# voutcn/megahit

Measured on NVIDIA H100. Metric: sorted (k+1)-mer edges/sec at k=27 on 150bp reads, higher is better.
Workload: dtype u32

## Files before the change

### include/mhb.h

```cpp
#ifndef MHB_H
#define MHB_H
#include <stddef.h>
#include <stdint.h>

#ifdef __cplusplus
extern "C" {
#endif

#define MHB_OK 0
#define MHB_ERR_ARG 1
#define MHB_ERR_CUDA 2
#define MHB_ERR_IO 3
#define MHB_ERR_NOMEM 4

#define MHB_NUM_BUCKETS 65536
#define MHB_MAX_MUL 65535
#define MHB_MAX_K 255
#define MHB_SENTINEL_OFFSET 0xFFFFFFFFu

const char *mhb_last_error(void);
const char *mhb_version(void);
int mhb_device_count(void);
uint64_t mhb_launch_count(void);

uint32_t mhb_count_record_words(uint32_t k);
uint32_t mhb_words_per_edge(uint32_t k);
uint32_t mhb_s2s_record_words(uint32_t k);
uint32_t mhb_count_sort_bytes(uint32_t k, uint8_t *bytes);
uint32_t mhb_s2s_sort_bytes(uint32_t k, uint8_t *bytes);
size_t mhb_sort_workspace_bytes(uint64_t n, uint32_t words);


typedef struct {
  const uint32_t *bin;
  uint64_t bin_words;
  uint64_t n_reads;
  uint32_t fixed_len;
  const uint64_t *rec_off;
  const uint64_t *edge_off;
} mhb_dev_reads;

int mhb_count_extract(void *stream, const mhb_dev_reads *reads, uint32_t k, uint32_t *records,
                      uint64_t n_edges, uint64_t *hist256, int hist_byte);

int mhb_check_fixed_len(void *stream, const uint32_t *bin_dev, uint64_t n_reads, uint32_t fixed_len, uint64_t *flag_dev);

int mhb_count_extract_range(void *stream, const mhb_dev_reads *reads, uint32_t k, uint32_t lo, uint32_t hi, int write,
                            uint64_t *per_read, uint32_t *records, uint64_t *hist256, int hist_byte,
                            uint64_t *total_dev);

int mhb_sort_records(void *stream, uint32_t *a, uint32_t *b, uint64_t n, uint32_t words,
                     const uint8_t *bytes, uint32_t n_bytes, const uint64_t *first_hist, void *ws,
                     size_t ws_bytes, int *result_in_b);

int mhb_sort_records_relaxed(void *stream, uint32_t *a, uint32_t *b, uint64_t n, uint32_t words, const uint8_t *bytes,
                             uint32_t n_bytes, const uint64_t *first_hist, void *ws, size_t ws_bytes, int *result_in_b);

int mhb_partition_scatter(void *stream, const uint32_t *recs, uint64_t n, uint32_t words, int byte,
                          const uint8_t *owner_of_byte_dev, const uint64_t *bin_addr_dev, void *ws, size_t ws_bytes);
int mhb_partition_scatter_hist(void *stream, const uint32_t *recs, uint64_t n, uint32_t words, int byte,
                               const uint8_t *owner_of_byte_dev, const uint64_t *bin_addr_dev, void *ws, size_t ws_bytes,
                               int next_byte, uint64_t *owner_next_hist, int *hist_done);
int mhb_plan_partition(void *stream, const uint64_t *hist_all_dev, uint32_t world, uint32_t rank, uint32_t record_bytes,
                       const uint64_t *peer_base_host, uint8_t *owner_lut_dev, uint64_t *bin_addr_dev, uint64_t *plan_dev);
int mhb_compact_tip_edges(void *stream, const uint32_t *edges, const uint8_t *aux, uint64_t n_solid, uint32_t k,
                          uint32_t *tips_out, uint8_t *tip_aux_out, uint64_t capacity, uint64_t *cursor_dev);
int mhb_dev_malloc(void **ptr, size_t bytes);
int mhb_dev_free(void *ptr);
int mhb_ipc_export(const void *dev_ptr, uint8_t *handle64);
int mhb_ipc_open(const uint8_t *handle64, void **peer_ptr);
int mhb_ipc_close(void *peer_ptr);

int mhb_set_sort_cfg(int cfg);

int mhb_sort_pass_ms(int back, double *pass_ms, uint32_t max_passes, uint32_t *n_passes, uint64_t *n_records,
                     uint32_t *words);

size_t mhb_count_solid_scratch_bytes(uint64_t n);
int mhb_count_solid(void *stream, const uint32_t *sorted_records, uint64_t n, uint32_t k, int32_t m,
                    uint32_t *edges_out, uint8_t *aux_out, uint64_t capacity_edges, uint64_t *mul_hist,
                    uint64_t *n_solid_out, void *scratch, size_t scratch_bytes);

int mhb_count_hashed_supported(uint32_t k, int32_t m);
size_t mhb_count_hashed_workspace_bytes(uint64_t n, uint32_t k, int32_t m);
int mhb_count_solid_hashed(void *stream, uint32_t *recs_a, uint32_t *recs_b, uint64_t n, uint32_t k, int32_t m,
                           const uint64_t *hist_byte5, uint32_t *edges_out, uint8_t *aux_out, uint64_t capacity_edges,
                           uint64_t *mul_hist, uint64_t *n_solid_out, void *ws, size_t ws_bytes);

size_t mhb_tipset_bytes(uint64_t n_tip_edges, uint32_t k);
int mhb_tipset_build(void *stream, const uint32_t *edges, const uint8_t *aux, uint64_t n_solid, uint32_t k,
                     void *tipset, size_t tipset_bytes, uint64_t n_tip_edges);
int mhb_count_mark_mercy(void *stream, const mhb_dev_reads *reads, uint32_t k, const void *tipset,
                         size_t tipset_bytes, uint64_t n_tip_edges, uint32_t *first_0_out, uint32_t *last_0_in);
int mhb_count_tip_edges(void *stream, const uint8_t *aux, uint64_t n_solid, uint64_t *n_tip_host);

size_t mhb_mercy_candidates_scratch_bytes(uint64_t n_reads);
int mhb_mercy_candidates(void *stream, const uint32_t *first_0_out, const uint32_t *last_0_in, uint64_t n_reads,
                         uint64_t *cand_ids, uint64_t *n_cand_host, void *scratch, size_t scratch_bytes);
size_t mhb_mercy_edges_scratch_bytes(uint64_t n_cand, uint32_t max_read_len);
int mhb_mercy_edges(void *stream, const mhb_dev_reads *reads, const uint64_t *cand_ids, uint64_t n_cand,
                    uint32_t max_read_len, uint32_t k, const uint32_t *edges, uint64_t n_edges, uint32_t *mercy_out,
                    uint64_t capacity, uint64_t *n_mercy_host, void *scratch, size_t scratch_bytes);
int mhb_mercy_edges_count(void *stream, const mhb_dev_reads *reads, const uint64_t *cand_ids, uint64_t n_cand,
                          uint32_t max_read_len, uint32_t k, uint32_t n_segs, const uint32_t *const *seg_edges,
                          const uint64_t *seg_counts, const void *const *seg_luts, const uint8_t *owner_of_byte,
                          uint64_t *n_mercy_host, void *scratch, size_t scratch_bytes);
int mhb_mercy_edges_write(void *stream, const mhb_dev_reads *reads, const uint64_t *cand_ids, uint64_t n_cand,
                          uint32_t max_read_len, uint32_t k, uint32_t *mercy_out, uint64_t capacity, uint64_t n_mercy,
                          void *scratch, size_t scratch_bytes);

size_t mhb_mercy_planes_words(uint64_t n_cand, uint32_t max_read_len);
int mhb_mercy_probe_owned(void *stream, const mhb_dev_reads *reads, const uint64_t *cand_ids, uint64_t n_cand,
                          uint32_t max_read_len, uint32_t k, const uint32_t *edges, uint64_t n_edges, const void *lut,
                          const uint8_t *owner_of_byte, uint32_t me, uint32_t *planes_out);
int mhb_mercy_count_planes(void *stream, const mhb_dev_reads *reads, const uint64_t *cand_ids, uint64_t n_cand,
                           uint32_t max_read_len, uint32_t k, const uint32_t *planes, uint32_t n_src,
                           uint64_t src_stride_words, uint64_t *n_mercy_host, void *scratch, size_t scratch_bytes);

int mhb_mercy_edges_segs(void *stream, const mhb_dev_reads *reads, const uint64_t *cand_ids, uint64_t n_cand,
                         uint32_t max_read_len, uint32_t k, uint32_t n_segs, const uint32_t *const *seg_edges,
                         const uint64_t *seg_counts, const void *const *seg_luts, const uint8_t *owner_of_byte,
                         uint32_t *mercy_out, uint64_t capacity, uint64_t *n_mercy_host, void *scratch,
                         size_t scratch_bytes);
size_t mhb_edge_lut_bytes(void);
int mhb_edge_lut_build(void *stream, const uint32_t *edges, uint64_t n_edges, uint32_t k, void *lut);

typedef struct {
  const uint32_t *words;
  uint64_t n_words;
  uint64_t n_seqs;
  uint32_t fixed_len;
  const uint64_t *word_off;
  const uint32_t *len;
  const uint64_t *item_off;
  const uint16_t *mult;
  uint32_t fixed_stride;
} mhb_dev_seqs;

int mhb_s2s_extract(void *stream, const mhb_dev_seqs *seqs, uint32_t k, uint32_t *records, uint64_t n_items,
// ... 139 lines not shown

typedef struct {
  uint32_t *bin;
  uint64_t bin_words;
  uint64_t n_reads, n_bases;
  uint32_t n_libs;
  uint64_t *lib_begin, *lib_end;
  uint32_t *lib_max_len;
  uint64_t n_chunks;
  uint64_t n_walk_passes;
  double t_total_ms;
} mhb_buildlib_result;

int mhb_buildlib_host(const mhb_buildlib_args *args, mhb_buildlib_result *res);
void mhb_buildlib_free(mhb_buildlib_result *res);
int mhb_set_buildlib_chunk(uint64_t bytes);

int mhb_mercy_host(uint32_t k, const uint32_t *edges, uint64_t n_edges, const uint32_t *cand_bin, uint64_t cand_words,
                   uint32_t **mercy_out, uint64_t *n_mercy_out, uint64_t *n_cand_reads_out);

void mhb_free(void *p);
int mhb_release(void);

typedef struct {
  uint32_t k;
  int32_t m;
  double host_mem;
  int32_t num_cpu_threads;
  const char *read_lib_file;
  const char *output_prefix;
  int32_t mem_flag;
} mhb_count_opts;

typedef struct {
  double host_mem;
  uint32_t k;
  uint32_t k_from;
  int32_t num_cpu_threads;
  const char *contig;
  const char *bubble;
  const char *addi_contig;
  const char *local_contig;
  const char *input_prefix;
  const char *output_prefix;
  int32_t need_mercy;
  int32_t mem_flag;
} mhb_seq2sdbg_opts;

typedef struct {
  uint32_t k;
  int32_t m;
  double host_mem;
  int32_t num_cpu_threads;
  const char *read_lib_file;
  const char *output_prefix;
  int32_t mem_flag;
  int32_t need_mercy;
} mhb_read2sdbg_opts;

typedef struct {
  const char *contig_file;
  const char *bubble_file;
  const char *read_file;
  int32_t num_cpu_threads;
  uint32_t k;
  uint32_t step;
  const char *output_prefix;
} mhb_iterate_opts;

int mhb_count_run(const mhb_count_opts *opts);
int mhb_seq2sdbg_run(const mhb_seq2sdbg_opts *opts);
int mhb_iterate_run(const mhb_iterate_opts *opts);
int mhb_read2sdbg_run(const mhb_read2sdbg_opts *opts);
int mhb_buildlib_run(const char *lib_file, const char *out_prefix);

int mhb_count_run_multi(const mhb_count_opts *opts, int n_gpus);

int mhb_selftest_count_record(const uint32_t *read_words, uint32_t nwords, uint32_t L, uint32_t k, uint32_t q,
                              uint32_t *rec_out, uint32_t *strand_out);
int mhb_selftest_count_records_roll(const uint32_t *read_words, uint32_t nwords, uint32_t L, uint32_t k, uint32_t q,
                                    uint64_t *rec4_out, uint32_t *strand4_out);
int mhb_selftest_s2s_record(const uint32_t *seq_words, uint32_t nwords, uint32_t L, uint32_t k, uint32_t strand,
                            uint32_t offset, uint32_t mult, uint32_t *rec_out);

int mhb_selftest_r2s_s1_record(const uint32_t *pkg_words, uint32_t nwords, uint32_t L, uint32_t k, uint32_t e,
                               uint64_t base_off, uint32_t *rec_out);
int mhb_selftest_r2s_item(const uint32_t *pkg_words, uint32_t nwords, uint32_t L, uint32_t k, uint32_t i, uint32_t strand,
                          uint32_t type, uint32_t *rec_out, uint32_t *palindrome_out);
int mhb_selftest_kmsort(uint32_t *recs, uint64_t n, uint32_t nw);
int mhb_selftest_kmsort_smem(uint32_t *recs, uint64_t n, uint32_t nw, uint32_t cap, uint32_t wcap);
int mhb_selftest_r2s_s1_group(const uint32_t *recs, uint64_t n, uint32_t k, int32_t m, uint32_t fixed_len, uint64_t n_reads,
                              int need_mercy, uint32_t *is_solid, uint32_t *no_in, uint32_t *no_out, uint32_t *any,
                              int64_t *counting);
int mhb_selftest_iterate(const mhb_iterate_args *args, mhb_iterate_result *res);
int mhb_selftest_fastx(const uint8_t *text, uint64_t n, uint32_t *len_out, uint32_t *bpos_out, uint64_t cap,
                       uint64_t *n_rec_out, uint32_t *bin_out, uint64_t bin_cap, uint64_t *bin_words_out);
int mhb_selftest_r2s_mercy_read(uint32_t fixed_len, uint64_t n_reads, uint64_t r, uint32_t k, const uint32_t *is_solid,
                                const uint32_t *no_in, const uint32_t *no_out, const uint32_t *any, uint32_t *mercy,
                                uint32_t *added_out);

#ifdef __cplusplus
}
#endif
#endif
```

### megahit_b200/csrc/mhb_hashcount.cu

```cuda
#include <cuda_runtime.h>
#include <stdio.h>
#include <string.h>

#include "mhb.h"
#include "mhb_common.cuh"
#include "mhb_count.cuh"

using namespace mhb;

namespace {

constexpr int kHcHist = 1024;
constexpr u64 kHcEmpty = ~0ull;
constexpr int kHcBatch = 8;
constexpr u32 kRemBits = 42;
constexpr u32 kHcHotCount = 256;
constexpr int kHcHotRound = 32;
constexpr int kHcMaxProbes = 48;
constexpr int kHcStack = 72;
constexpr u32 kHcHistDone = 1u << 31;
constexpr u32 kHcPrefetchChunk = 16384;

__device__ __forceinline__ u64 rec_key64(const uint2 r) { return ((u64)r.x << 32) | r.y; }

__global__ void k_bucket_bounds(const uint2 *__restrict__ recs, u64 n, u64 *__restrict__ bounds) {
  const u32 b = blockIdx.x * blockDim.x + threadIdx.x;
  if (b > 65536u) return;
  u64 lo = 0, hi = n;
  while (lo < hi) {
    const u64 mid = (lo + hi) >> 1;
    if ((recs[mid].x >> 16) < b) lo = mid + 1;
    else hi = mid;
  }
  bounds[b] = lo;
}

__device__ __forceinline__ u64 hc_align(const uint2 *__restrict__ recs, u64 p, u64 lo, u64 hi) {
  if (p <= lo) return lo;
  if (p >= hi) return hi;
  const u32 pre = recs[p - 1].x >> 8;
  u64 a = p, z = hi;
  while (a < z) {
    const u64 mid = (a + z) >> 1;
    if ((recs[mid].x >> 8) > pre) z = mid;
    else a = mid + 1;
  }
  return a;
}

__global__ void k_slice_plan(const uint2 *__restrict__ recs, const u64 *__restrict__ bounds, const u64 *__restrict__ slice_off,
                             int m, ulonglong2 *__restrict__ plan, u64 *__restrict__ slice_base, u32 *__restrict__ slice_bucket) {
  const u32 b = blockIdx.x * blockDim.x + threadIdx.x;
  if (b >= 65536u) return;
  const u64 s0 = slice_off[b], ns = slice_off[b + 1] - s0;
  if (!ns) return;
  const u64 blo = bounds[b], bhi = bounds[b + 1], step = (bhi - blo + ns - 1) / ns;
  u64 lo = blo;
  for (u64 i = 0; i < ns; ++i) {
    const u64 hi = i + 1 == ns ? bhi : hc_align(recs, blo + (i + 1) * step, blo, bhi);
    plan[s0 + i] = make_ulonglong2(lo, hi);
    slice_base[s0 + i] = lo / (u64)m + s0 + i;
    slice_bucket[s0 + i] = b;
    lo = hi;
  }
}

template <int THREADS_, int LOG_SLOTS_, int CTAS_>
struct HcGeom {
  static constexpr int THREADS = THREADS_, LOG_SLOTS = LOG_SLOTS_, SLOTS = 1 << LOG_SLOTS_, CTAS = CTAS_;
  static constexpr int MAX_SOLID = SLOTS / 4;
  static constexpr int CELLS = 2 * THREADS;
  static constexpr int LOG_CELLS = LOG_SLOTS_ - 2 >= 0 ? (THREADS_ == 256 ? 9 : (THREADS_ == 512 ? 10 : 11)) : 9;
  static constexpr u32 SLICE = (u32)(SLOTS * 1.83);
};

template <class G>
struct HcShared {
  u64 keys[G::SLOTS];
  u32 cnt[G::SLOTS];
  u32 pt[G::SLOTS];
  u32 nt[G::SLOTS];
  u64 sorted[G::MAX_SOLID];
  u64 tmp[G::MAX_SOLID];
  u32 cell_base[G::CELLS];
  u32 cell_cur[G::CELLS];
  u32 cta_hist[kHcHist];
  u32 wide[kHcHotRound][8];
  uint16_t hot_rank[G::MAX_SOLID];
  u64 st_prefix[kHcStack];
  u32 st_bits[kHcStack];
  u32 warp_sum[G::THREADS / 32];
  ulonglong2 nx_range[2];
  u32 nx_sl[2];
  u32 n_solid[2], n_hot[2], overflow[2];
};

__device__ __forceinline__ u32 lane_lt_mask() { return (1u << (threadIdx.x & 31)) - 1u; }

__device__ __forceinline__ void smem_add(u32 *p, u32 v) {
  asm volatile("red.shared.add.u32 [%0], %1;" ::"r"((u32)__cvta_generic_to_shared(p)), "r"(v) : "memory");
}

__device__ __forceinline__ void hc_prefetch_l2(const uint2 *recs, u64 lo, u64 hi) {
  const u64 a0 = (u64)(recs + lo) & ~15ull, a1 = (u64)(recs + hi) & ~15ull;
  for (u64 a = a0; a < a1; a += kHcPrefetchChunk) {
    const u32 sz = (u32)(a1 - a < kHcPrefetchChunk ? a1 - a : kHcPrefetchChunk);
    asm volatile("cp.async.bulk.prefetch.L2.global [%0], %1;" ::"l"(a), "r"(sz) : "memory");
  }
}

template <class G>
__device__ __forceinline__ u32 hc_hash(u64 r) { return (u32)((r * 0x9E3779B97F4A7C15ull) >> (64 - G::LOG_SLOTS)); }

template <class G>
__device__ __forceinline__ u32 hc_insert(HcShared<G> &s, u64 r) {
  u32 h = hc_hash<G>(r);
  for (int probes = 0; probes < kHcMaxProbes; ++probes) {
    u64 cur = s.keys[h];
// ... 358 lines not shown
                                                             misc + 1);
  CK_LAUNCH();
  return MHB_OK;
}

struct HcLayout {
  size_t sort_ws, off_bounds, off_bcnt, off_soff, off_bsum, off_misc, off_scount, off_sdst, off_sbase, off_sbucket, off_plan,
      off_list, total;
  uint64_t max_slices;
};
HcLayout hc_layout(uint64_t n, int32_t m) {
  HcLayout L;
  auto pad = [](size_t x) { return (x + 255) & ~(size_t)255; };
  L.max_slices = n / HcGeomB::SLICE + 65536 + 2;
  L.sort_ws = pad(mhb_sort_workspace_bytes(n, 2));
  size_t p = L.sort_ws;
  L.off_bounds = p;
  p += pad(65537 * 8);
  L.off_bcnt = p;
  p += pad(65537 * 4);
  L.off_soff = p;
  p += pad(65537 * 8);
  L.off_bsum = p;
  p += pad((L.max_slices / kScanTile + 4) * 8);
  L.off_misc = p;
  p += 256;
  L.off_scount = p;
  p += pad(L.max_slices * 4);
  L.off_sdst = p;
  p += pad(L.max_slices * 8);
  L.off_sbase = p;
  p += pad(L.max_slices * 8);
  L.off_sbucket = p;
  p += pad(L.max_slices * 4);
  L.off_plan = p;
  p += pad(L.max_slices * 16);
  L.off_list = p;
  p += pad((size_t)(n / (uint64_t)(m < 1 ? 1 : m) + L.max_slices + 8) * 8);
  L.total = p;
  return L;
}

}

extern "C" int mhb_count_hashed_supported(uint32_t k, int32_t m) {
  return count_record_words(k) == 2 && 2 * (k + 1) >= 24 && m >= 1 && m <= kHcHist;
}

extern "C" size_t mhb_count_hashed_workspace_bytes(uint64_t n, uint32_t k, int32_t m) {
  (void)k;
  return hc_layout(n, m).total;
}

extern "C" int mhb_count_solid_hashed(void *stream, uint32_t *recs_a, uint32_t *recs_b, uint64_t n, uint32_t k, int32_t m,
                                      const uint64_t *hist_byte5, uint32_t *edges_out, uint8_t *aux_out,
                                      uint64_t capacity_edges, uint64_t *mul_hist, uint64_t *n_solid_out, void *ws,
                                      size_t ws_bytes) {
  if (!mhb_count_hashed_supported(k, m)) return mhb_set_error(MHB_ERR_ARG, "hashed count needs 8-byte records (13 <= k <= 28) and 1 <= m <= %d", kHcHist);
  if (!mul_hist || !n_solid_out || !ws) return mhb_set_error(MHB_ERR_ARG, "bad args");
  if (n == 0) return MHB_OK;
  if (n >= (1ull << 40)) return mhb_set_error(MHB_ERR_ARG, "too many records for one hashed count call");
  const HcLayout L = hc_layout(n, m);
  if (ws_bytes < L.total) return mhb_set_error(MHB_ERR_ARG, "hashed count workspace too small (%zu < %zu)", ws_bytes, L.total);
  cudaStream_t st = (cudaStream_t)stream;
  const uint8_t bytes[3] = {5, 6, 7};
  int in_b = 0;
  if (int rc = mhb_sort_records_impl(st, recs_a, recs_b, n, 2, bytes, 3, hist_byte5, ws, L.sort_ws, &in_b, nullptr)) return rc;
  const uint2 *recs = (const uint2 *)(in_b ? recs_b : recs_a);
  char *w = (char *)ws;
  u64 *bounds = (u64 *)(w + L.off_bounds);
  u32 *bcnt = (u32 *)(w + L.off_bcnt);
  u64 *slice_off = (u64 *)(w + L.off_soff);
  u64 *bsum = (u64 *)(w + L.off_bsum);
  u32 *misc = (u32 *)(w + L.off_misc);
  u32 *slice_count = (u32 *)(w + L.off_scount);
  u64 *slice_dst = (u64 *)(w + L.off_sdst);
  u64 *slice_base = (u64 *)(w + L.off_sbase);
  u32 *slice_bucket = (u32 *)(w + L.off_sbucket);
  ulonglong2 *plan = (ulonglong2 *)(w + L.off_plan);
  u64 *list = (u64 *)(w + L.off_list);
  u64 *n_slices_dev = (u64 *)(misc + 2);
  CK(cudaMemsetAsync(misc, 0, 256, st));
  CK(cudaMemsetAsync(slice_count, 0, L.max_slices * 4, st));
  k_bucket_bounds<<<(65537 + 255) / 256, 256, 0, st>>>(recs, n, bounds);
  CK_LAUNCH();
  k_slice_counts<<<65536 / 256, 256, 0, st>>>(bounds, HcGeomB::SLICE, bcnt);
  CK_LAUNCH();
  if (int rc = scan_counts(st, bcnt, 65536, slice_off, n_slices_dev, bsum)) return rc;
  CK(cudaMemcpyAsync(slice_off + 65536, n_slices_dev, 8, cudaMemcpyDeviceToDevice, st));
  k_slice_plan<<<65536 / 256, 256, 0, st>>>(recs, bounds, slice_off, m, plan, slice_base, slice_bucket);
  CK_LAUNCH();
  if (int rc = launch_hash_count<HcGeomB>(st, recs, plan, n_slices_dev, m, misc, list, slice_count, mul_hist)) return rc;
  if (int rc = scan_counts(st, slice_count, L.max_slices, slice_dst, n_solid_out, bsum)) return rc;
  k_hash_gather<<<sm_count() * 4, 256, 0, st>>>(list, n_slices_dev, slice_count, slice_dst, slice_base, slice_bucket,
                                               words_per_edge(k), edges_out, aux_out, capacity_edges, misc + 1, n_solid_out);
  CK_LAUNCH();
  return MHB_OK;
}
```

### megahit_b200/csrc/mhb_host.cu

```cuda
#include <cuda_runtime.h>
#include <stdio.h>
#include <stdlib.h>
#include <string.h>

#include <algorithm>
#include <vector>

#include "mhb.h"
#include "mhb_bits.cuh"
#include "mhb_internal.h"

using namespace mhb;

#define CK(call)                                                                                   \
  do {                                                                                             \
    cudaError_t e_ = (call);                                                                       \
    if (e_ != cudaSuccess)                                                                         \
      return mhb_set_error(MHB_ERR_CUDA, "%s failed at %s:%d: %s", #call, __FILE__, __LINE__,      \
                           cudaGetErrorString(e_));                                                \
  } while (0)
#define CKR(call)           \
  do {                      \
    int rc_ = (call);       \
    if (rc_) return rc_;    \
// ... 570 lines not shown
  res->t_h2d_ms = t.stop();

  mhb_dev_reads reads;
  reads.bin = d_bin;
  reads.bin_words = args->bin_words;
  reads.n_reads = n_reads;
  reads.fixed_len = ix.fixed_len;
  reads.rec_off = d_rec_off;
  reads.edge_off = d_edge_off;

  t.start();
  CKR(mhb_count_extract(st, &reads, k, d_a, n, d_hist0, cw.hist_byte));
  res->t_extract_ms = t.stop();

  t.start();
  res->n_rounds = 1;
  CKR(run_count_stage(st, cw, d_a, d_b, n, k, m, d_hist0, d_edges, d_aux, cap_edges, d_mul_hist, d_nsolid, d_work,
                      res->sort_pass_ms, &res->n_sort_passes));
  for (uint32_t p = 0; p < res->n_sort_passes; ++p) res->t_sort_ms += res->sort_pass_ms[p];
  uint64_t n_solid = 0;
  CK(cudaMemcpyAsync(&n_solid, d_nsolid, 8, cudaMemcpyDeviceToHost, st));
  CK(cudaStreamSynchronize(st));
  res->t_count_ms = t.stop();
  if (n_solid > cap_edges) return mhb_set_error(MHB_ERR_NOMEM, "internal: solid edges exceed capacity");
  res->n_solid = n_solid;

  std::vector<uint32_t> h_first, h_last;
  if (args->want_mercy && n_reads) {
    t.start();
    uint64_t n_tip = 0;
    CKR(mhb_count_tip_edges(st, d_aux, n_solid, &n_tip));
    const size_t ts_bytes = mhb_tipset_bytes(n_tip, k);
    char *d_tips = nullptr;
    uint32_t *d_free = d_a;
    bool own = false;
    if (ts_bytes <= (size_t)n * WR * 4) d_tips = (char *)d_free;
    else {
      CK(cudaMalloc((void **)&d_tips, ts_bytes));
      own = true;
    }
    int rc = mhb_tipset_build(st, d_edges, d_aux, n_solid, k, d_tips, ts_bytes, n_tip);
    if (!rc) rc = mhb_count_mark_mercy(st, &reads, k, d_tips, ts_bytes, n_tip, d_first, d_last);
    h_first.resize(n_reads);
    h_last.resize(n_reads);
    if (!rc) {
      cudaMemcpyAsync(h_first.data(), d_first, n_reads * 4, cudaMemcpyDeviceToHost, st);
      cudaMemcpyAsync(h_last.data(), d_last, n_reads * 4, cudaMemcpyDeviceToHost, st);
      if (cudaStreamSynchronize(st) != cudaSuccess) rc = mhb_set_error(MHB_ERR_CUDA, "mercy marking failed: %s", cudaGetErrorString(cudaGetLastError()));
    }
    if (own) cudaFree(d_tips);
    if (rc) return rc;
    res->t_mercy_ms = t.stop();
  }

  t.start();
  res->edges = (uint32_t *)malloc(std::max<size_t>(1, (size_t)n_solid * WE * 4));
  if (!res->edges) return mhb_set_error(MHB_ERR_NOMEM, "host malloc failed");
  if (n_solid) CK(cudaMemcpyAsync(res->edges, d_edges, (size_t)n_solid * WE * 4, cudaMemcpyDeviceToHost, st));
  std::vector<uint64_t> h_hist(65536);
  CK(cudaMemcpyAsync(h_hist.data(), d_mul_hist, 65536 * 8, cudaMemcpyDeviceToHost, st));
  CK(cudaStreamSynchronize(st));
  res->t_d2h_ms = t.stop();
  for (int i = 0; i <= MHB_MAX_MUL; ++i) res->counting[i] = (int64_t)h_hist[i];

  if (args->want_mercy) {
    std::vector<uint64_t> ids;
    for (uint64_t r = 0; r < n_reads; ++r) {
      const uint32_t f = h_first[r], l = h_last[r];
      if (f != MHB_SENTINEL_OFFSET && l != MHB_SENTINEL_OFFSET) {
        ++res->n_has_tips;
        if (l > f) ids.push_back(r);
      }
    }
    res->n_cand = ids.size();
    res->cand_ids = (uint64_t *)malloc(std::max<size_t>(1, ids.size() * 8));
    if (!ids.empty()) memcpy(res->cand_ids, ids.data(), ids.size() * 8);
  }
  res->t_total_ms = t_all.stop();
  return MHB_OK;
}

namespace {
size_t s2s_round_bytes(uint64_t n, uint32_t W, uint32_t k) {
  return 2 * Arena::pad((size_t)n * W * 4 + 16) + Arena::pad(mhb_sort_workspace_bytes(n, W)) +
         Arena::pad(mhb_s2s_emit_scratch_bytes(n, k)) + Arena::pad((size_t)n * (4ull + 4ull * words_per_tip_label(k)) + 16);
}
}

static int s2s_host_rounds(const mhb_s2s_args *args, mhb_s2s_result *res, const std::vector<uint64_t> &item_off,
                           uint64_t n_items, bool fixed, uint32_t L0, uint64_t n_words, uint64_t max_items) {
  const uint32_t k = args->k;
  const uint64_t ns = args->n_seqs;
  const uint32_t W = s2s_record_words(k), WPT = words_per_tip_label(k);
  uint8_t sort_bytes[72];
  const uint32_t n_sort = mhb_s2s_sort_bytes(k, sort_bytes);
  const int top_byte = (int)(4 * W - 1);
  cudaStream_t st = 0;
  Timer t_all(st), t(st);
  t_all.start();

  const size_t fixed_b = Arena::pad(n_words * 4 + 64) + Arena::pad((ns + 1) * 8) * 2 + Arena::pad((ns + 1) * 4) +
                         Arena::pad((ns + 1) * 2) + Arena::pad((size_t)MHB_NUM_BUCKETS * 4 * 8) + 2 * Arena::pad(256 * 8) +
                         Arena::pad(16 * 8) + Arena::pad(64) + 8192;
  if (!max_items) {
    size_t free_b = 0, total_b = 0;
    CK(cudaMemGetInfo(&free_b, &total_b));
    const size_t avail = (size_t)((double)(free_b + g_arena.cap) * 0.92);
    if (avail <= fixed_b) return mhb_set_error(MHB_ERR_NOMEM, "the sequences alone (%zu bytes) do not fit the device", fixed_b);
    uint64_t lo = 1, hi = n_items;
    while (lo < hi) {
      const uint64_t mid = lo + (hi - lo + 1) / 2;
      if (fixed_b + s2s_round_bytes(mid, W, k) <= avail) lo = mid;
      else hi = mid - 1;
    }
    max_items = lo;
  }
  max_items = std::min<uint64_t>(std::max<uint64_t>(max_items, 1), std::max<uint64_t>(n_items, 1));
  CKR(g_arena.reserve(fixed_b + s2s_round_bytes(max_items, W, k)));
  uint32_t *d_words = g_arena.take<uint32_t>(n_words + 16);
  uint64_t *d_word_off = g_arena.take<uint64_t>(ns + 1);
  uint64_t *d_item_off = g_arena.take<uint64_t>(ns + 1);
  uint32_t *d_len = g_arena.take<uint32_t>(ns + 1);
  uint16_t *d_mult = g_arena.take<uint16_t>(ns + 1);
  uint64_t *d_table = g_arena.take<uint64_t>((size_t)MHB_NUM_BUCKETS * 4);
  uint64_t *d_hist0 = g_arena.take<uint64_t>(256);
  uint64_t *d_hist_top = g_arena.take<uint64_t>(256);
  uint64_t *d_totals = g_arena.take<uint64_t>(16);
  uint64_t *d_cursor = g_arena.take<uint64_t>(8);
  uint32_t *d_a = g_arena.take<uint32_t>((size_t)max_items * W + 4);
  uint32_t *d_b = g_arena.take<uint32_t>((size_t)max_items * W + 4);
  const size_t ws_bytes = mhb_sort_workspace_bytes(max_items, W);
  const size_t scratch_bytes = mhb_s2s_emit_scratch_bytes(max_items, k);
  const uint64_t cap_bytes = max_items * (4ull + 4ull * WPT) + 16;
  char *d_ws = g_arena.take<char>(ws_bytes);
  char *d_scratch = g_arena.take<char>(scratch_bytes);
  uint8_t *d_bytes = g_arena.take<uint8_t>(cap_bytes);

  if (ns) {
    CK(cudaMemcpyAsync(d_words, args->words, n_words * 4, cudaMemcpyHostToDevice, st));
    CK(cudaMemcpyAsync(d_word_off, args->word_off, (ns + 1) * 8, cudaMemcpyHostToDevice, st));
    CK(cudaMemcpyAsync(d_item_off, item_off.data(), (ns + 1) * 8, cudaMemcpyHostToDevice, st));
    CK(cudaMemcpyAsync(d_len, args->len, ns * 4, cudaMemcpyHostToDevice, st));
    CK(cudaMemcpyAsync(d_mult, args->mult, ns * 2, cudaMemcpyHostToDevice, st));
  }
  CK(cudaMemsetAsync(d_hist_top, 0, 256 * 8, st));
  mhb_dev_seqs seqs;
  seqs.words = d_words;
  seqs.n_words = n_words;
  seqs.n_seqs = ns;
  seqs.fixed_len = fixed ? L0 : 0;
  seqs.word_off = d_word_off;
  seqs.len = d_len;
  seqs.item_off = d_item_off;
  seqs.mult = d_mult;
  seqs.fixed_stride = 0;

  t.start();
  uint64_t h_top[256];
  CKR(mhb_s2s_extract_range(st, &seqs, k, nullptr, n_items, 0, 65535, nullptr, 0, d_hist_top, top_byte));
  CK(cudaMemcpyAsync(h_top, d_hist_top, sizeof(h_top), cudaMemcpyDeviceToHost, st));
  CK(cudaStreamSynchronize(st));
  std::vector<uint64_t> h_sub;
  for (uint32_t b = 0; b < 256; ++b) {
    if (h_top[b] <= max_items) continue;
    if (h_sub.empty()) h_sub.assign(256 * 256, 0);
    CK(cudaMemsetAsync(d_hist0, 0, 256 * 8, st));
    CKR(mhb_s2s_extract_range(st, &seqs, k, nullptr, n_items, b << 8, (b << 8) | 255u, nullptr, 0, d_hist0, top_byte - 1));
    CK(cudaMemcpyAsync(h_sub.data() + (size_t)b * 256, d_hist0, 256 * 8, cudaMemcpyDeviceToHost, st));
    CK(cudaStreamSynchronize(st));
  }
  std::vector<uint32_t> r_lo(65536), r_hi(65536);
  const int n_ranges = mhb_plan_rounds16(h_top, h_sub.empty() ? nullptr : h_sub.data(), max_items, r_lo.data(), r_hi.data(), 65536);
  if (n_ranges < 0) return MHB_ERR_NOMEM;
  res->t_extract_ms = t.stop();

  SdbgStitch out;
  for (int ri = 0; ri < n_ranges; ++ri) {
    t.start();
    CK(cudaMemsetAsync(d_hist0, 0, 256 * 8, st));
    CK(cudaMemsetAsync(d_cursor, 0, 64, st));
    CKR(mhb_s2s_extract_range(st, &seqs, k, d_a, n_items, r_lo[ri], r_hi[ri], d_cursor, max_items, d_hist0, sort_bytes[0]));
    uint64_t n_round = 0;
    CK(cudaMemcpyAsync(&n_round, d_cursor, 8, cudaMemcpyDeviceToHost, st));
    CK(cudaStreamSynchronize(st));
    res->t_extract_ms += t.stop();
    if (n_round > max_items) return mhb_set_error(MHB_ERR_NOMEM, "internal: round of %llu items exceeds its plan", (unsigned long long)n_round);
    if (n_round == 0) continue;
    t.start();
    int in_b = 0;
    CKR(mhb_sort_records_impl(st, d_a, d_b, n_round, W, sort_bytes, n_sort, d_hist0, d_ws, ws_bytes, &in_b, nullptr));
    res->t_sort_ms += t.stop();
    t.start();
    CKR(mhb_s2s_emit(st, in_b ? d_b : d_a, n_round, k, d_bytes, cap_bytes, d_table, d_totals, d_scratch, scratch_bytes));
    CKR(out.append(st, d_bytes, cap_bytes, d_table, d_totals));
    res->t_emit_ms += t.stop();
  }
  res->n_bytes = out.tot[0];
  res->n_items = out.tot[1];
  res->n_tips = out.tot[2];
  res->n_large_mul = out.tot[3];
  for (int i = 0; i < 9; ++i) res->w_count[i] = out.tot[4 + i];
  res->ones_in_last = out.tot[13];
  memcpy(res->bucket_table, out.table.data(), sizeof(res->bucket_table));
  res->bytes = (uint8_t *)malloc(std::max<size_t>(1, out.bytes.size()));
  if (!res->bytes) return mhb_set_error(MHB_ERR_NOMEM, "host malloc failed");
  if (!out.bytes.empty()) memcpy(res->bytes, out.bytes.data(), out.bytes.size());
  res->t_total_ms = t_all.stop();
  return MHB_OK;
}

extern "C" int mhb_s2s_host(const mhb_s2s_args *args, mhb_s2s_result *res) {
  if (!args || !res) return mhb_set_error(MHB_ERR_ARG, "null args");
  memset(res, 0, sizeof(*res));
  const uint32_t k = args->k;
  if (k < 9 || k > MHB_MAX_K) return mhb_set_error(MHB_ERR_ARG, "kmer size must be >= 9!");
  if (mhb_device_count() == 0) return mhb_set_error(MHB_ERR_CUDA, "no CUDA device: libmhb has no CPU path");
  res->words_per_tip_label = words_per_tip_label(k);
  const uint64_t ns = args->n_seqs;

  std::vector<uint64_t> item_off(ns + 1);
  uint64_t n_items = 0;
  bool fixed = ns > 0;
  const uint32_t L0 = ns ? args->len[0] : 0;
  for (uint64_t s = 0; s < ns; ++s) {
    item_off[s] = n_items;
    const uint32_t L = args->len[s];
    if (L >= k + 1) n_items += 2ull * (L - k + 2);
    if (L != L0 || args->word_off[s] != s * (uint64_t)div_ceil(L0, 16)) fixed = false;
  }
  item_off[ns] = n_items;
  if (L0 < k + 1) fixed = false;
  const uint64_t n_words = ns ? args->word_off[ns] : 0;
  res->n_records = n_items;

  cudaStream_t st = 0;
  Timer t_all(st), t(st);
  t_all.start();
  const uint32_t W = s2s_record_words(k);
  uint8_t sort_bytes[72];
  const uint32_t n_sort = mhb_s2s_sort_bytes(k, sort_bytes);
  const size_t ws_bytes = mhb_sort_workspace_bytes(n_items, W);
  const size_t scratch_bytes = mhb_s2s_emit_scratch_bytes(n_items, k);
  const uint64_t cap_bytes = n_items * (4ull + 4ull * res->words_per_tip_label) + 16;
  size_t need = Arena::pad(n_words * 4 + 64) + Arena::pad((ns + 1) * 8) * 2 + Arena::pad((ns + 1) * 4) +
                Arena::pad((ns + 1) * 2) + 2 * Arena::pad((size_t)n_items * W * 4 + 16) + Arena::pad(ws_bytes) +
                Arena::pad(scratch_bytes) + Arena::pad(cap_bytes) + Arena::pad((size_t)MHB_NUM_BUCKETS * 4 * 8) +
                Arena::pad(256 * 8) + Arena::pad(16 * 8) + 4096;
  {
    bool rounds = g_s2s_round_limit && n_items > g_s2s_round_limit;
    if (!rounds && need > g_arena.cap) {
      size_t free_b = 0, total_b = 0;
      CK(cudaMemGetInfo(&free_b, &total_b));
      rounds = (double)need > 0.92 * (double)(free_b + g_arena.cap);
    }
    if (rounds) return s2s_host_rounds(args, res, item_off, n_items, fixed, L0, n_words, g_s2s_round_limit);
  }
  CKR(g_arena.reserve(need));
  uint32_t *d_words = g_arena.take<uint32_t>(n_words + 16);
  uint64_t *d_word_off = g_arena.take<uint64_t>(ns + 1);
  uint64_t *d_item_off = g_arena.take<uint64_t>(ns + 1);
  uint32_t *d_len = g_arena.take<uint32_t>(ns + 1);
  uint16_t *d_mult = g_arena.take<uint16_t>(ns + 1);
  uint32_t *d_a = g_arena.take<uint32_t>((size_t)n_items * W + 4);
  uint32_t *d_b = g_arena.take<uint32_t>((size_t)n_items * W + 4);
  char *d_ws = g_arena.take<char>(ws_bytes);
  char *d_scratch = g_arena.take<char>(scratch_bytes);
  uint8_t *d_bytes = g_arena.take<uint8_t>(cap_bytes);
  uint64_t *d_table = g_arena.take<uint64_t>((size_t)MHB_NUM_BUCKETS * 4);
  uint64_t *d_hist0 = g_arena.take<uint64_t>(256);
  uint64_t *d_totals = g_arena.take<uint64_t>(16);

  if (ns) {
    CK(cudaMemcpyAsync(d_words, args->words, n_words * 4, cudaMemcpyHostToDevice, st));
    CK(cudaMemcpyAsync(d_word_off, args->word_off, (ns + 1) * 8, cudaMemcpyHostToDevice, st));
    CK(cudaMemcpyAsync(d_item_off, item_off.data(), (ns + 1) * 8, cudaMemcpyHostToDevice, st));
    CK(cudaMemcpyAsync(d_len, args->len, ns * 4, cudaMemcpyHostToDevice, st));
    CK(cudaMemcpyAsync(d_mult, args->mult, ns * 2, cudaMemcpyHostToDevice, st));
  }
  CK(cudaMemsetAsync(d_hist0, 0, 256 * 8, st));

  mhb_dev_seqs seqs;
  seqs.words = d_words;
  seqs.n_words = n_words;
  seqs.n_seqs = ns;
  seqs.fixed_len = fixed ? L0 : 0;
  seqs.word_off = d_word_off;
  seqs.len = d_len;
  seqs.item_off = d_item_off;
  seqs.mult = d_mult;
  seqs.fixed_stride = 0;

  t.start();
  CKR(mhb_s2s_extract(st, &seqs, k, d_a, n_items, d_hist0, sort_bytes[0]));
  res->t_extract_ms = t.stop();
  t.start();
  int in_b = 0;
  CKR(mhb_sort_records_impl(st, d_a, d_b, n_items, W, sort_bytes, n_sort, d_hist0, d_ws, ws_bytes, &in_b, nullptr));
  res->t_sort_ms = t.stop();
  t.start();
  CKR(mhb_s2s_emit(st, in_b ? d_b : d_a, n_items, k, d_bytes, cap_bytes, d_table, d_totals, d_scratch, scratch_bytes));
  uint64_t totals[16];
  CK(cudaMemcpyAsync(totals, d_totals, sizeof(totals), cudaMemcpyDeviceToHost, st));
  CK(cudaMemcpyAsync(res->bucket_table, d_table, sizeof(res->bucket_table), cudaMemcpyDeviceToHost, st));
  CK(cudaStreamSynchronize(st));
  res->t_emit_ms = t.stop();
  res->n_bytes = totals[0];
  res->n_items = totals[1];
  res->n_tips = totals[2];
  res->n_large_mul = totals[3];
  for (int i = 0; i < 9; ++i) res->w_count[i] = totals[4 + i];
  res->ones_in_last = totals[13];
  if (res->n_bytes > cap_bytes) return mhb_set_error(MHB_ERR_NOMEM, "internal: SdBG byte stream exceeds capacity");
  res->bytes = (uint8_t *)malloc(std::max<size_t>(1, res->n_bytes));
  if (!res->bytes) return mhb_set_error(MHB_ERR_NOMEM, "host malloc failed");
  if (res->n_bytes) CK(cudaMemcpy(res->bytes, d_bytes, res->n_bytes, cudaMemcpyDeviceToHost));
  res->t_total_ms = t_all.stop();
  return MHB_OK;
}

static int build_host_impl(const mhb_build_args *args, mhb_build_result *res, bool full_index);

static int build_host_rounds(const mhb_build_args *args, mhb_build_result *res) {
  memset(res, 0, sizeof(*res));
  const uint32_t k = args->k, WE = words_per_edge(k), NWE = div_ceil(k + 1, 16);
  mhb_count_args ca;
  memset(&ca, 0, sizeof(ca));
  ca.k = k;
  ca.m = args->m;
  ca.bin = args->bin;
  ca.bin_words = args->bin_words;
  ca.n_reads = args->n_reads;
  ca.want_mercy = args->need_mercy;
  std::vector<char> cbuf(sizeof(mhb_count_result));
  mhb_count_result *cr = reinterpret_cast<mhb_count_result *>(cbuf.data());
  CKR(mhb_count_host(&ca, cr));
  struct Owned {
    mhb_count_result *r;
    ~Owned() {
      free(r->edges);
      free(r->cand_ids);
    }
  } owned{cr};
  res->n_edge_records = cr->n_edge_records;
  res->n_solid = cr->n_solid;
  res->n_cand = cr->n_cand;
  res->words_per_edge = WE;
  res->words_per_tip_label = words_per_tip_label(k);
  res->t_count_ms = cr->t_total_ms;
  uint32_t *mercy = nullptr;
  uint64_t n_mercy = 0;
  if (args->need_mercy && cr->n_cand) {
    std::vector<uint32_t> cand;
    uint64_t r = 0;
    size_t pos = 0;
    for (uint64_t c = 0; c < cr->n_cand; ++c) {
      while (r < cr->cand_ids[c]) {
        pos += 1 + div_ceil(args->bin[pos], 16);
        ++r;
      }
      const uint32_t L = args->bin[pos], nw = div_ceil(L, 16);
      const size_t at = cand.size();
      cand.resize(at + 1 + nw, 0u);
      cand[at] = L;
      for (uint32_t i = 0; i < L; ++i) cand[at + 1 + (i >> 4)] |= base_at(&args->bin[pos + 1], L - 1 - i) << (30 - 2 * (i & 15));
    }
    uint64_t n_cr = 0;
    CKR(mhb_mercy_host(k, cr->edges, cr->n_solid, cand.data(), cand.size(), &mercy, &n_mercy, &n_cr));
  }
  struct FreeMercy {
    uint32_t *&p;
    ~FreeMercy() { free(p); }
  } fm{mercy};
  res->n_mercy = n_mercy;
  const uint64_t n_seqs = cr->n_solid + n_mercy;
  std::vector<uint32_t> words((size_t)n_seqs * NWE + 1, 0u), len(n_seqs, k + 1);
  std::vector<uint64_t> word_off(n_seqs + 1);
  std::vector<uint16_t> mult(n_seqs);
  const uint32_t tail = (k + 1) % 16;
  for (uint64_t i = 0; i < n_seqs; ++i) {
    const uint32_t *e = i < cr->n_solid ? cr->edges + i * WE : mercy + (i - cr->n_solid) * WE;
// ... 6 lines not shown
  mhb_s2s_args sa;
  memset(&sa, 0, sizeof(sa));
  sa.k = k;
  sa.words = words.data();
  sa.word_off = word_off.data();
  sa.len = len.data();
  sa.mult = mult.data();
  sa.n_seqs = n_seqs;
  std::vector<char> sbuf(sizeof(mhb_s2s_result));
  mhb_s2s_result *sr = reinterpret_cast<mhb_s2s_result *>(sbuf.data());
  CKR(mhb_s2s_host(&sa, sr));
  res->n_sort_items = sr->n_records;
  res->n_items = sr->n_items;
  res->n_tips = sr->n_tips;
  res->n_large_mul = sr->n_large_mul;
  res->n_bytes = sr->n_bytes;
  for (int i = 0; i < 9; ++i) res->w_count[i] = sr->w_count[i];
  res->ones_in_last = sr->ones_in_last;
  res->t_s2s_ms = sr->t_total_ms;
  res->bucket_table = (uint64_t *)malloc((size_t)MHB_NUM_BUCKETS * 32);
  if (!res->bucket_table) {
    free(sr->bytes);
    return mhb_set_error(MHB_ERR_NOMEM, "host malloc failed");
  }
  memcpy(res->bucket_table, sr->bucket_table, (size_t)MHB_NUM_BUCKETS * 32);
  if (args->sdbg_out && args->sdbg_out_capacity >= sr->n_bytes) {
    if (sr->n_bytes) memcpy(args->sdbg_out, sr->bytes, sr->n_bytes);
    free(sr->bytes);
    res->bytes = args->sdbg_out;
  } else {
    res->bytes = sr->bytes;
  }
  if (args->want_edges) {
    res->counting = (int64_t *)malloc(65536 * 8);
    if (!res->counting) return mhb_set_error(MHB_ERR_NOMEM, "host malloc failed");
    memcpy(res->counting, cr->counting, 65536 * 8);
    res->edges = cr->edges;
    res->cand_ids = cr->cand_ids;
    cr->edges = nullptr;
    cr->cand_ids = nullptr;
  }
  res->t_total_ms = res->t_count_ms + res->t_s2s_ms;
  return MHB_OK;
}

extern "C" int mhb_build_host(const mhb_build_args *args, mhb_build_result *res) {
  if (!args || !res) return mhb_set_error(MHB_ERR_ARG, "null args");
  if (g_round_limit || g_s2s_round_limit) return build_host_rounds(args, res);
  const int rc = build_host_impl(args, res, false);
  if (rc == MHB_ERR_NOMEM) {
    mhb_free(res->bytes == args->sdbg_out ? nullptr : res->bytes);
    mhb_free(res->bucket_table);
    mhb_free(res->edges);
    mhb_free(res->cand_ids);
    mhb_free(res->counting);
    mhb_release();
    return build_host_rounds(args, res);
  }
  return rc;
}
static int build_host_impl(const mhb_build_args *args, mhb_build_result *res, bool full_index) {
  memset(res, 0, sizeof(*res));
  const uint32_t k = args->k;
  if (k < 9 || k > MHB_MAX_K) return mhb_set_error(MHB_ERR_ARG, "kmer size must be >= 9 and <= 255");
  if (args->need_mercy && k < 12) return mhb_set_error(MHB_ERR_ARG, "mercy edges need k >= 12");
  if (mhb_device_count() == 0) return mhb_set_error(MHB_ERR_CUDA, "no CUDA device: libmhb has no CPU path");
  const uint32_t WR = count_record_words(k), WE = words_per_edge(k), W2 = s2s_record_words(k), WPT = words_per_tip_label(k);
  res->words_per_edge = WE;
  res->words_per_tip_label = WPT;

  BinIndex ix;
  CKR(index_bin(args->bin, args->bin_words, args->n_reads, k, &ix, !full_index));
  const bool verify_fixed = !full_index && ix.fixed_len != 0;
  const uint64_t n = ix.n_edges, n_reads = args->n_reads;
  res->n_edge_records = n;
  uint32_t max_len = ix.fixed_len;
  if (!ix.fixed_len)
    for (uint64_t r = 0; r < n_reads; ++r) max_len = std::max(max_len, args->bin[ix.rec_off[r]]);

  cudaStream_t st = 0;
  Timer t_all(st), t(st);
  t_all.start();

  uint8_t cbytes[72], sbytes[72];
  const uint32_t n_csort = mhb_count_sort_bytes(k, cbytes), n_ssort = mhb_s2s_sort_bytes(k, sbytes);
  const int32_t m = args->m;
  const uint64_t cap_edges = n / (uint64_t)std::max(1, m) + 1;
  const size_t bin_bytes = (args->bin_words * 4 + 15) & ~(size_t)15;
  const CountWork cw = count_work_plan(n, k, m);
  const size_t count_work = 2 * Arena::pad((size_t)n * WR * 4 + 16) + Arena::pad(cw.bytes);
  size_t fixed = Arena::pad(bin_bytes + 16) + Arena::pad((size_t)cap_edges * WE * 4) + Arena::pad(cap_edges) +
                 Arena::pad(65536 * 8) + 2 * Arena::pad(256 * 8) + Arena::pad(64) + Arena::pad((size_t)MHB_NUM_BUCKETS * 32) +
                 Arena::pad(128) + 8192;
  if (!ix.fixed_len) fixed += 2 * Arena::pad((n_reads + 1) * 8);
  if (args->need_mercy) fixed += 2 * Arena::pad((n_reads + 1) * 4) + Arena::pad((n_reads + 1) * 8);
  CKR(g_arena.reserve(fixed + count_work));

  uint32_t *d_bin = g_arena.take<uint32_t>(bin_bytes / 4 + 4);
  uint32_t *d_edges = g_arena.take<uint32_t>((size_t)cap_edges * WE);
  uint8_t *d_aux = g_arena.take<uint8_t>(cap_edges);
  uint64_t *d_mul_hist = g_arena.take<uint64_t>(65536);
  uint64_t *d_hist0 = g_arena.take<uint64_t>(256);
  uint64_t *d_hist1 = g_arena.take<uint64_t>(256);
  uint64_t *d_nsolid = g_arena.take<uint64_t>(8);
  uint64_t *d_table = g_arena.take<uint64_t>((size_t)MHB_NUM_BUCKETS * 4);
  uint64_t *d_totals = g_arena.take<uint64_t>(16);
  uint64_t *d_rec_off = nullptr, *d_edge_off = nullptr, *d_cand = nullptr;
  uint32_t *d_first = nullptr, *d_last = nullptr;
  if (!ix.fixed_len) {
    d_rec_off = g_arena.take<uint64_t>(n_reads + 1);
    d_edge_off = g_arena.take<uint64_t>(n_reads + 1);
  }
  if (args->need_mercy) {
    d_first = g_arena.take<uint32_t>(n_reads + 1);
    d_last = g_arena.take<uint32_t>(n_reads + 1);
    d_cand = g_arena.take<uint64_t>(n_reads + 1);
  }
  char *work = g_arena.take<char>(count_work);
  size_t work_bytes = count_work;
  char *extra = nullptr;
  char *big_edges = nullptr;
  struct ExtraGuard {
    char *&p;
    ~ExtraGuard() {
      if (p) cudaFree(p);
    }
  } guard{extra}, guard2{big_edges};
  uint32_t *d_all_edges = d_edges;

  static const int h2d_chunks_env = getenv("MHB_H2D_CHUNKS") ? atoi(getenv("MHB_H2D_CHUNKS")) : 4;
  const bool chunked = h2d_chunks_env > 1 && ix.fixed_len >= k + 1 && n_reads >= (uint64_t)h2d_chunks_env * 64;
  t.start();
  CK(cudaMemsetAsync(d_mul_hist, 0, 65536 * 8, st));
  CK(cudaMemsetAsync(d_hist0, 0, 256 * 8, st));
  CK(cudaMemsetAsync(d_hist1, 0, 256 * 8, st));
  CK(cudaMemsetAsync(d_nsolid, 0, 64, st));
  if (!chunked) {
    if (args->bin_words) CK(cudaMemcpyAsync(d_bin, args->bin, args->bin_words * 4, cudaMemcpyHostToDevice, st));
    if (!ix.fixed_len && n_reads) {
      CK(cudaMemcpyAsync(d_rec_off, ix.rec_off.data(), (n_reads + 1) * 8, cudaMemcpyHostToDevice, st));
      CK(cudaMemcpyAsync(d_edge_off, ix.edge_off.data(), (n_reads + 1) * 8, cudaMemcpyHostToDevice, st));
    }
  }
  res->t_h2d_ms = t.stop();

  mhb_dev_reads reads;
  reads.bin = d_bin;
  reads.bin_words = args->bin_words;
  reads.n_reads = n_reads;
  reads.fixed_len = ix.fixed_len;
  reads.rec_off = d_rec_off;
  reads.edge_off = d_edge_off;

  t.start();
  uint32_t *c_a = (uint32_t *)work;
  uint32_t *c_b = (uint32_t *)(work + Arena::pad((size_t)n * WR * 4 + 16));
  char *c_wsp = work + 2 * Arena::pad((size_t)n * WR * 4 + 16);
  if (!chunked) {
    CKR(mhb_count_extract(st, &reads, k, c_a, n, d_hist0, cw.hist_byte));
  } else {
    static cudaStream_t copy_st = nullptr;
    static cudaEvent_t ev[64];
    static bool ev_ready = false;
    if (!ev_ready) {
      CK(cudaStreamCreateWithFlags(&copy_st, cudaStreamNonBlocking));
      for (int i = 0; i < 64; ++i) CK(cudaEventCreateWithFlags(&ev[i], cudaEventDisableTiming));
      ev_ready = true;
    }
// ... 5 lines not shown
    CK(cudaEventRecord(start_ev, st));
    CK(cudaStreamWaitEvent(copy_st, start_ev, 0));
    int c = 0;
    for (uint64_t r0 = 0; r0 < n_reads; r0 += per, ++c) {
      const uint64_t r1 = std::min(n_reads, r0 + per);
      const uint64_t w0 = r0 * stride, w1 = r1 * stride;
      CK(cudaMemcpyAsync(d_bin + w0, args->bin + w0, (w1 - w0) * 4, cudaMemcpyHostToDevice, copy_st));
      CK(cudaEventRecord(ev[c], copy_st));
      CK(cudaStreamWaitEvent(st, ev[c], 0));
      mhb_dev_reads piece = reads;
      piece.bin = d_bin + w0;
      piece.bin_words = w1 - w0;
      piece.n_reads = r1 - r0;
      CKR(mhb_count_extract(st, &piece, k, c_a + (size_t)r0 * e_per_read * WR, (r1 - r0) * e_per_read, d_hist0, cw.hist_byte));
    }
  }
  if (verify_fixed) CKR(mhb_check_fixed_len(st, d_bin, n_reads, ix.fixed_len, d_nsolid + 1));
  CKR(run_count_stage(st, cw, c_a, c_b, n, k, m, d_hist0, d_edges, d_aux, cap_edges, d_mul_hist, d_nsolid, c_wsp, nullptr, nullptr));
  uint64_t h_scal[2] = {0, 0};
  CK(cudaMemcpyAsync(h_scal, d_nsolid, 16, cudaMemcpyDeviceToHost, st));
  CK(cudaStreamSynchronize(st));
  if (verify_fixed && h_scal[1]) return build_host_impl(args, res, true);
  const uint64_t n_solid = h_scal[0];
  if (n_solid > cap_edges) return mhb_set_error(MHB_ERR_NOMEM, "internal: solid edges exceed capacity");
  res->n_solid = n_solid;
  res->t_count_ms = t.stop();

  uint64_t n_cand = 0, n_mercy = 0;
  if (args->need_mercy && n_reads) {
    t.start();
    uint64_t n_tip = 0;
    CKR(mhb_count_tip_edges(st, d_aux, n_solid, &n_tip));
    const size_t ts_bytes = mhb_tipset_bytes(n_tip, k);
    const size_t cs_bytes = mhb_mercy_candidates_scratch_bytes(n_reads);
    auto work_area = [&](size_t bytes) -> char * {
      if (bytes <= work_bytes) return work;
      if (extra) cudaFree(extra);
      extra = nullptr;
      if (cudaMalloc((void **)&extra, bytes) != cudaSuccess) {
        cudaGetLastError();
        return nullptr;
      }
      return extra;
    };
    char *d_tips = work_area(Arena::pad(ts_bytes) + Arena::pad(cs_bytes));
    if (!d_tips) return mhb_set_error(MHB_ERR_NOMEM, "cudaMalloc for the mercy stage failed");
    char *d_cs = d_tips + Arena::pad(ts_bytes);
    CKR(mhb_tipset_build(st, d_edges, d_aux, n_solid, k, d_tips, ts_bytes, n_tip));
    CKR(mhb_count_mark_mercy(st, &reads, k, d_tips, ts_bytes, n_tip, d_first, d_last));
    CKR(mhb_mercy_candidates(st, d_first, d_last, n_reads, d_cand, &n_cand, d_cs, cs_bytes));
    if (n_cand) {
      const size_t ms_bytes = mhb_mercy_edges_scratch_bytes(n_cand, max_len);
      CK(cudaStreamSynchronize(st));
      char *d_ms = work_area(ms_bytes);
      if (!d_ms) return mhb_set_error(MHB_ERR_NOMEM, "cudaMalloc for the mercy stage failed");
      const size_t core = ms_bytes - mhb_edge_lut_bytes();
      void *lut = d_ms + core;
      CKR(mhb_edge_lut_build(st, d_edges, n_solid, k, lut));
      const uint32_t *seg_e[1] = {d_edges};
      const uint64_t seg_n[1] = {n_solid};
      const void *seg_l[1] = {lut};
      CKR(mhb_mercy_edges_count(st, &reads, d_cand, n_cand, max_len, k, 1, seg_e, seg_n, seg_l, nullptr, &n_mercy, d_ms, core));
      if (n_mercy > cap_edges - n_solid) {
        const size_t eb = Arena::pad((size_t)(n_solid + n_mercy) * WE * 4 + 16);
        if (cudaMalloc((void **)&big_edges, eb) != cudaSuccess) {
          cudaGetLastError();
          return mhb_set_error(MHB_ERR_NOMEM, "cudaMalloc of %zu bytes for solid + mercy edges failed", eb);
        }
        CK(cudaMemcpyAsync(big_edges, d_edges, (size_t)n_solid * WE * 4, cudaMemcpyDeviceToDevice, st));
        d_all_edges = (uint32_t *)big_edges;
      }
      CKR(mhb_mercy_edges_write(st, &reads, d_cand, n_cand, max_len, k, d_all_edges + (size_t)n_solid * WE, n_mercy, n_mercy,
                                d_ms, core));
    }
    res->t_mercy_ms = t.stop();
  }
  res->n_cand = n_cand;
  res->n_mercy = n_mercy;

  t.start();
  const uint64_t n_seqs = n_solid + n_mercy;
  const uint64_t n_items = n_seqs * 6;
  res->n_sort_items = n_items;
  const size_t s_ws = mhb_sort_workspace_bytes(n_items, W2), s_scr = mhb_s2s_emit_scratch_bytes(n_items, k);
  const uint64_t cap_bytes = n_items * (4ull + 4ull * WPT) + 16;
  const size_t s2s_work = 2 * Arena::pad((size_t)n_items * W2 * 4 + 16) + Arena::pad(s_ws) + Arena::pad(s_scr) + Arena::pad(cap_bytes);
  char *sw = work;
  if (s2s_work > work_bytes) {
    CK(cudaStreamSynchronize(st));
    if (extra) cudaFree(extra);
    extra = nullptr;
    cudaError_t e = cudaMalloc((void **)&extra, s2s_work);
    if (e != cudaSuccess) {
      cudaGetLastError();
      return mhb_set_error(MHB_ERR_NOMEM, "cudaMalloc of %zu bytes for the SdBG stage failed", s2s_work);
    }
    sw = extra;
  }
  uint32_t *s_a = (uint32_t *)sw;
  uint32_t *s_b = (uint32_t *)(sw + Arena::pad((size_t)n_items * W2 * 4 + 16));
  char *s_wsp = sw + 2 * Arena::pad((size_t)n_items * W2 * 4 + 16);
  char *s_scrp = s_wsp + Arena::pad(s_ws);
  uint8_t *d_bytes = (uint8_t *)(s_scrp + Arena::pad(s_scr));
  mhb_dev_seqs seqs;
  memset(&seqs, 0, sizeof(seqs));
  seqs.words = d_all_edges;
  seqs.n_words = n_seqs * WE;
  seqs.n_seqs = n_seqs;
  seqs.fixed_len = k + 1;
  seqs.fixed_stride = WE;
  static const bool no_prune = getenv("MHB_S2S_NO_PRUNE") != nullptr;
  uint64_t n_sorted = n_items;
  if (!no_prune) {
    CK(cudaMemsetAsync(d_nsolid + 4, 0, 8, st));
    CKR(mhb_s2s_extract_edges_pruned(st, d_all_edges, d_aux, n_seqs, n_solid, k, s_a, n_items, d_nsolid + 4, d_hist1, sbytes[0]));
    CK(cudaMemcpyAsync(&n_sorted, d_nsolid + 4, 8, cudaMemcpyDeviceToHost, st));
    CK(cudaStreamSynchronize(st));
    if (n_sorted > n_items) return mhb_set_error(MHB_ERR_CUDA, "internal: pruned item count exceeds 6 per edge");
    res->n_sort_items = n_sorted;
  } else {
    CKR(mhb_s2s_extract(st, &seqs, k, s_a, n_items, d_hist1, sbytes[0]));
  }
  int s_in_b = 0;
  CKR(mhb_sort_records_impl(st, s_a, s_b, n_sorted, W2, sbytes, n_ssort, d_hist1, s_wsp, s_ws, &s_in_b, nullptr));
  CKR(mhb_s2s_emit(st, s_in_b ? s_b : s_a, n_sorted, k, d_bytes, cap_bytes, d_table, d_totals, s_scrp, s_scr));
  uint64_t totals[16];
  CK(cudaMemcpyAsync(totals, d_totals, sizeof(totals), cudaMemcpyDeviceToHost, st));
  CK(cudaStreamSynchronize(st));
  res->t_s2s_ms = t.stop();
  res->n_bytes = totals[0];
  res->n_items = totals[1];
  res->n_tips = totals[2];
  res->n_large_mul = totals[3];
  for (int i = 0; i < 9; ++i) res->w_count[i] = totals[4 + i];
  res->ones_in_last = totals[13];
  if (res->n_bytes > cap_bytes) return mhb_set_error(MHB_ERR_NOMEM, "internal: SdBG byte stream exceeds capacity");

  t.start();
  res->bucket_table = (uint64_t *)malloc((size_t)MHB_NUM_BUCKETS * 32);
  if (args->sdbg_out && args->sdbg_out_capacity >= res->n_bytes) res->bytes = args->sdbg_out;
  else res->bytes = (uint8_t *)malloc(std::max<size_t>(1, res->n_bytes));
  if (!res->bucket_table || !res->bytes) return mhb_set_error(MHB_ERR_NOMEM, "host malloc failed");
  CK(cudaMemcpyAsync(res->bucket_table, d_table, (size_t)MHB_NUM_BUCKETS * 32, cudaMemcpyDeviceToHost, st));
  if (res->n_bytes) CK(cudaMemcpyAsync(res->bytes, d_bytes, res->n_bytes, cudaMemcpyDeviceToHost, st));
  if (args->want_edges) {
    res->edges = (uint32_t *)malloc(std::max<size_t>(1, (size_t)n_solid * WE * 4));
    res->cand_ids = (uint64_t *)malloc(std::max<size_t>(1, n_cand * 8));
    res->counting = (int64_t *)malloc(65536 * 8);
    if (!res->edges || !res->cand_ids || !res->counting) return mhb_set_error(MHB_ERR_NOMEM, "host malloc failed");
    if (n_solid) CK(cudaMemcpyAsync(res->edges, d_edges, (size_t)n_solid * WE * 4, cudaMemcpyDeviceToHost, st));
    if (n_cand) CK(cudaMemcpyAsync(res->cand_ids, d_cand, n_cand * 8, cudaMemcpyDeviceToHost, st));
    CK(cudaMemcpyAsync(res->counting, d_mul_hist, 65536 * 8, cudaMemcpyDeviceToHost, st));
  }
  CK(cudaStreamSynchronize(st));
  res->t_d2h_ms = t.stop();
  res->t_total_ms = t_all.stop();
  return MHB_OK;
}

extern "C" int mhb_mercy_host(uint32_t k, const uint32_t *edges, uint64_t n_edges, const uint32_t *cand_bin,
                              uint64_t cand_words, uint32_t **mercy_out, uint64_t *n_mercy_out, uint64_t *n_cand_reads_out) {
  if (!mercy_out || !n_mercy_out) return mhb_set_error(MHB_ERR_ARG, "null output");
  *mercy_out = nullptr;
  *n_mercy_out = 0;
  if (n_cand_reads_out) *n_cand_reads_out = 0;
  if (k < 12 || k > MHB_MAX_K) return mhb_set_error(MHB_ERR_ARG, "mercy edges need 12 <= k <= 255");
  if (mhb_device_count() == 0) return mhb_set_error(MHB_ERR_CUDA, "no CUDA device: libmhb has no CPU path");
  const uint32_t WE = words_per_edge(k);
  std::vector<uint32_t> bin;
  std::vector<uint64_t> rec_off, edge_off;
  bin.reserve(cand_words + 8);
  uint32_t max_len = 0;
  uint64_t pos = 0, e = 0;
  while (pos < cand_words) {
    const uint32_t L = cand_bin[pos], nw = div_ceil(L, 16);
    if (pos + 1 + nw > cand_words) return mhb_set_error(MHB_ERR_IO, "candidate read image is truncated");
    rec_off.push_back(bin.size());
    edge_off.push_back(e);
    if (L >= k + 1) e += L - k;
    const size_t at = bin.size();
    bin.resize(at + 1 + nw, 0);
    bin[at] = L;
    for (uint32_t i = 0; i < L; ++i)
      bin[at + 1 + (i >> 4)] |= base_at(cand_bin + pos + 1, L - 1 - i) << (30 - 2 * (i & 15));
    max_len = std::max(max_len, L);
    pos += 1 + nw;
  }
  const uint64_t n_reads = rec_off.size();
  rec_off.push_back(bin.size());
  edge_off.push_back(e);
  if (n_cand_reads_out) *n_cand_reads_out = n_reads;
  if (n_reads == 0 || n_edges == 0) {
    *mercy_out = (uint32_t *)malloc(4);
    return MHB_OK;
  }
  const size_t bin_bytes = (bin.size() * 4 + 15) & ~(size_t)15;
  const size_t ms_bytes = mhb_mercy_edges_scratch_bytes(n_reads, max_len);
  const size_t need = Arena::pad(bin_bytes + 16) + 3 * Arena::pad((n_reads + 1) * 8) + Arena::pad((size_t)n_edges * WE * 4 + 16) +
                      Arena::pad(ms_bytes) + 4096;
  CKR(g_arena.reserve(need));
  cudaStream_t st = 0;
  uint32_t *d_bin = g_arena.take<uint32_t>(bin_bytes / 4 + 4);
  uint64_t *d_rec_off = g_arena.take<uint64_t>(n_reads + 1);
  uint64_t *d_edge_off = g_arena.take<uint64_t>(n_reads + 1);
  uint64_t *d_ids = g_arena.take<uint64_t>(n_reads + 1);
  uint32_t *d_edges = g_arena.take<uint32_t>((size_t)n_edges * WE + 4);
  char *d_ms = g_arena.take<char>(ms_bytes);
// ... 96 lines not shown
```

### megahit_b200/csrc/mhb_internal.h

```cpp
#pragma once
#include <stddef.h>
#include <stdint.h>

#include <vector>

int mhb_set_error(int code, const char *fmt, ...);

int mhb_sort_records_impl(void *stream, uint32_t *a, uint32_t *b, uint64_t n, uint32_t words, const uint8_t *bytes,
                          uint32_t n_bytes, const uint64_t *first_hist, void *ws, size_t ws_bytes, int *result_in_b,
                          double *pass_ms_host);

size_t mhb_arena_bytes(void);

struct SdbgStitch {
  std::vector<uint8_t> bytes;
  std::vector<uint64_t> table = std::vector<uint64_t>((size_t)65536 * 4);
  uint64_t tot[16] = {0};
  int append(void *stream, const uint8_t *d_bytes, uint64_t cap_bytes, const uint64_t *d_table, const uint64_t *d_totals);

 private:
  std::vector<uint64_t> round_table = std::vector<uint64_t>((size_t)65536 * 4);
};
```

### megahit_b200/csrc/mhb_kernels.cuh

```cuda
#pragma once
#include <cuda_runtime.h>
#include <stdint.h>

#include "mhb_bits.cuh"

namespace mhb {

static constexpr u32 kSentinel = 4;


template <int W, int WR>
MHB_HD void make_count_record(const u32 *s, u32 nwords, u32 L, u32 k, u32 q, u32 (&rec)[WR], u32 &strand) {
  const u32 K1 = k + 1;
  u32 prev_pkg, next_pkg;
  bool st;
  if constexpr (W == 2) {
    const u32 w0 = q >> 4, sh = (q & 15) * 2;
    const u32 x0 = s[w0];
    const u32 x1 = (w0 + 1 < nwords) ? s[w0 + 1] : 0u;
    const u32 x2 = (w0 + 2 < nwords) ? s[w0 + 2] : 0u;
    const u32 pi = q + K1;
    const u32 pw = ((pi >> 4) == w0 + 1) ? x1 : x2;
    prev_pkg = (pi < L) ? ((pw >> (30 - 2 * (pi & 15))) & 3u) : kSentinel;
    const u32 nwd = (q & 15) ? x0 : (q ? s[w0 - 1] : 0u);
// ... 8 lines not shown
    rec[1] = (u32)key;
    if constexpr (WR == 3) rec[2] = 0u;
  } else {
    prev_pkg = (q + K1 < L) ? base_at(s, q + K1) : kSentinel;
    next_pkg = (q > 0) ? base_at(s, q - 1) : kSentinel;
    u32 S[W], A[W], B[W];
    load_sub<W>(s, nwords, q, K1, S);
    reverse_sub<W>(S, K1, A);
    complement_sub<W>(S, K1, B);
    st = less_words<W>(B, A);
#pragma unroll
    for (int j = 0; j < WR; ++j) rec[j] = j < W ? (st ? B[j] : A[j]) : 0u;
  }
  u32 p = prev_pkg, n = next_pkg;
  if (st) {
    p = next_pkg == kSentinel ? kSentinel : 3u - next_pkg;
    n = prev_pkg == kSentinel ? kSentinel : 3u - prev_pkg;
  }
  rec[WR - 1] |= (p << 3) | n;
  strand = st ? 1u : 0u;
}

template <int R>
MHB_HD void make_count_records_roll(const u32 *s, u32 nwords, u32 L, u32 k, u32 q, u64 (&rec)[R], u32 (&strand)[R]) {
  const u32 K1 = k + 1;
  const u32 T = 64u - 2u * K1;
  const u32 w0 = q >> 4, sh = (q & 15) * 2;
  const u32 x0 = s[w0];
  const u32 x1 = (w0 + 1 < nwords) ? s[w0 + 1] : 0u;
  const u32 x2 = (w0 + 2 < nwords) ? s[w0 + 2] : 0u;
  const u32 x3 = (w0 + 3 < nwords) ? s[w0 + 3] : 0u;
  u64 S = ((((u64)fshl(x0, x1, sh) << 32) | fshl(x1, x2, sh)) >> T) << T;
  u64 B = ((~S) >> T) << T;
  u64 A = (((u64)rev2((u32)S) << 32) | rev2((u32)(S >> 32))) << T;
  const u32 pi = q + K1;
  const u32 wa = (pi >> 4) - w0;
  u32 LA = fshl(wa == 1 ? x1 : x2, wa == 1 ? x2 : x3, (pi & 15) * 2);
  u32 next_pkg = (q > 0) ? (((q & 15) ? (x0 >> (32 - sh)) : s[w0 - 1]) & 3u) : kSentinel;
  const u64 lowmask = ~((1ull << T) - 1ull);
#pragma unroll
  for (int j = 0; j < R; ++j) {
    const u32 b = LA >> 30;
    const u32 prev_pkg = (pi + j < L) ? b : kSentinel;
    const bool st = B < A;
    const u64 key = st ? B : A;
    u32 p = prev_pkg, n = next_pkg;
    if (st) {
      p = next_pkg == kSentinel ? kSentinel : 3u - next_pkg;
      n = prev_pkg == kSentinel ? kSentinel : 3u - prev_pkg;
    }
    rec[j] = key | (u64)((p << 3) | n);
    strand[j] = st ? 1u : 0u;
    next_pkg = (u32)(S >> 62);
    S = (S << 2) | ((u64)b << T);
    B = (B << 2) | ((u64)(3u - b) << T);
    A = ((A >> 2) & lowmask) | ((u64)b << 62);
    LA <<= 2;
  }
}

template <int W>
MHB_HD void make_s2s_record(const u32 *s, u32 nwords, u32 L, u32 k, u32 strand, u32 offset, u32 mult,
                            u32 (&rec)[W]) {
  const u32 nc = k - ((offset + k > L) ? 1u : 0u);
  const u32 counting = (offset > 0 && offset + k <= L) ? mult : 0u;
  u32 prev;
  if (strand == 0) {
    prev = offset == 0 ? kSentinel : base_at(s, offset - 1);
    load_sub<W>(s, nwords, offset, nc, rec);
  } else {
    prev = offset == 0 ? kSentinel : 3u - base_at(s, L - offset);
    int off2 = (int)L - (int)k - (int)offset;
    if (off2 < 0) off2 = 0;
    u32 S[W], T[W];
    load_sub<W>(s, nwords, (u32)off2, nc, S);
    reverse_sub<W>(S, nc, T);
    complement_sub<W>(T, nc, rec);
  }
  rec[W - 1] |= ((nc == k) ? 1u : 0u) << 19;
  rec[W - 1] |= prev << 16;
  rec[W - 1] |= 65535u - counting;
}

#if defined(__CUDACC__)
template <int WR>
__device__ __forceinline__ void ld_rec(const u32 *base, u64 idx, u32 (&r)[WR]) {
  if constexpr (WR % 4 == 0) {
    const uint4 *p = reinterpret_cast<const uint4 *>(base + idx * WR);
#pragma unroll
    for (int j = 0; j < WR / 4; ++j) {
      const uint4 v = p[j];
      r[4 * j] = v.x;
      r[4 * j + 1] = v.y;
      r[4 * j + 2] = v.z;
      r[4 * j + 3] = v.w;
    }
  } else if constexpr (WR % 2 == 0) {
    const uint2 *p = reinterpret_cast<const uint2 *>(base + idx * WR);
#pragma unroll
    for (int j = 0; j < WR / 2; ++j) {
      const uint2 v = p[j];
      r[2 * j] = v.x;
      r[2 * j + 1] = v.y;
    }
  } else {
    const u32 *p = base + idx * WR;
#pragma unroll
    for (int j = 0; j < WR; ++j) r[j] = p[j];
  }
}
template <int WR>
__device__ __forceinline__ void st_rec(u32 *base, u64 idx, const u32 (&r)[WR]) {
  if constexpr (WR % 4 == 0) {
    uint4 *p = reinterpret_cast<uint4 *>(base + idx * WR);
#pragma unroll
    for (int j = 0; j < WR / 4; ++j) p[j] = make_uint4(r[4 * j], r[4 * j + 1], r[4 * j + 2], r[4 * j + 3]);
  } else if constexpr (WR % 2 == 0) {
    uint2 *p = reinterpret_cast<uint2 *>(base + idx * WR);
#pragma unroll
    for (int j = 0; j < WR / 2; ++j) p[j] = make_uint2(r[2 * j], r[2 * j + 1]);
  } else {
    u32 *p = base + idx * WR;
#pragma unroll
    for (int j = 0; j < WR; ++j) p[j] = r[j];
  }
}

template <int WR>
__device__ __forceinline__ u32 rec_byte(const u32 (&r)[WR], int b) {
  return (pick<WR>(r, (u32)(WR - 1 - (b >> 2))) >> (8 * (b & 3))) & 255u;
}

__device__ __forceinline__ u32 lane_id() { return threadIdx.x & 31; }
__device__ __forceinline__ u32 lanemask_lt() {
  u32 m;
  asm("mov.u32 %0, %%lanemask_lt;" : "=r"(m));
  return m;
}

__device__ __forceinline__ u32 smem_u32(const void *p) { return (u32)__cvta_generic_to_shared(p); }
__device__ __forceinline__ void mbar_init(u64 *bar, u32 count) {
  asm volatile("mbarrier.init.shared::cta.b64 [%0], %1;" ::"r"(smem_u32(bar)), "r"(count) : "memory");
}
__device__ __forceinline__ void mbar_fence_init() {
  asm volatile("fence.mbarrier_init.release.cluster;" ::: "memory");
  asm volatile("fence.proxy.async.shared::cta;" ::: "memory");
}
__device__ __forceinline__ void mbar_expect_tx(u64 *bar, u32 bytes) {
  asm volatile("mbarrier.arrive.expect_tx.shared::cta.b64 _, [%0], %1;" ::"r"(smem_u32(bar)), "r"(bytes)
               : "memory");
}
__device__ __forceinline__ void bulk_g2s(void *dst, const void *src, u32 bytes, u64 *bar) {
  asm volatile("cp.async.bulk.shared::cluster.global.mbarrier::complete_tx::bytes [%0], [%1], %2, [%3];" ::"r"(
                   smem_u32(dst)),
               "l"(src), "r"(bytes), "r"(smem_u32(bar))
               : "memory");
}
__device__ __forceinline__ bool mbar_try_wait(u64 *bar, u32 parity) {
  u32 ok;
  asm volatile(
      "{\n\t.reg .pred p;\n\tmbarrier.try_wait.parity.shared::cta.b64 p, [%1], %2;\n\tselp.u32 %0, 1, 0, p;\n\t}"
      : "=r"(ok)
      : "r"(smem_u32(bar)), "r"(parity)
      : "memory");
  return ok != 0;
}
__device__ __forceinline__ void mbar_wait(u64 *bar, u32 parity) {
  while (!mbar_try_wait(bar, parity)) {
  }
}

__device__ __forceinline__ u64 ld_relaxed(const u64 *p) {
  u64 v;
  asm volatile("ld.relaxed.gpu.global.u64 %0, [%1];" : "=l"(v) : "l"(p) : "memory");
  return v;
}
__device__ __forceinline__ void st_relaxed(u64 *p, u64 v) {
  asm volatile("st.relaxed.gpu.global.u64 [%0], %1;" ::"l"(p), "l"(v) : "memory");
}

static constexpr u64 kLbPartial = 1ull << 62, kLbInclusive = 2ull << 62, kLbStatusMask = 3ull << 62;
static constexpr u64 kLbValueMask = (1ull << 54) - 1;
__host__ __device__ inline u64 lb_epoch(u32 e) { return (u64)(e & 255u) << 54; }

template <int THREADS>
__device__ __forceinline__ u32 block_excl_scan(u32 v, u32 *s_warp , u32 &total) {
  const u32 lane = lane_id(), warp = threadIdx.x >> 5;
  u32 inc = v;
#pragma unroll
  for (int d = 1; d < 32; d <<= 1) {
    u32 t = __shfl_up_sync(0xffffffffu, inc, d);
    if (lane >= (u32)d) inc += t;
  }
  if (lane == 31) s_warp[warp] = inc;
  __syncthreads();
  if (warp == 0) {
    u32 w = lane < THREADS / 32 ? s_warp[lane] : 0u;
    u32 winc = w;
#pragma unroll
    for (int d = 1; d < 32; d <<= 1) {
      u32 t = __shfl_up_sync(0xffffffffu, winc, d);
      if (lane >= (u32)d) winc += t;
    }
    if (lane < THREADS / 32) s_warp[lane] = winc - w;
    if (lane == 31) s_warp[THREADS / 32] = winc;
  }
  __syncthreads();
  u32 res = s_warp[warp] + inc - v;
  total = s_warp[THREADS / 32];
  __syncthreads();
  return res;
}
#endif
// ... 3 lines not shown
```

### megahit_b200/csrc/mhb_r2s.cu

```cuda
#include <stdio.h>
#include <stdlib.h>
#include <string.h>

#include <algorithm>
#include <vector>

#include "mhb_common.cuh"
#include "mhb_r2s.cuh"

using namespace mhb;

int scan32(cudaStream_t st, const uint32_t *in, uint64_t n, uint64_t *out, uint64_t *total_dev, uint64_t *bsum);
#define MHB_FOR_RW(M) M(3) M(4) M(5) M(6) M(7) M(8) M(9) M(10) M(11) M(12) M(13) M(14) M(15) M(16) M(17)

namespace {

struct DevBuf {
  void *p = nullptr;
  size_t bytes = 0;
  ~DevBuf() { release(); }
  void release() {
    if (p) cudaFree(p);
    p = nullptr;
    bytes = 0;
// ... 85 lines not shown
    int bad = 0;
#pragma omp parallel for reduction(| : bad) schedule(static)
    for (long long r = 0; r < (long long)n_reads; ++r) bad |= bin[(uint64_t)r * stride] != L0;
    fixed = !bad;
  }
  if (fixed) {
    ix->fixed_len = ix->max_len = L0;
    ix->fixed_words = div_ceil(L0, 16);
    ix->n_words = n_reads * ix->fixed_words;
    ix->n_bases = n_reads * (uint64_t)L0;
    if (L0 >= k + 1) {
      ix->n_s1 = n_reads * (uint64_t)(L0 - k + 4);
      ix->n_edges = n_reads * (uint64_t)(L0 - k);
    }
    return MHB_OK;
  }
  ix->rec_off.resize(n_reads + 1);
  ix->word_off.resize(n_reads + 1);
  ix->base_off.resize(n_reads + 1);
  ix->s1_off.resize(n_reads + 1);
  ix->edge_off.resize(n_reads + 1);
  ix->len.resize(n_reads);
  uint64_t pos = 0, w = 0, b = 0, s1 = 0, e = 0;
  for (uint64_t r = 0; r < n_reads; ++r) {
    if (pos >= bin_words) return mhb_set_error(MHB_ERR_ARG, ".bin image truncated at read %llu", (unsigned long long)r);
    const uint32_t L = bin[pos];
    const uint32_t eff = L == 0 ? 1 : L;
    ix->rec_off[r] = pos;
    ix->word_off[r] = w;
    ix->base_off[r] = b;
    ix->s1_off[r] = s1;
    ix->edge_off[r] = e;
    ix->len[r] = eff;
    ix->max_len = std::max(ix->max_len, eff);
    pos += 1 + div_ceil(L, 16);
    w += div_ceil(eff, 16);
    b += eff;
    if (eff >= k + 1) {
      s1 += eff - k + 4;
      e += eff - k;
    }
  }
  if (pos > bin_words) return mhb_set_error(MHB_ERR_ARG, ".bin image truncated");
  ix->rec_off[n_reads] = pos;
  ix->word_off[n_reads] = w;
  ix->base_off[n_reads] = b;
  ix->s1_off[n_reads] = s1;
  ix->edge_off[n_reads] = e;
  ix->n_words = w;
  ix->n_bases = b;
  ix->n_s1 = s1;
  ix->n_edges = e;
  return MHB_OK;
}

template <class T>
int upload(DevBuf &d, const std::vector<T> &v, const char *what) {
  CKR(d.alloc(v.size() * sizeof(T), what));
  if (!v.empty()) CK(cudaMemcpy(d.p, v.data(), v.size() * sizeof(T), cudaMemcpyHostToDevice));
  return MHB_OK;
}

uint64_t g_r2s_s1_limit = 0, g_r2s_s2_limit = 0;

size_t pad(size_t b) { return (b + 255) & ~(size_t)255; }

size_t free_device_bytes() {
  size_t f = 0, t = 0;
  if (cudaMemGetInfo(&f, &t) != cudaSuccess) {
    cudaGetLastError();
    return 0;
  }
  return f;
}

size_t s1_pass_bytes(uint64_t n, uint32_t RW) {
  const uint64_t seg_cap = n / (kKmInsertThreshold + 1) + 2;
  return 2 * pad((size_t)n * RW * 4 + 16) + pad(mhb_sort_workspace_bytes(n, RW)) + pad((MHB_NUM_BUCKETS + 1) * 8) +
         2 * pad(seg_cap * sizeof(KmSeg)) + 2 * pad((n / 32 + 2) * 4) + pad((size_t)n * 2 + 64) + 256;
}

size_t s2_pass_bytes(uint64_t n, uint32_t W, uint32_t k) {
  const uint64_t n_tiles = (n + kDdTile - 1) / kDdTile;
  return 2 * pad((size_t)n * W * 4 + 16) + pad(mhb_sort_workspace_bytes(n, W)) + pad(n_tiles * 4) + pad(n_tiles * 8) +
         pad((n_tiles / 4096 + 4) * 8) + pad((size_t)n * 8) + pad(mhb_s2s_emit_scratch_bytes(n, k)) +
         pad((size_t)n * (4ull + 4ull * words_per_tip_label(k)) + 16);
}

template <class F>
uint64_t largest_round(uint64_t n_max, size_t fixed, size_t avail, F bytes) {
  if (fixed + bytes(1) > avail) return 0;
  uint64_t lo = 1, hi = std::max<uint64_t>(n_max, 1);
  while (lo < hi) {
    const uint64_t mid = lo + (hi - lo + 1) / 2;
    if (fixed + bytes(mid) <= avail) lo = mid;
    else hi = mid - 1;
  }
  return lo;
}

int plan_bucket_ranges(const std::vector<uint64_t> &h16, uint64_t max_n, std::vector<std::pair<uint32_t, uint32_t>> *out) {
  uint64_t h256[256] = {0};
  for (size_t b = 0; b < (size_t)MHB_NUM_BUCKETS; ++b) h256[b >> 8] += h16[b];
  std::vector<uint32_t> lo(MHB_NUM_BUCKETS), hi(MHB_NUM_BUCKETS);
  const int n = mhb_plan_rounds16(h256, h16.data(), max_n, lo.data(), hi.data(), MHB_NUM_BUCKETS);
  if (n < 0) return MHB_ERR_NOMEM;
  out->clear();
  for (int i = 0; i < n; ++i) out->push_back({lo[i], hi[i]});
  return MHB_OK;
}

int s1_sort_post(cudaStream_t st, const PkgView &pv, uint32_t k, int32_t m, bool need_mercy, const S1Out &out,
                 unsigned long long *d_mul_hist, PhaseTrace &tr, BigBufs &big, uint64_t n);

int run_stage1(cudaStream_t st, const PkgView &pv, const PkgIndex &ix, uint32_t k, int32_t m, bool need_mercy, const S1Out &out,
               unsigned long long *d_mul_hist, PhaseTrace &tr, BigBufs &big, size_t min_rec_bytes, size_t min_ws_bytes) {
  const uint32_t NW = r2s_s1_key_words(k), RW = NW + 2;
  const uint64_t n = ix.n_s1;
  if (n == 0) return MHB_OK;
  if (RW > 17)
    return mhb_set_error(MHB_ERR_ARG, "read2sdbg: stage 1 supports k <= 237 (record of %u words > 17)", RW);
  if (n >= (1ull << 40)) return mhb_set_error(MHB_ERR_ARG, "read2sdbg: too many stage-1 records for one round");
  DevBuf &a = big.a, &b = big.b, &ws = big.ws;
  const size_t rec_bytes = (size_t)n * RW * 4 + 16, ws_bytes = mhb_sort_workspace_bytes(n, RW);
  CKR(a.ensure(std::max(rec_bytes, min_rec_bytes), "records"));
  CKR(b.ensure(std::max(rec_bytes, min_rec_bytes), "records (sort buffer)"));
  CKR(ws.ensure(std::max(ws_bytes, min_ws_bytes), "sort workspace"));
#define M(WW)                                                                                         \
  if (NW == WW) k_r2s_s1_extract<WW><<<grid_for(n, 256), 256, 0, st>>>(pv, k, a.as<u32>(), n);
  MHB_FOR_W(M)
#undef M
  CK_LAUNCH();
  tr.mark("s1.extract");
  return s1_sort_post(st, pv, k, m, need_mercy, out, d_mul_hist, tr, big, n);
}

int run_stage1_rounds(cudaStream_t st, const PkgView &pv, const PkgIndex &ix, uint32_t k, int32_t m, bool need_mercy,
                      const S1Out &out, unsigned long long *d_mul_hist, PhaseTrace &tr, BigBufs &big, uint64_t max_n,
                      uint32_t *n_rounds) {
  const uint32_t NW = r2s_s1_key_words(k), RW = NW + 2;
  if (RW > 17)
    return mhb_set_error(MHB_ERR_ARG, "read2sdbg: stage 1 supports k <= 237 (record of %u words > 17)", RW);
  const uint64_t n_reads = ix.n_reads;
  DevBuf per_read, off, bsum, h16, total;
  CKR(per_read.alloc(n_reads * 4, "per-read record counts"));
  CKR(off.alloc((n_reads + 1) * 8, "per-read record offsets"));
  CKR(bsum.alloc((n_reads / 4096 + 4) * 8, "scan sums"));
  CKR(h16.alloc(MHB_NUM_BUCKETS * 8, "bucket histogram"));
  CKR(total.alloc(8, "round size"));
  CKR(big.a.ensure((size_t)max_n * RW * 4 + 16, "records"));
  CKR(big.b.ensure((size_t)max_n * RW * 4 + 16, "records (sort buffer)"));
  CKR(big.ws.ensure(mhb_sort_workspace_bytes(max_n, RW), "sort workspace"));
  const unsigned grid = grid_for(n_reads * 32, 256);
  CK(cudaMemsetAsync(h16.p, 0, MHB_NUM_BUCKETS * 8, st));
#define M(WW)      \
  if (NW == WW)    \
    k_r2s_s1_range<WW, kS1Hist><<<grid, 256, 0, st>>>(pv, k, 0, 65535, h16.as<unsigned long long>(), nullptr, nullptr, nullptr);
  MHB_FOR_W(M)
#undef M
  CK_LAUNCH();
  std::vector<uint64_t> h_h16(MHB_NUM_BUCKETS);
  CK(cudaMemcpyAsync(h_h16.data(), h16.p, MHB_NUM_BUCKETS * 8, cudaMemcpyDeviceToHost, st));
  CK(cudaStreamSynchronize(st));
  tr.mark("s1.extract.plan");
  std::vector<std::pair<uint32_t, uint32_t>> ranges;
  CKR(plan_bucket_ranges(h_h16, max_n, &ranges));
  uint64_t seen = 0;
// ... 77 lines not shown
    u32 *other = in_b ? a.as<u32>() : b.as<u32>();
#define M(WW)                                                                                                           \
  if (RW == WW) {                                                                                                       \
    CK(cudaFuncSetAttribute(k_r2s_km_bucket<WW>, cudaFuncAttributeMaxDynamicSharedMemorySize, (int)cap));               \
    k_r2s_km_bucket<WW><<<MHB_NUM_BUCKETS, 128, cap, st>>>(recs, other, bstart.as<u64>(), NW, kb, cap,                   \
                                                           src16.as<uint16_t>(), bnd.as<u32>(), d_todo, nxt, d_cnt, seg_cap); \
  }
    MHB_FOR_RW(M)
#undef M
    CK_LAUNCH();
    recs = other;
  } else {
#define M(WW)                                                                                                      \
  if (RW == WW)                                                                                                    \
    k_r2s_kmsort_level<WW><<<MHB_NUM_BUCKETS / 128, 128, 0, st>>>(recs, NW, kb, nullptr, bstart.as<u64>(),          \
                                                                  MHB_NUM_BUCKETS, nxt, d_cnt, seg_cap, bnd.as<u32>());
    MHB_FOR_RW(M)
#undef M
    CK_LAUNCH();
  }
  for (;;) {
    snprintf(level_names[level], sizeof(level_names[level]), "s1.kmsort.L%d", level);
    tr.mark(level_names[level]);
    if (level < 71) ++level;
    unsigned long long n_next = 0;
    CK(cudaMemcpyAsync(&n_next, d_cnt, 8, cudaMemcpyDeviceToHost, st));
    CK(cudaStreamSynchronize(st));
    if (n_next == 0 || kb == 0) break;
    if (n_next > seg_cap) return mhb_set_error(MHB_ERR_CUDA, "read2sdbg: internal: kmsort range list overflow");
    std::swap(cur, nxt);
    --kb;
    CK(cudaMemsetAsync(d_cnt, 0, 8, st));
    if (!km_global) {
#define M(WW)                                                                                                            \
  if (RW == WW) {                                                                                                        \
    const size_t smem = (size_t)kKmWarps * km_warp_smem<WW>();                                                           \
    static bool attr = false;                                                                                            \
    if (!attr) {                                                                                                         \
      CK(cudaFuncSetAttribute(k_r2s_km_warp<WW>, cudaFuncAttributeMaxDynamicSharedMemorySize, (int)smem));               \
      attr = true;                                                                                                       \
    }                                                                                                                    \
    uint64_t g = (n_next + kKmWarps - 1) / kKmWarps;                                                                     \
    if (g > (uint64_t)sm_count() * 8) g = (uint64_t)sm_count() * 8;                                                      \
    k_r2s_km_warp<WW><<<(unsigned)g, kKmWarps * 32, smem, st>>>(recs, NW, kb, cur, n_next, nxt, d_cnt, seg_cap,           \
                                                              bnd.as<u32>(), d_todo);                                    \
  }
      MHB_FOR_RW(M)
#undef M
    } else {
#define M(WW)                                                                                                         \
  if (RW == WW)                                                                                                       \
    k_r2s_kmsort_level<WW><<<(unsigned)((n_next + 127) / 128), 128, 0, st>>>(recs, NW, kb, cur, nullptr, n_next, nxt, \
                                                                            d_cnt, seg_cap, bnd.as<u32>());
      MHB_FOR_RW(M)
#undef M
    }
    CK_LAUNCH();
  }
#define M(WW) \
  if (RW == WW) k_r2s_kmsort_finish<WW><<<grid_for(n, 256, 32), 256, 0, st>>>(recs, n, NW, bnd.as<u32>(), d_todo);
  MHB_FOR_RW(M)
#undef M
  CK_LAUNCH();
  tr.mark("s1.kmsort.finish");
#define M(WW)                                                                                                          \
  if (RW == WW)                                                                                                        \
    k_r2s_s1_post<WW><<<grid_for(n, 256, 32), 256, 0, st>>>(recs, n, NW, k, m, pv, out, need_mercy ? 1 : 0, d_mul_hist);
  MHB_FOR_RW(M)
#undef M
  CK_LAUNCH();
  tr.mark("s1.post");
  CK(cudaStreamSynchronize(st));
  return MHB_OK;
}

struct S2Bufs {
  DevBuf tile_heads, tile_off, bsum, heads, scr, bytes;
};

int s2_sort_emit(cudaStream_t st, uint32_t k, BigBufs &big, S2Bufs &sb, uint64_t n, u64 *d_table, u64 *d_totals,
                 unsigned long long *d_counter, PhaseTrace &tr, uint64_t *n_u_out, uint64_t *cap_bytes) {
  const uint32_t W = s2s_record_words(k), WPT = words_per_tip_label(k);
  DevBuf &a = big.a, &b = big.b, &ws = big.ws;
  const size_t ws_bytes = mhb_sort_workspace_bytes(n, W);
  uint8_t sbytes[80];
  const uint32_t n_sb = mhb_s2s_sort_bytes(k, sbytes);
  int in_b = 0;
  CKR(mhb_sort_records_relaxed(st, a.as<u32>(), b.as<u32>(), n, W, sbytes, n_sb, nullptr, ws.p, ws_bytes, &in_b));
  tr.mark("s2.sort");
  const u32 *sorted = in_b ? b.as<u32>() : a.as<u32>();
  u32 *uniq = in_b ? a.as<u32>() : b.as<u32>();
  const uint64_t n_tiles = (n + kDdTile - 1) / kDdTile;
  CKR(sb.tile_heads.ensure(n_tiles * 4, "tile counts"));
  CKR(sb.tile_off.ensure(n_tiles * 8, "tile offsets"));
  CKR(sb.bsum.ensure((n_tiles / 4096 + 4) * 8, "scan sums"));
#define M(WW) \
  if (W == WW) k_r2s_dd_count<WW><<<(unsigned)n_tiles, kDdThreads, 0, st>>>(sorted, n, sb.tile_heads.as<u32>());
  MHB_FOR_WR(M)
#undef M
  CK_LAUNCH();
  CKR(scan32(st, sb.tile_heads.as<u32>(), n_tiles, sb.tile_off.as<u64>(), (uint64_t *)(d_counter + 2), sb.bsum.as<u64>()));
  unsigned long long n_u = 0;
  CK(cudaMemcpyAsync(&n_u, d_counter + 2, 8, cudaMemcpyDeviceToHost, st));
  CK(cudaStreamSynchronize(st));
  CKR(sb.heads.ensure((size_t)n_u * 8, "run heads"));
#define M(WW)                                                                                                             \
  if (W == WW)                                                                                                            \
    k_r2s_dd_heads<WW><<<(unsigned)n_tiles, kDdThreads, 0, st>>>(sorted, n, sb.tile_off.as<u64>(), sb.heads.as<u64>());
  MHB_FOR_WR(M)
#undef M
  CK_LAUNCH();
#define M(WW) \
  if (W == WW) k_r2s_dd_build<WW><<<grid_for(n_u, 256), 256, 0, st>>>(sorted, n, sb.heads.as<u64>(), n_u, uniq);
  MHB_FOR_WR(M)
#undef M
  CK_LAUNCH();
  tr.mark("s2.collapse");
  const size_t scr_bytes = mhb_s2s_emit_scratch_bytes(n_u, k);
  *cap_bytes = (uint64_t)n_u * (4ull + 4ull * WPT) + 16;
  CKR(sb.scr.ensure(scr_bytes, "emit scratch"));
  CKR(sb.bytes.ensure(*cap_bytes, "SdBG stream"));
  CKR(mhb_s2s_emit_fmt(st, uniq, n_u, k, sb.bytes.as<uint8_t>(), *cap_bytes, d_table, d_totals, sb.scr.p, scr_bytes, 1));
  *n_u_out = n_u;
  return MHB_OK;
}

}

extern "C" int mhb_set_r2s_round_limit(uint64_t max_s1_records, uint64_t max_s2_items) {
  g_r2s_s1_limit = max_s1_records;
  g_r2s_s2_limit = max_s2_items;
  return MHB_OK;
}

extern "C" int mhb_read2sdbg_host(const mhb_build_args *args, mhb_build_result *res) {
  if (!args || !res) return mhb_set_error(MHB_ERR_ARG, "null argument");
  memset(res, 0, sizeof(*res));
  const uint32_t k = args->k;
  const int32_t m = args->m;
  if (k < 9 || k > MHB_MAX_K || m < 1) return mhb_set_error(MHB_ERR_ARG, "read2sdbg: need 9 <= k <= 255 and m >= 1");
  if (mhb_device_count() <= 0) return mhb_set_error(MHB_ERR_CUDA, "no CUDA device: libmhb has no CPU path");
  cudaStream_t st = 0;
  PhaseTrace tr;
  tr.mark("start");
  PkgIndex ix;
  CKR(index_pkg(args->bin, args->bin_words, args->n_reads, k, &ix));
  const uint32_t W = s2s_record_words(k), WPT = words_per_tip_label(k);
  res->words_per_tip_label = WPT;
  res->n_edge_records = ix.n_edges;
  res->bucket_table = (uint64_t *)calloc((size_t)MHB_NUM_BUCKETS * 4, 8);
  res->counting = (int64_t *)calloc(65536, 8);
  struct ResGuard {
    mhb_build_result *r;
    const uint8_t *caller_buf;
    bool ok = false;
    ~ResGuard() {
      if (ok) return;
      free(r->bucket_table);
      free(r->counting);
      if (r->bytes != caller_buf) free(r->bytes);
      r->bucket_table = nullptr;
      r->counting = nullptr;
      r->bytes = nullptr;
    }
  } guard{res, args->sdbg_out};
  if (!res->bucket_table || !res->counting) return mhb_set_error(MHB_ERR_NOMEM, "host malloc failed");

  const uint32_t RW = r2s_s1_key_words(k) + 2;
  const bool s1_runs = m > 1 && ix.n_s1 > 0;
  const bool mercy = args->need_mercy && m > 1;
  const uint64_t bit_words = ix.n_bases / 32 + 2;
  const size_t resident = pad((size_t)ix.n_words * 4 + 64) +
                          (ix.fixed_len ? 0 : 5 * pad((ix.n_reads + 1) * 8) + pad(ix.n_reads * 4)) + pad(bit_words * 4) +
                          (mercy ? pad(bit_words * 16) : 0) + pad(65536 * 8) + pad(64) + pad((size_t)MHB_NUM_BUCKETS * 32) +
                          pad(128);
  const size_t upload_bytes = pad((size_t)args->bin_words * 4 + 64) + (ix.fixed_len ? 0 : pad((ix.n_reads + 1) * 8));
  const uint64_t est_items = (uint64_t)(2.2 * (double)ix.n_edges) + 1024;
  const size_t s1_one = s1_runs ? s1_pass_bytes(ix.n_s1, RW) : 0;
  const size_t s2_est = ix.n_edges ? s2_pass_bytes(est_items, W, k) : 0;
  if (mhb_arena_bytes() &&
      (double)(resident + std::max({upload_bytes, s1_one, s2_est})) > 0.92 * (double)free_device_bytes())
    mhb_release();
  if (resident + upload_bytes > free_device_bytes())
    return mhb_set_error(MHB_ERR_NOMEM, "read2sdbg: the read library alone needs %zu bytes of device memory, %zu are free",
                         resident + upload_bytes, free_device_bytes());

  DevBuf d_pkg, d_word_off, d_len, d_base_off, d_s1_off, d_edge_off;
  PkgView pv;
  memset(&pv, 0, sizeof(pv));
  pv.n_reads = ix.n_reads;
  pv.fixed_len = ix.fixed_len;
  pv.fixed_words = ix.fixed_words;
  CKR(d_pkg.alloc((size_t)ix.n_words * 4 + 64, "package"));
  if (ix.n_reads) {
    DevBuf d_bin, d_rec_off;
    CKR(d_bin.alloc((size_t)args->bin_words * 4 + 64, ".bin image"));
    CK(cudaMemcpyAsync(d_bin.p, args->bin, (size_t)args->bin_words * 4, cudaMemcpyHostToDevice, st));
    if (!ix.fixed_len) {
      CKR(upload(d_rec_off, ix.rec_off, "record offsets"));
      CKR(upload(d_word_off, ix.word_off, "word offsets"));
      CKR(upload(d_len, ix.len, "lengths"));
      CKR(upload(d_base_off, ix.base_off, "base offsets"));
      CKR(upload(d_s1_off, ix.s1_off, "stage-1 offsets"));
      CKR(upload(d_edge_off, ix.edge_off, "edge offsets"));
      pv.word_off = d_word_off.as<u64>();
      pv.len = d_len.as<u32>();
      pv.base_off = d_base_off.as<u64>();
      pv.s1_off = d_s1_off.as<u64>();
      pv.edge_off = d_edge_off.as<u64>();
    }
    if (ix.n_words) {
      k_r2s_reverse<<<grid_for(ix.n_words, 256), 256, 0, st>>>(d_bin.as<u32>(), ix.n_reads, ix.fixed_len, d_rec_off.as<u64>(), pv,
                                                                d_pkg.as<u32>(), ix.n_words);
      CK_LAUNCH();
    }
    CK(cudaStreamSynchronize(st));
  }
  pv.words = d_pkg.as<u32>();
  tr.mark("h2d.upload+reverse");

  DevBuf d_solid, d_planes, d_hist, d_cnt;
  CKR(d_solid.alloc(bit_words * 4, "solid marker"));
  CK(cudaMemsetAsync(d_solid.p, 0, bit_words * 4, st));
  CKR(d_hist.alloc(65536 * 8, "multiplicity histogram"));
  CK(cudaMemsetAsync(d_hist.p, 0, 65536 * 8, st));
  CKR(d_cnt.alloc(64, "counters"));
  CK(cudaMemsetAsync(d_cnt.p, 0, 64, st));
  unsigned long long *d_counter = d_cnt.as<unsigned long long>();
  DevBuf d_table, d_totals;
  CKR(d_table.alloc((size_t)MHB_NUM_BUCKETS * 32, "bucket table"));
  CKR(d_totals.alloc(16 * 8, "totals"));
  BigBufs big;
  if (s1_runs) {
    S1Out so;
    memset(&so, 0, sizeof(so));
    so.is_solid = d_solid.as<u32>();
    if (mercy) {
      CKR(d_planes.alloc(bit_words * 4 * 4, "mercy candidate planes"));
      CK(cudaMemsetAsync(d_planes.p, 0, bit_words * 4 * 4, st));
      so.no_in = d_planes.as<u32>();
      so.no_out = so.no_in + bit_words;
      so.any = so.no_out + bit_words;
    }
    const size_t avail = (size_t)(0.92 * (double)free_device_bytes());
    uint64_t max_n = g_r2s_s1_limit;
    const bool rounds = (max_n && ix.n_s1 > max_n) || s1_one > avail;
    if (!rounds) {
      const size_t rec1 = pad((size_t)ix.n_s1 * RW * 4 + 16), ws1 = pad(mhb_sort_workspace_bytes(ix.n_s1, RW));
      const size_t rec2 = pad((size_t)est_items * W * 4 + 16), ws2 = pad(mhb_sort_workspace_bytes(est_items, W));
      const bool share = s1_one - 2 * rec1 - ws1 + 2 * std::max(rec1, rec2) + std::max(ws1, ws2) <= avail;
      CKR(run_stage1(st, pv, ix, k, m, mercy, so, d_hist.as<unsigned long long>(), tr, big,
                     share ? (size_t)est_items * W * 4 + 16 : 0, share ? mhb_sort_workspace_bytes(est_items, W) : 0));
      res->n_rounds_s1 = 1;
    } else {
      if (!max_n) {
        const size_t fixed = pad(ix.n_reads * 4) + pad((ix.n_reads + 1) * 8) + pad((ix.n_reads / 4096 + 4) * 8) +
                             pad(MHB_NUM_BUCKETS * 8) + 256;
        max_n = largest_round(ix.n_s1, fixed, avail, [&](uint64_t n) { return s1_pass_bytes(n, RW); });
        if (!max_n)
          return mhb_set_error(MHB_ERR_NOMEM, "read2sdbg: the resident read library leaves no room for a stage-1 round "
                               "(%zu bytes free)", avail);
      }
      max_n = std::min(max_n, ix.n_s1);
      CKR(run_stage1_rounds(st, pv, ix, k, m, mercy, so, d_hist.as<unsigned long long>(), tr, big, max_n,
                            &res->n_rounds_s1));
    }
    if (mercy) {
      u32 *d_mercy = so.any + bit_words;
      k_r2s_mercy<<<grid_for(ix.n_reads, 256), 256, 0, st>>>(pv, k, so, d_mercy, d_counter + 1);
      CK_LAUNCH();
      k_r2s_or_words<<<grid_for(bit_words, 256), 256, 0, st>>>(d_solid.as<u32>(), d_mercy, bit_words);
      CK_LAUNCH();
      unsigned long long nm = 0;
      CK(cudaMemcpyAsync(&nm, d_counter + 1, 8, cudaMemcpyDeviceToHost, st));
      CK(cudaStreamSynchronize(st));
      res->n_mercy = nm;
      tr.mark("s1.mercy");
    }
    CK(cudaMemcpyAsync(res->counting, d_hist.p, 65536 * 8, cudaMemcpyDeviceToHost, st));
    CK(cudaStreamSynchronize(st));
    d_planes.release();
  }

  uint64_t n_items = 0;
  if (ix.n_edges) {
    CK(cudaMemsetAsync(d_counter, 0, 8, st));
#define M(WW)                                                                                                             \
  if (W == WW)                                                                                                            \
    k_r2s_s2_extract<WW, kS2Count><<<grid_for(ix.n_edges, 256), 256, 0, st>>>(pv, k, d_solid.as<u32>(), m == 1, ix.n_edges, \
                                                                             nullptr, d_counter, 0);
    MHB_FOR_WR(M)
#undef M
    CK_LAUNCH();
    unsigned long long c = 0;
    CK(cudaMemcpyAsync(&c, d_counter, 8, cudaMemcpyDeviceToHost, st));
    CK(cudaStreamSynchronize(st));
    n_items = c;
    tr.mark("s2.count");
  }
  res->n_sort_items = n_items;
  uint64_t max_items = g_r2s_s2_limit;
  bool s2_rounds = false;
  if (n_items) {
    const size_t held = big.a.bytes + big.b.bytes + big.ws.bytes;
    s2_rounds = (max_items && n_items > max_items) ||
                (double)s2_pass_bytes(n_items, W, k) > 0.92 * (double)(free_device_bytes() + held);
  }
  if (n_items == 0) {
    res->bytes = args->sdbg_out ? args->sdbg_out : (uint8_t *)malloc(1);
  } else if (!s2_rounds) {
    S2Bufs sb;
    DevBuf &a = big.a, &b = big.b, &ws = big.ws;
    const size_t rec_bytes = (size_t)n_items * W * 4 + 16, ws_bytes = mhb_sort_workspace_bytes(n_items, W);
    CKR(a.ensure(rec_bytes, "stage-2 items"));
    CKR(b.ensure(rec_bytes, "stage-2 items (sort buffer)"));
    CKR(ws.ensure(ws_bytes, "sort workspace"));
    CK(cudaMemsetAsync(d_counter, 0, 8, st));
#define M(WW)                                                                                                             \
  if (W == WW)                                                                                                            \
    k_r2s_s2_extract<WW, kS2Write><<<grid_for(ix.n_edges, 256), 256, 0, st>>>(pv, k, d_solid.as<u32>(), m == 1, ix.n_edges, \
                                                                             a.as<u32>(), d_counter, n_items);
    MHB_FOR_WR(M)
#undef M
    CK_LAUNCH();
    tr.mark("s2.extract");
    uint64_t n_u = 0, cap_bytes = 0;
    CKR(s2_sort_emit(st, k, big, sb, n_items, d_table.as<u64>(), d_totals.as<u64>(), d_counter, tr, &n_u, &cap_bytes));
    uint64_t totals[16];
    CK(cudaMemcpyAsync(totals, d_totals.p, sizeof(totals), cudaMemcpyDeviceToHost, st));
    CK(cudaStreamSynchronize(st));
    tr.mark("s2.emit");
    res->n_bytes = totals[0];
    res->n_items = totals[1];
    res->n_tips = totals[2];
    res->n_large_mul = totals[3];
    for (int i = 0; i < 9; ++i) res->w_count[i] = totals[4 + i];
    res->ones_in_last = totals[13];
    if (res->n_bytes > cap_bytes) return mhb_set_error(MHB_ERR_NOMEM, "internal: SdBG byte stream exceeds capacity");
    if (args->sdbg_out && args->sdbg_out_capacity >= res->n_bytes) res->bytes = args->sdbg_out;
    else res->bytes = (uint8_t *)malloc(std::max<size_t>(1, res->n_bytes));
    if (!res->bytes) return mhb_set_error(MHB_ERR_NOMEM, "host malloc failed");
    CK(cudaMemcpyAsync(res->bucket_table, d_table.p, (size_t)MHB_NUM_BUCKETS * 32, cudaMemcpyDeviceToHost, st));
    if (res->n_bytes) CK(cudaMemcpyAsync(res->bytes, sb.bytes.p, res->n_bytes, cudaMemcpyDeviceToHost, st));
    CK(cudaStreamSynchronize(st));
    tr.mark("d2h");
    res->n_solid = n_u;
    res->n_rounds_s2 = 1;
  } else {
    big.a.release();
    big.b.release();
    big.ws.release();
    DevBuf h16;
    CKR(h16.alloc(MHB_NUM_BUCKETS * 8, "bucket histogram"));
    if (!max_items) {
      const size_t avail = (size_t)(0.92 * (double)free_device_bytes());
      max_items = largest_round(n_items, 0, avail, [&](uint64_t n) { return s2_pass_bytes(n, W, k); });
      if (!max_items)
        return mhb_set_error(MHB_ERR_NOMEM, "read2sdbg: the resident read library leaves no room for a stage-2 round "
                             "(%zu bytes free)", avail);
    }
    max_items = std::min(max_items, n_items);
    CK(cudaMemsetAsync(h16.p, 0, MHB_NUM_BUCKETS * 8, st));
#define M(WW)                                                                                                            \
  if (W == WW)                                                                                                           \
    k_r2s_s2_extract<WW, kS2Hist><<<grid_for(ix.n_edges, 256), 256, 0, st>>>(pv, k, d_solid.as<u32>(), m == 1, ix.n_edges, \
                                                                            nullptr, nullptr, 0, 0, 65535,            \
                                                                            h16.as<unsigned long long>());
    MHB_FOR_WR(M)
#undef M
    CK_LAUNCH();
    std::vector<uint64_t> h_h16(MHB_NUM_BUCKETS);
    CK(cudaMemcpyAsync(h_h16.data(), h16.p, MHB_NUM_BUCKETS * 8, cudaMemcpyDeviceToHost, st));
    CK(cudaStreamSynchronize(st));
    tr.mark("s2.extract.plan");
    std::vector<std::pair<uint32_t, uint32_t>> ranges;
    CKR(plan_bucket_ranges(h_h16, max_items, &ranges));
    CKR(big.a.ensure((size_t)max_items * W * 4 + 16, "stage-2 items"));
    CKR(big.b.ensure((size_t)max_items * W * 4 + 16, "stage-2 items (sort buffer)"));
    CKR(big.ws.ensure(mhb_sort_workspace_bytes(max_items, W), "sort workspace"));
    S2Bufs sb;
    SdbgStitch out;
    uint64_t seen = 0;
    for (const auto &rg : ranges) {
      CK(cudaMemsetAsync(d_counter, 0, 8, st));
#define M(WW)                                                                                                             \
  if (W == WW)                                                                                                            \
    k_r2s_s2_extract<WW, kS2Range><<<grid_for(ix.n_edges, 256), 256, 0, st>>>(pv, k, d_solid.as<u32>(), m == 1, ix.n_edges, \
                                                                             big.a.as<u32>(), d_counter, max_items,    \
                                                                             rg.first, rg.second, nullptr);
      MHB_FOR_WR(M)
#undef M
      CK_LAUNCH();
      unsigned long long n = 0;
      CK(cudaMemcpyAsync(&n, d_counter, 8, cudaMemcpyDeviceToHost, st));
      CK(cudaStreamSynchronize(st));
      tr.mark("s2.extract");
      if (n > max_items)
        return mhb_set_error(MHB_ERR_CUDA, "read2sdbg: internal: round of %llu stage-2 items exceeds its plan (%llu)",
                             (unsigned long long)n, (unsigned long long)max_items);
      seen += n;
      if (n == 0) continue;
      uint64_t n_u = 0, cap_bytes = 0;
      CKR(s2_sort_emit(st, k, big, sb, n, d_table.as<u64>(), d_totals.as<u64>(), d_counter, tr, &n_u, &cap_bytes));
      tr.mark("s2.emit");
      CKR(out.append(st, sb.bytes.as<uint8_t>(), cap_bytes, d_table.as<u64>(), d_totals.as<u64>()));
      tr.mark("d2h");
      res->n_solid += n_u;
      ++res->n_rounds_s2;
    }
    if (seen != n_items)
      return mhb_set_error(MHB_ERR_CUDA, "read2sdbg: internal: the rounds saw %llu of %llu stage-2 items",
                           (unsigned long long)seen, (unsigned long long)n_items);
    res->n_bytes = out.tot[0];
    res->n_items = out.tot[1];
    res->n_tips = out.tot[2];
    res->n_large_mul = out.tot[3];
    for (int i = 0; i < 9; ++i) res->w_count[i] = out.tot[4 + i];
    res->ones_in_last = out.tot[13];
    memcpy(res->bucket_table, out.table.data(), (size_t)MHB_NUM_BUCKETS * 32);
    if (args->sdbg_out && args->sdbg_out_capacity >= res->n_bytes) res->bytes = args->sdbg_out;
    else res->bytes = (uint8_t *)malloc(std::max<size_t>(1, res->n_bytes));
    if (!res->bytes) return mhb_set_error(MHB_ERR_NOMEM, "host malloc failed");
    if (res->n_bytes) memcpy(res->bytes, out.bytes.data(), res->n_bytes);
  }
  tr.mark("release");
  CK(cudaStreamSynchronize(st));
  res->t_h2d_ms = tr.sum("h2d");
  res->t_count_ms = tr.sum("s1.extract") + tr.sum("s1.partition");
  res->t_mercy_ms = tr.sum("s1.kmsort");
  res->t_s2s_ms = tr.sum("s2");
  res->t_d2h_ms = tr.sum("d2h");
  res->t_total_ms = tr.sum("");
  tr.report();
  guard.ok = true;
  return MHB_OK;
}

extern "C" int mhb_selftest_r2s_s1_record(const uint32_t *pkg_words, uint32_t nwords, uint32_t L, uint32_t k, uint32_t e,
                                          uint64_t base_off, uint32_t *rec_out) {
  if (k < 9 || k > MHB_MAX_K || L < k + 1 || e >= L - k + 4) return mhb_set_error(MHB_ERR_ARG, "bad args");
  const uint32_t NW = r2s_s1_key_words(k);
  u32 p, want;
  s1_emission(L, k, e, p, want);
#define M(WW)                                                       \
  if (NW == WW) {                                                   \
    u32 rec[WW + 2];                                                \
    make_s1_record<WW>(pkg_words, nwords, L, k, p, want, base_off, rec); \
    memcpy(rec_out, rec, sizeof(rec));                              \
  }
  MHB_FOR_W(M)
#undef M
  return MHB_OK;
}

extern "C" int mhb_selftest_r2s_item(const uint32_t *pkg_words, uint32_t nwords, uint32_t L, uint32_t k, uint32_t i,
                                     uint32_t strand, uint32_t type, uint32_t *rec_out, uint32_t *palindrome_out) {
  if (k < 9 || k > MHB_MAX_K || i + k >= L || strand > 1 || type > 2) return mhb_set_error(MHB_ERR_ARG, "bad args");
  const uint32_t W = s2s_record_words(k);
#define M(WW)                                                              \
  if (W == WW) {                                                           \
    u32 rec[WW];                                                           \
    make_r2s_item<WW>(pkg_words, nwords, k, i, strand, type, rec);         \
// ... 161 lines not shown
```

### megahit_b200/csrc/mhb_sortdisp.cu

```cuda
#include <cuda_runtime.h>
#include <stdio.h>
#include <stdlib.h>
#include <string.h>

#include "mhb.h"
#include "mhb_common.cuh"
#include "mhb_kernels.cuh"
#include "mhb_sort.cuh"
#include "mhb_sort3.cuh"
#include "mhb_part.cuh"

using namespace mhb;

#define MHB_V3_DEFAULT 0x180
#define MHB_V3_LIST(X) X(0x180) X(0x080) X(0x000) X(0x1080) X(0x082)
static bool v3_listed(int bits) {
#define X(B) \
  if (bits == B) return true;
  MHB_V3_LIST(X)
#undef X
  return false;
}
static int g_sort_cfg = -1;
extern "C" int mhb_set_sort_cfg(int cfg) {
// ... 103 lines not shown
    k_radix_pass3<WR, CFG, false, false><<<(int)grid, C::THREADS, C::SMEM, st>>>(in, n, (u32)tiles, byte_idx, bin_base, lookback,
                                                                                  tile_counter, nullptr, 0, epoch);
  CK_LAUNCH();
  return MHB_OK;
}

template <int WR>
static int launch_part_unstable(cudaStream_t st, const u32 *in, u64 n, int byte_idx, const u64 *bin_base,
                                unsigned long long *gcursor, u32 *tile_counter, u64 *next_hist, int next_byte,
                                const uint8_t *lut) {
  using C = PartCfg<WR>;
  static int bps = 0;
  if (!bps) {
    CK(cudaFuncSetAttribute(k_part_unstable<WR, false, true>, cudaFuncAttributeMaxDynamicSharedMemorySize, (int)C::SMEM));
    CK(cudaFuncSetAttribute(k_part_unstable<WR, false, false>, cudaFuncAttributeMaxDynamicSharedMemorySize, (int)C::SMEM));
    CK(cudaFuncSetAttribute(k_part_unstable<WR, true, false>, cudaFuncAttributeMaxDynamicSharedMemorySize, (int)C::SMEM));
    CK(cudaFuncSetAttribute(k_part_unstable<WR, true, true>, cudaFuncAttributeMaxDynamicSharedMemorySize, (int)C::SMEM_OWNER_HIST));
    CK(cudaOccupancyMaxActiveBlocksPerMultiprocessor(&bps, k_part_unstable<WR, false, true>, C::THREADS, C::SMEM));
    if (bps < 1) return mhb_set_error(MHB_ERR_CUDA, "partition pass (WR=%d) does not fit an SM", WR);
    if (getenv("MHB_VERBOSE")) fprintf(stderr, "[mhb] unstable partition pass WR=%d: %d threads x %d rec, %zu B smem, %d CTA/SM\n", WR, C::THREADS, C::IPT, C::SMEM, bps);
  }
  const u64 tiles = (n + C::TILE - 1) / C::TILE;
  u64 grid = (u64)bps * sm_count();
  if (grid > tiles) grid = tiles;
  if (lut && next_hist)
    k_part_unstable<WR, true, true><<<(int)grid, C::THREADS, C::SMEM_OWNER_HIST, st>>>(in, n, (u32)tiles, byte_idx, bin_base, gcursor,
                                                                                       tile_counter, next_hist, next_byte, lut);
  else if (lut)
    k_part_unstable<WR, true, false><<<(int)grid, C::THREADS, C::SMEM, st>>>(in, n, (u32)tiles, byte_idx, bin_base, gcursor,
                                                                             tile_counter, nullptr, 0, lut);
  else if (next_hist)
    k_part_unstable<WR, false, true><<<(int)grid, C::THREADS, C::SMEM, st>>>(in, n, (u32)tiles, byte_idx, bin_base, gcursor,
                                                                             tile_counter, next_hist, next_byte, nullptr);
  else
    k_part_unstable<WR, false, false><<<(int)grid, C::THREADS, C::SMEM, st>>>(in, n, (u32)tiles, byte_idx, bin_base, gcursor,
                                                                              tile_counter, nullptr, 0, nullptr);
  CK_LAUNCH();
  return MHB_OK;
}

template <int WR>
static int launch_radix_pass(cudaStream_t st, const u32 *in, u64 n, int byte_idx, const u64 *bin_base,
                             u64 *lookback, u32 *tile_counter, u64 *next_hist, int next_byte, u32 epoch) {
  const int cfg = sort_cfg();
  if (cfg >= 256) {
    if constexpr (WR == 2 || WR == 3) {
#define X(B) \
  if (cfg - 256 == B) return launch_radix_pass_cfg3<WR, B>(st, in, n, byte_idx, bin_base, lookback, tile_counter, next_hist, next_byte, epoch);
      MHB_V3_LIST(X)
#undef X
    }
    return launch_radix_pass_cfg3<WR, MHB_V3_DEFAULT>(st, in, n, byte_idx, bin_base, lookback, tile_counter, next_hist, next_byte, epoch);
  }
  if constexpr (WR <= 3) {
    switch (cfg) {
      case 1: return launch_radix_pass_cfg<WR, 1>(st, in, n, byte_idx, bin_base, lookback, tile_counter, next_hist, next_byte, epoch);
      case 2: return launch_radix_pass_cfg<WR, 2>(st, in, n, byte_idx, bin_base, lookback, tile_counter, next_hist, next_byte, epoch);
      case 3: return launch_radix_pass_cfg<WR, 3>(st, in, n, byte_idx, bin_base, lookback, tile_counter, next_hist, next_byte, epoch);
      default: break;
    }
  }
  return launch_radix_pass_cfg<WR, 0>(st, in, n, byte_idx, bin_base, lookback, tile_counter, next_hist, next_byte, epoch);
}

#ifdef MHB_SORT_TIMELINE
extern "C" int mhb_debug_set_sort_timeline(unsigned long long *dev_buf, unsigned long long rows) {
  CK(cudaMemcpyToSymbol(g_sort_timeline, &dev_buf, sizeof(dev_buf)));
  CK(cudaMemcpyToSymbol(g_sort_timeline_rows, &rows, sizeof(rows)));
  return MHB_OK;
}
#endif

namespace {
struct SortTrace {
  cudaEvent_t ev[74];
  bool created = false;
  uint32_t n_passes = 0, words = 0;
  uint64_t n = 0;
};
SortTrace g_trace[4];
uint64_t g_trace_seq = 0;
}

int mhb_sort_records_ex(void *stream, uint32_t *a, uint32_t *b, uint64_t n, uint32_t words, const uint8_t *bytes,
                        uint32_t n_bytes, const uint64_t *first_hist, void *ws, size_t ws_bytes, int *result_in_b,
                        double *pass_ms_host, int relaxed);
int mhb_sort_records_impl(void *stream, uint32_t *a, uint32_t *b, uint64_t n, uint32_t words, const uint8_t *bytes,
                          uint32_t n_bytes, const uint64_t *first_hist, void *ws, size_t ws_bytes, int *result_in_b,
                          double *pass_ms_host) {
  return mhb_sort_records_ex(stream, a, b, n, words, bytes, n_bytes, first_hist, ws, ws_bytes, result_in_b, pass_ms_host, 1);
}
int mhb_sort_records_ex(void *stream, uint32_t *a, uint32_t *b, uint64_t n, uint32_t words, const uint8_t *bytes,
                          uint32_t n_bytes, const uint64_t *first_hist, void *ws, size_t ws_bytes, int *result_in_b,
                        double *pass_ms_host, int relaxed) {
  static const bool stable_first = getenv("MHB_SORT_STABLE_FIRST") != nullptr;
  if (stable_first) relaxed = 0;
  if (words < 1 || words > 17 || n_bytes > 72 || !result_in_b)
    return mhb_set_error(MHB_ERR_ARG, "bad sort geometry (words=%u n_bytes=%u)", words, n_bytes);
  *result_in_b = 0;
  if (n == 0 || n_bytes == 0) return MHB_OK;
  if (ws_bytes < mhb_sort_workspace_bytes(n, words)) return mhb_set_error(MHB_ERR_ARG, "sort workspace too small");
  if (n >= (1ull << 53)) return mhb_set_error(MHB_ERR_ARG, "too many records");
  cudaStream_t st = (cudaStream_t)stream;
  u64 *hist = (u64 *)ws;
  u64 *bin_base = hist + (72 + 1) * 256;
  u32 *tile_counter = (u32 *)(bin_base + 256);
  unsigned long long *gcursor = (unsigned long long *)(tile_counter + 128);
  u64 *lookback = (u64 *)((char *)ws + kSortHeadBytes);
  CK(cudaMemsetAsync(ws, 0, kSortHeadBytes + lb_bytes(sort_num_tiles(n, words)) + 256, st));
  if (first_hist) {
    CK(cudaMemcpyAsync(hist, first_hist, 256 * 8, cudaMemcpyDeviceToDevice, st));
  } else {
#define M(WW) \
  if (words == WW) k_hist_byte<WW><<<sm_count() * 4, 256, 0, st>>>(a, n, bytes[0], hist);
    MHB_FOR_WR(M)
#undef M
    CK_LAUNCH();
  }
  SortTrace &tr = g_trace[g_trace_seq++ & 3];
  if (!tr.created) {
    for (int i = 0; i < 74; ++i) CK(cudaEventCreate(&tr.ev[i]));
    tr.created = true;
  }
  tr.n_passes = n_bytes;
  tr.words = words;
  tr.n = n;
  CK(cudaEventRecord(tr.ev[0], st));
  u32 *in = a, *out = b;
  for (u32 p = 0; p < n_bytes; ++p) {
    k_hist_scan256<<<1, 256, 0, st>>>(hist + (u64)p * 256, bin_base, (u64)(uintptr_t)out, words * 4);
    CK_LAUNCH();
    u64 *next_hist = p + 1 < n_bytes ? hist + (u64)(p + 1) * 256 : nullptr;
    const int next_byte = p + 1 < n_bytes ? bytes[p + 1] : 0;
    int rc = MHB_ERR_ARG;
    if (p == 0 && relaxed && words == 2) rc = launch_part_unstable<2>(st, in, n, bytes[p], bin_base, gcursor, tile_counter + p, next_hist, next_byte, nullptr);
    else if (p == 0 && relaxed && words == 3) rc = launch_part_unstable<3>(st, in, n, bytes[p], bin_base, gcursor, tile_counter + p, next_hist, next_byte, nullptr);
    else {
#define M(WW) \
  if (words == WW) rc = launch_radix_pass<WW>(st, in, n, bytes[p], bin_base, lookback, tile_counter + p, next_hist, next_byte, p + 1);
      MHB_FOR_WR(M)
#undef M
    }
    if (rc) return rc;
    CK(cudaEventRecord(tr.ev[p + 1], st));
    u32 *t = in;
    in = out;
    out = t;
  }
  *result_in_b = (in == b) ? 1 : 0;
  if (pass_ms_host) {
    CK(cudaEventSynchronize(tr.ev[n_bytes]));
    for (u32 p = 0; p < n_bytes; ++p) {
      float ms = 0;
      CK(cudaEventElapsedTime(&ms, tr.ev[p], tr.ev[p + 1]));
      pass_ms_host[p] = ms;
    }
  }
  return MHB_OK;
}

template <int WR>
static int launch_partition_pass(cudaStream_t st, const u32 *in, u64 n, int byte_idx, const u64 *bin_addr, u64 *lookback,
                                 u32 *tile_counter, const uint8_t *lut) {
  using C = SortCfg<WR, 0>;
  static int blocks_per_sm = 0;
  if (!blocks_per_sm) {
    CK(cudaFuncSetAttribute(k_radix_pass<WR, 0, true>, cudaFuncAttributeMaxDynamicSharedMemorySize, (int)C::SMEM));
    CK(cudaOccupancyMaxActiveBlocksPerMultiprocessor(&blocks_per_sm, k_radix_pass<WR, 0, true>, C::THREADS, C::SMEM));
    if (blocks_per_sm < 1) return mhb_set_error(MHB_ERR_CUDA, "partition pass kernel (WR=%d) does not fit an SM", WR);
  }
  const u64 tiles = sort_tiles_cfg<WR, 0>(n);
  u64 grid = (u64)blocks_per_sm * sm_count();
  if (grid > tiles) grid = tiles;
  k_radix_pass<WR, 0, true><<<(int)grid, C::THREADS, C::SMEM, st>>>(in, n, (u32)tiles, byte_idx, bin_addr, lookback,
                                                                     tile_counter, nullptr, 0, 1, lut);
  CK_LAUNCH();
  return MHB_OK;
}

static int partition_scatter_impl(void *stream, const uint32_t *recs, uint64_t n, uint32_t words, int byte,
                                  const uint8_t *owner_of_byte_dev, const uint64_t *bin_addr_dev, void *ws, size_t ws_bytes,
                                  int next_byte, uint64_t *owner_next_hist, int *hist_done);
extern "C" int mhb_partition_scatter(void *stream, const uint32_t *recs, uint64_t n, uint32_t words, int byte,
                                     const uint8_t *owner_of_byte_dev, const uint64_t *bin_addr_dev, void *ws,
                                     size_t ws_bytes) {
  return partition_scatter_impl(stream, recs, n, words, byte, owner_of_byte_dev, bin_addr_dev, ws, ws_bytes, 0, nullptr, nullptr);
}
extern "C" int mhb_partition_scatter_hist(void *stream, const uint32_t *recs, uint64_t n, uint32_t words, int byte,
                                          const uint8_t *owner_of_byte_dev, const uint64_t *bin_addr_dev, void *ws,
                                          size_t ws_bytes, int next_byte, uint64_t *owner_next_hist, int *hist_done) {
  if (!owner_of_byte_dev || !owner_next_hist || !hist_done || next_byte < 0 || next_byte >= (int)(4 * words))
    return mhb_set_error(MHB_ERR_ARG, "bad owner-histogram arguments");
  return partition_scatter_impl(stream, recs, n, words, byte, owner_of_byte_dev, bin_addr_dev, ws, ws_bytes, next_byte,
                                owner_next_hist, hist_done);
}
static int partition_scatter_impl(void *stream, const uint32_t *recs, uint64_t n, uint32_t words, int byte,
                                  const uint8_t *owner_of_byte_dev, const uint64_t *bin_addr_dev, void *ws, size_t ws_bytes,
                                  int next_byte, uint64_t *owner_next_hist, int *hist_done) {
  if (hist_done) *hist_done = 0;
  if (words < 1 || words > 17 || byte < 0 || byte >= (int)(4 * words)) return mhb_set_error(MHB_ERR_ARG, "bad geometry");
  if (n == 0) return MHB_OK;
  u64 tiles = 0;
#define M(WW) \
  if (words == WW) tiles = sort_tiles_cfg<WW, 0>(n);
  MHB_FOR_WR(M)
#undef M
  const size_t need = kSortHeadBytes + (size_t)tiles * 256 * 8 + 256;
  if (ws_bytes < need) return mhb_set_error(MHB_ERR_ARG, "sort workspace too small");
  cudaStream_t st = (cudaStream_t)stream;
  u64 *hist = (u64 *)ws;
  u32 *tile_counter = (u32 *)(hist + (72 + 1) * 256 + 256);
  u64 *lookback = (u64 *)((char *)ws + kSortHeadBytes);
  CK(cudaMemsetAsync(ws, 0, need, st));
  int rc = MHB_ERR_ARG;
  static const bool stable_first = getenv("MHB_SORT_STABLE_FIRST") != nullptr;
  if (owner_of_byte_dev && !stable_first && (words == 2 || words == 3)) {
    unsigned long long *gcursor = (unsigned long long *)(tile_counter + 128);
    rc = words == 2 ? launch_part_unstable<2>(st, recs, n, byte, bin_addr_dev, gcursor, tile_counter, owner_next_hist, next_byte, owner_of_byte_dev)
                    : launch_part_unstable<3>(st, recs, n, byte, bin_addr_dev, gcursor, tile_counter, owner_next_hist, next_byte, owner_of_byte_dev);
    if (!rc && owner_next_hist && hist_done) *hist_done = 1;
  } else if (owner_of_byte_dev) {
#define M(WW) \
  if (words == WW) rc = launch_partition_pass<WW>(st, recs, n, byte, bin_addr_dev, lookback, tile_counter, owner_of_byte_dev);
    MHB_FOR_WR(M)
#undef M
  } else {
#define M(WW) \
  if (words == WW) rc = launch_radix_pass_cfg<WW, 0>(st, recs, n, byte, bin_addr_dev, lookback, tile_counter, nullptr, 0, 1);
    MHB_FOR_WR(M)
#undef M
  }
  return rc;
}

extern "C" int mhb_dev_malloc(void **ptr, size_t bytes) {
  CK(cudaMalloc(ptr, bytes));
  return MHB_OK;
// ... 52 lines not shown
```

### megahit_b200/dev.py

```python
from __future__ import annotations

import ctypes as C
import os

import numpy as np
import torch

from . import lib


def _ptr(t):
    return C.c_void_p(t.data_ptr()) if t is not None else None


def _stream():
    return C.c_void_p(torch.cuda.current_stream().cuda_stream)


def sort_records(a: torch.Tensor, b: torch.Tensor, n: int, words: int, sort_bytes, first_hist=None, ws=None, relaxed=False):
    L = lib.load()
    need = L.mhb_sort_workspace_bytes(n, words)
    if ws is None or ws.numel() < need:
        ws = torch.empty(need, dtype=torch.uint8, device=a.device)
    bytes_arr = (C.c_uint8 * len(sort_bytes))(*sort_bytes)
    in_b = C.c_int(0)
    fn = L.mhb_sort_records_relaxed if relaxed else L.mhb_sort_records
    lib._check(fn(_stream(), _ptr(a), _ptr(b), n, words, bytes_arr, len(sort_bytes), _ptr(first_hist), _ptr(ws), ws.numel(),
                  C.byref(in_b)))
    return b if in_b.value else a


class CountPlan:

    def __init__(self, n_reads: int, read_len: int, k: int, m: int, device, want_mercy: bool = True, mode: str | None = None):
        import os
        L = lib.load()
        self.L, self.k, self.m, self.n_reads, self.read_len, self.device = L, k, m, n_reads, read_len, device
        self.want_mercy = want_mercy
        mode = mode or os.environ.get("MHB_COUNT_MODE") or "auto"
        ok = bool(L.mhb_count_hashed_supported(k, m))
        if mode == "hashed" and not ok:
            raise lib.MhbError(f"hashed count is not available for k={k}, m={m}")
        self.hashed = ok and mode in ("hashed", "auto")
        self.n = n_reads * (read_len - k) if read_len >= k + 1 else 0
        self.WR, self.WE = lib.count_record_words(k), lib.words_per_edge(k)
        self.sort_bytes = lib.count_sort_bytes(k)
        n = self.n
        i32 = dict(dtype=torch.int32, device=device)
        self.a = torch.empty(n * self.WR + 4, **i32)
        self.b = torch.empty(n * self.WR + 4, **i32)
        if self.hashed:
            self.ws = torch.empty(L.mhb_count_hashed_workspace_bytes(n, k, m), dtype=torch.uint8, device=device)
            self.scratch = None
        else:
            self.ws = torch.empty(L.mhb_sort_workspace_bytes(n, self.WR), dtype=torch.uint8, device=device)
            self.scratch = torch.empty(L.mhb_count_solid_scratch_bytes(n), dtype=torch.uint8, device=device)
        self.cap_edges = n // max(1, m) + 1
        self.edges = torch.empty(self.cap_edges * self.WE, **i32)
        self.aux = torch.empty(self.cap_edges, dtype=torch.uint8, device=device)
        self.mul_hist = torch.zeros(65536, dtype=torch.int64, device=device)
        self.hist0 = torch.zeros(256, dtype=torch.int64, device=device)
        self.n_solid_dev = torch.zeros(8, dtype=torch.int64, device=device)
        self.first = torch.empty(n_reads + 1, **i32) if want_mercy else None
        self.last = torch.empty(n_reads + 1, **i32) if want_mercy else None
        self.tipset = None
        self.events = {}

    def _reads(self, bin_dev: torch.Tensor) -> lib.DevReads:
        return lib.DevReads(bin_dev.data_ptr(), bin_dev.numel(), self.n_reads, self.read_len, None, None)

    def _mark(self, name):
        ev = torch.cuda.Event(enable_timing=True)
        ev.record()
        self.events.setdefault(name, []).append(ev)

    def extract(self, bin_dev):
        self.hist0.zero_()
        lib._check(self.L.mhb_count_extract(_stream(), C.byref(self._reads(bin_dev)), self.k, _ptr(self.a), self.n,
                                            _ptr(self.hist0), 5 if self.hashed else self.sort_bytes[0]))

    def sort(self):
        if self.hashed:
            return None
        self.sorted = sort_records(self.a, self.b, self.n, self.WR, self.sort_bytes, self.hist0, self.ws, relaxed=True)
        return self.sorted

    def count(self):
        self.mul_hist.zero_()
        self.n_solid_dev.zero_()
        if self.hashed:
            lib._check(self.L.mhb_count_solid_hashed(_stream(), _ptr(self.a), _ptr(self.b), self.n, self.k, self.m,
                                                     _ptr(self.hist0), _ptr(self.edges), _ptr(self.aux), self.cap_edges,
                                                     _ptr(self.mul_hist), _ptr(self.n_solid_dev), _ptr(self.ws), self.ws.numel()))
            return
        lib._check(self.L.mhb_count_solid(_stream(), _ptr(self.sorted), self.n, self.k, self.m, _ptr(self.edges),
                                          _ptr(self.aux), self.cap_edges, _ptr(self.mul_hist), _ptr(self.n_solid_dev),
                                          _ptr(self.scratch), self.scratch.numel()))

    def mercy(self, bin_dev):
        n_solid = int(self.n_solid_dev[0].item())
        n_tip = C.c_uint64(0)
        lib._check(self.L.mhb_count_tip_edges(_stream(), _ptr(self.aux), n_solid, C.byref(n_tip)))
        need = self.L.mhb_tipset_bytes(n_tip.value, self.k)
        if self.tipset is None or self.tipset.numel() < need:
            self.tipset = torch.empty(need, dtype=torch.uint8, device=self.device)
        lib._check(self.L.mhb_tipset_build(_stream(), _ptr(self.edges), _ptr(self.aux), n_solid, self.k,
                                           _ptr(self.tipset), need, n_tip.value))
        lib._check(self.L.mhb_count_mark_mercy(_stream(), C.byref(self._reads(bin_dev)), self.k, _ptr(self.tipset),
                                               need, n_tip.value, _ptr(self.first), _ptr(self.last)))
        return n_solid, n_tip.value

    def mercy_edges(self, bin_dev: torch.Tensor, n_solid: int) -> int:
        L = self.L
        if not hasattr(self, "cand"):
            self.cand = torch.empty(self.n_reads + 1, dtype=torch.int64, device=self.device)
            self.cand_scratch = torch.empty(L.mhb_mercy_candidates_scratch_bytes(self.n_reads), dtype=torch.uint8, device=self.device)
            self.mercy_scratch = None
        nc = C.c_uint64(0)
        lib._check(L.mhb_mercy_candidates(_stream(), _ptr(self.first), _ptr(self.last), self.n_reads, _ptr(self.cand), C.byref(nc),
                                          _ptr(self.cand_scratch), self.cand_scratch.numel()))
        self.n_cand = nc.value
        if not self.n_cand:
            return 0
        need = L.mhb_mercy_edges_scratch_bytes(self.n_cand, self.read_len)
        if self.mercy_scratch is None or self.mercy_scratch.numel() < need:
            self.mercy_scratch = torch.empty(int(need * 1.2), dtype=torch.uint8, device=self.device)
        nm = C.c_uint64(0)
        lib._check(L.mhb_mercy_edges(_stream(), C.byref(self._reads(bin_dev)), _ptr(self.cand), self.n_cand, self.read_len, self.k,
                                     _ptr(self.edges), n_solid, C.c_void_p(self.edges.data_ptr() + n_solid * self.WE * 4),
                                     self.cap_edges - n_solid, C.byref(nm), _ptr(self.mercy_scratch), self.mercy_scratch.numel()))
        return nm.value

    def run(self, bin_dev: torch.Tensor, timed: bool = False):
        if timed:
            self._mark("t0")
        self.extract(bin_dev)
        if timed:
            self._mark("extract")
        self.sort()
        if timed:
            self._mark("sort")
        self.count()
        if timed:
            self._mark("count")
        if self.want_mercy:
            n_solid, _ = self.mercy(bin_dev)
        else:
            n_solid = int(self.n_solid_dev[0].item())
        if timed:
            self._mark("mercy")
        return n_solid

    def edges_host(self, n_solid: int) -> np.ndarray:
        return self.edges[: n_solid * self.WE].cpu().numpy().view(np.uint32).reshape(-1, self.WE)


class S2sPlan:

    def __init__(self, n_seqs: int, seq_len: int, k: int, device):
        L = lib.load()
        self.L, self.k, self.n_seqs, self.seq_len, self.device = L, k, n_seqs, seq_len, device
        self.W = lib.s2s_record_words(k)
        self.sort_bytes = lib.s2s_sort_bytes(k)
        self.n_items = n_seqs * 2 * (seq_len - k + 2)
        n = self.n_items
        i32 = dict(dtype=torch.int32, device=device)
        self.a = torch.empty(n * self.W + 4, **i32)
        self.b = torch.empty(n * self.W + 4, **i32)
        self.ws = torch.empty(L.mhb_sort_workspace_bytes(n, self.W), dtype=torch.uint8, device=device)
        self.scratch = torch.empty(L.mhb_s2s_emit_scratch_bytes(n, k), dtype=torch.uint8, device=device)
        wpt = (k + 15) // 16
        self.cap_bytes = n * (4 + 4 * wpt) + 16
        self.bytes = torch.empty(self.cap_bytes, dtype=torch.uint8, device=device)
        self.table = torch.zeros(65536 * 4, dtype=torch.int64, device=device)
        self.totals = torch.zeros(16, dtype=torch.int64, device=device)
        self.hist0 = torch.zeros(256, dtype=torch.int64, device=device)
        self.cursor = torch.zeros(1, dtype=torch.int64, device=device)
        self.events = []

    def run(self, words: torch.Tensor, mult: torch.Tensor | None = None, n_seqs: int | None = None, stride: int = 0,
            timed: bool = False, aux: torch.Tensor | None = None, n_aux: int = 0):
        n_seqs = self.n_seqs if n_seqs is None else n_seqs
        assert n_seqs <= self.n_seqs
        self.n_items = n_seqs * 2 * (self.seq_len - self.k + 2)
        if aux is not None and mult is None and not os.environ.get("MHB_S2S_NO_PRUNE"):
            return self._run_pruned(words, n_seqs, aux, n_aux, timed)
        seqs = lib.DevSeqs(words.data_ptr(), words.numel(), n_seqs, self.seq_len, None, None, None,
                           mult.data_ptr() if mult is not None else None, stride)
        self.hist0.zero_()
        ev = [torch.cuda.Event(enable_timing=True) for _ in range(4)] if timed else None
        if timed:
            ev[0].record()
        lib._check(self.L.mhb_s2s_extract(_stream(), C.byref(seqs), self.k, _ptr(self.a), self.n_items, _ptr(self.hist0),
                                          self.sort_bytes[0]))
        if timed:
            ev[1].record()
        srt = sort_records(self.a, self.b, self.n_items, self.W, self.sort_bytes, self.hist0, self.ws, relaxed=True)
        if timed:
            ev[2].record()
        lib._check(self.L.mhb_s2s_emit(_stream(), _ptr(srt), self.n_items, self.k, _ptr(self.bytes), self.cap_bytes,
                                       _ptr(self.table), _ptr(self.totals), _ptr(self.scratch), self.scratch.numel()))
        if timed:
            ev[3].record()
            self.events.append(ev)
        return self.totals

    def _run_pruned(self, edges: torch.Tensor, n_edges: int, aux: torch.Tensor, n_aux: int, timed: bool):
        cap = self.n_items
        self.hist0.zero_()
        self.cursor.zero_()
        ev = [torch.cuda.Event(enable_timing=True) for _ in range(4)] if timed else None
        if timed:
            ev[0].record()
        lib._check(self.L.mhb_s2s_extract_edges_pruned(_stream(), _ptr(edges), _ptr(aux), n_edges, n_aux, self.k, _ptr(self.a),
                                                       cap, _ptr(self.cursor), _ptr(self.hist0), self.sort_bytes[0]))
        self.n_items = int(self.cursor.item())
        assert self.n_items <= cap
        if timed:
            ev[1].record()
        srt = sort_records(self.a, self.b, self.n_items, self.W, self.sort_bytes, self.hist0, self.ws, relaxed=True)
        if timed:
            ev[2].record()
        lib._check(self.L.mhb_s2s_emit(_stream(), _ptr(srt), self.n_items, self.k, _ptr(self.bytes), self.cap_bytes,
                                       _ptr(self.table), _ptr(self.totals), _ptr(self.scratch), self.scratch.numel()))
        if timed:
            ev[3].record()
            self.events.append(ev)
        return self.totals
```

### megahit_b200/lib.py

```python
from __future__ import annotations

import ctypes as C
import os

import numpy as np

_HERE = os.path.dirname(os.path.abspath(__file__))
LIB_PATH = os.environ.get("MHB_LIB") or os.path.join(_HERE, "libmhb.so")
NUM_BUCKETS = 65536
SENTINEL_OFFSET = 0xFFFFFFFF

_lib = None


class MhbError(RuntimeError):
    pass


class DevReads(C.Structure):
    _fields_ = [("bin", C.c_void_p), ("bin_words", C.c_uint64), ("n_reads", C.c_uint64), ("fixed_len", C.c_uint32),
                ("rec_off", C.c_void_p), ("edge_off", C.c_void_p)]


class DevSeqs(C.Structure):
# ... 29 lines not shown
                ("t_total_ms", C.c_double), ("t_extract_ms", C.c_double), ("t_sort_ms", C.c_double),
                ("t_emit_ms", C.c_double)]


class BuildArgs(C.Structure):
    _fields_ = [("k", C.c_uint32), ("m", C.c_int32), ("bin", C.c_void_p), ("bin_words", C.c_uint64),
                ("n_reads", C.c_uint64), ("need_mercy", C.c_int32), ("want_edges", C.c_int32),
                ("sdbg_out", C.c_void_p), ("sdbg_out_capacity", C.c_uint64)]


class BuildResult(C.Structure):
    _fields_ = [("n_edge_records", C.c_uint64), ("n_solid", C.c_uint64), ("n_cand", C.c_uint64), ("n_mercy", C.c_uint64),
                ("n_sort_items", C.c_uint64), ("words_per_edge", C.c_uint32), ("words_per_tip_label", C.c_uint32),
                ("n_items", C.c_uint64), ("n_tips", C.c_uint64), ("n_large_mul", C.c_uint64), ("n_bytes", C.c_uint64),
                ("bytes", C.POINTER(C.c_uint8)), ("bucket_table", C.POINTER(C.c_uint64)), ("w_count", C.c_uint64 * 9),
                ("ones_in_last", C.c_uint64), ("edges", C.POINTER(C.c_uint32)), ("cand_ids", C.POINTER(C.c_uint64)),
                ("counting", C.POINTER(C.c_int64)),
                ("t_total_ms", C.c_double), ("t_h2d_ms", C.c_double), ("t_count_ms", C.c_double),
                ("t_mercy_ms", C.c_double), ("t_s2s_ms", C.c_double), ("t_d2h_ms", C.c_double),
                ("n_rounds_s1", C.c_uint32), ("n_rounds_s2", C.c_uint32)]


class CountOpts(C.Structure):
    _fields_ = [("k", C.c_uint32), ("m", C.c_int32), ("host_mem", C.c_double), ("num_cpu_threads", C.c_int32),
                ("read_lib_file", C.c_char_p), ("output_prefix", C.c_char_p), ("mem_flag", C.c_int32)]


class Seq2SdbgOpts(C.Structure):
    _fields_ = [("host_mem", C.c_double), ("k", C.c_uint32), ("k_from", C.c_uint32), ("num_cpu_threads", C.c_int32),
                ("contig", C.c_char_p), ("bubble", C.c_char_p), ("addi_contig", C.c_char_p),
                ("local_contig", C.c_char_p), ("input_prefix", C.c_char_p), ("output_prefix", C.c_char_p),
                ("need_mercy", C.c_int32), ("mem_flag", C.c_int32)]


class Read2SdbgOpts(C.Structure):
    _fields_ = [("k", C.c_uint32), ("m", C.c_int32), ("host_mem", C.c_double), ("num_cpu_threads", C.c_int32),
                ("read_lib_file", C.c_char_p), ("output_prefix", C.c_char_p), ("mem_flag", C.c_int32),
                ("need_mercy", C.c_int32)]


class IterateArgs(C.Structure):
    _fields_ = [("k", C.c_uint32), ("step", C.c_uint32), ("contig_words", C.c_void_p), ("contig_word_off", C.c_void_p),
                ("contig_len", C.c_void_p), ("n_contigs", C.c_uint64), ("bin", C.c_void_p), ("bin_words", C.c_uint64),
                ("n_reads", C.c_uint64)]


class IterateResult(C.Structure):
    _fields_ = [("n_flanks", C.c_uint64), ("n_aligned_reads", C.c_uint64), ("n_candidates", C.c_uint64), ("n_edges", C.c_uint64),
                ("words_per_edge", C.c_uint32), ("edges", C.POINTER(C.c_uint32)), ("t_total_ms", C.c_double)]


class IterateOpts(C.Structure):
    _fields_ = [("contig_file", C.c_char_p), ("bubble_file", C.c_char_p), ("read_file", C.c_char_p),
                ("num_cpu_threads", C.c_int32), ("k", C.c_uint32), ("step", C.c_uint32), ("output_prefix", C.c_char_p)]


class BuildlibLib(C.Structure):
    _fields_ = [("type", C.c_char_p), ("data", C.c_void_p * 2), ("size", C.c_uint64 * 2)]


class BuildlibArgs(C.Structure):
    _fields_ = [("libs", C.POINTER(BuildlibLib)), ("n_libs", C.c_uint32)]


class BuildlibResult(C.Structure):
    _fields_ = [("bin", C.POINTER(C.c_uint32)), ("bin_words", C.c_uint64), ("n_reads", C.c_uint64), ("n_bases", C.c_uint64),
                ("n_libs", C.c_uint32), ("lib_begin", C.POINTER(C.c_uint64)), ("lib_end", C.POINTER(C.c_uint64)),
                ("lib_max_len", C.POINTER(C.c_uint32)), ("n_chunks", C.c_uint64), ("n_walk_passes", C.c_uint64),
                ("t_total_ms", C.c_double)]


SYMBOLS = [
    "mhb_last_error", "mhb_version", "mhb_device_count", "mhb_launch_count", "mhb_count_record_words", "mhb_words_per_edge",
    "mhb_s2s_record_words", "mhb_count_sort_bytes", "mhb_s2s_sort_bytes", "mhb_sort_workspace_bytes",
    "mhb_count_extract", "mhb_check_fixed_len", "mhb_count_extract_range", "mhb_set_round_limit", "mhb_set_s2s_round_limit", "mhb_set_r2s_round_limit", "mhb_plan_rounds", "mhb_plan_rounds16", "mhb_sort_records", "mhb_sort_records_relaxed", "mhb_sort_pass_ms", "mhb_set_sort_cfg", "mhb_partition_scatter", "mhb_partition_scatter_hist", "mhb_plan_partition", "mhb_compact_tip_edges", "mhb_dev_malloc", "mhb_dev_free",
    "mhb_ipc_export", "mhb_ipc_open", "mhb_ipc_close", "mhb_count_solid_scratch_bytes", "mhb_count_solid", "mhb_count_hashed_supported", "mhb_count_hashed_workspace_bytes", "mhb_count_solid_hashed", "mhb_tipset_bytes",
    "mhb_tipset_build", "mhb_count_mark_mercy", "mhb_count_tip_edges", "mhb_s2s_extract", "mhb_s2s_extract_range",
    "mhb_s2s_emit_scratch_bytes", "mhb_s2s_emit", "mhb_set_device", "mhb_count_host", "mhb_s2s_host", "mhb_build_host", "mhb_free",
    "mhb_mercy_candidates_scratch_bytes", "mhb_mercy_candidates", "mhb_mercy_edges_scratch_bytes", "mhb_mercy_edges", "mhb_mercy_edges_count", "mhb_mercy_edges_write", "mhb_mercy_edges_segs", "mhb_mercy_host", "mhb_mercy_planes_words", "mhb_mercy_probe_owned", "mhb_mercy_count_planes", "mhb_edge_lut_bytes", "mhb_edge_lut_build",
    "mhb_release", "mhb_count_run", "mhb_count_run_multi", "mhb_seq2sdbg_run", "mhb_selftest_count_record", "mhb_selftest_count_records_roll", "mhb_selftest_s2s_record",
    "mhb_iterate_host", "mhb_iterate_run", "mhb_selftest_iterate", "mhb_s2s_extract_edges_pruned", "mhb_s2s_emit_fmt", "mhb_read2sdbg_host", "mhb_read2sdbg_run", "mhb_selftest_r2s_s1_record", "mhb_selftest_r2s_item",
    "mhb_selftest_kmsort", "mhb_selftest_kmsort_smem", "mhb_selftest_r2s_s1_group", "mhb_selftest_r2s_mercy_read",
    "mhb_buildlib_host", "mhb_buildlib_free", "mhb_set_buildlib_chunk", "mhb_buildlib_run", "mhb_selftest_fastx",
]


def load():
    global _lib
    if _lib is not None:
        return _lib
    if not os.path.exists(LIB_PATH):
        raise MhbError(f"{LIB_PATH} is missing: build it with `make -C megahit_b200/csrc` "
                       "(there is no CPU fallback for the CUDA path)")
    L = C.CDLL(LIB_PATH)
    L.mhb_last_error.restype = C.c_char_p
    L.mhb_version.restype = C.c_char_p
    for f in ("mhb_count_record_words", "mhb_words_per_edge", "mhb_s2s_record_words", "mhb_count_sort_bytes",
              "mhb_s2s_sort_bytes"):
        getattr(L, f).restype = C.c_uint32
    for f in ("mhb_sort_workspace_bytes", "mhb_count_solid_scratch_bytes", "mhb_tipset_bytes",
              "mhb_s2s_emit_scratch_bytes"):
        getattr(L, f).restype = C.c_size_t
    L.mhb_sort_workspace_bytes.argtypes = [C.c_uint64, C.c_uint32]
    L.mhb_count_solid_scratch_bytes.argtypes = [C.c_uint64]
    L.mhb_tipset_bytes.argtypes = [C.c_uint64, C.c_uint32]
    L.mhb_s2s_emit_scratch_bytes.argtypes = [C.c_uint64, C.c_uint32]
    L.mhb_count_extract.argtypes = [C.c_void_p, C.POINTER(DevReads), C.c_uint32, C.c_void_p, C.c_uint64, C.c_void_p,
                                    C.c_int]
    L.mhb_sort_records.argtypes = [C.c_void_p, C.c_void_p, C.c_void_p, C.c_uint64, C.c_uint32, C.c_void_p, C.c_uint32,
                                   C.c_void_p, C.c_void_p, C.c_size_t, C.POINTER(C.c_int)]
    L.mhb_sort_records_relaxed.argtypes = L.mhb_sort_records.argtypes
    L.mhb_count_solid.argtypes = [C.c_void_p, C.c_void_p, C.c_uint64, C.c_uint32, C.c_int32, C.c_void_p, C.c_void_p,
                                  C.c_uint64, C.c_void_p, C.c_void_p, C.c_void_p, C.c_size_t]
    L.mhb_count_hashed_workspace_bytes.restype = C.c_size_t
    L.mhb_count_hashed_workspace_bytes.argtypes = [C.c_uint64, C.c_uint32, C.c_int32]
    L.mhb_count_hashed_supported.argtypes = [C.c_uint32, C.c_int32]
    L.mhb_count_solid_hashed.argtypes = [C.c_void_p, C.c_void_p, C.c_void_p, C.c_uint64, C.c_uint32, C.c_int32, C.c_void_p,
                                         C.c_void_p, C.c_void_p, C.c_uint64, C.c_void_p, C.c_void_p, C.c_void_p, C.c_size_t]
    L.mhb_tipset_build.argtypes = [C.c_void_p, C.c_void_p, C.c_void_p, C.c_uint64, C.c_uint32, C.c_void_p, C.c_size_t,
                                   C.c_uint64]
    L.mhb_count_mark_mercy.argtypes = [C.c_void_p, C.POINTER(DevReads), C.c_uint32, C.c_void_p, C.c_size_t, C.c_uint64,
                                       C.c_void_p, C.c_void_p]
    L.mhb_count_tip_edges.argtypes = [C.c_void_p, C.c_void_p, C.c_uint64, C.POINTER(C.c_uint64)]
    L.mhb_s2s_extract.argtypes = [C.c_void_p, C.POINTER(DevSeqs), C.c_uint32, C.c_void_p, C.c_uint64, C.c_void_p,
                                  C.c_int]
    L.mhb_s2s_emit.argtypes = [C.c_void_p, C.c_void_p, C.c_uint64, C.c_uint32, C.c_void_p, C.c_uint64, C.c_void_p,
                               C.c_void_p, C.c_void_p, C.c_size_t]
    L.mhb_count_host.argtypes = [C.POINTER(CountArgs), C.POINTER(CountResult)]
    L.mhb_s2s_host.argtypes = [C.POINTER(S2sArgs), C.POINTER(S2sResult)]
    L.mhb_build_host.argtypes = [C.POINTER(BuildArgs), C.POINTER(BuildResult)]
    L.mhb_mercy_candidates_scratch_bytes.restype = C.c_size_t
    L.mhb_mercy_candidates_scratch_bytes.argtypes = [C.c_uint64]
    L.mhb_mercy_edges_scratch_bytes.restype = C.c_size_t
    L.mhb_mercy_edges_scratch_bytes.argtypes = [C.c_uint64, C.c_uint32]
    L.mhb_mercy_candidates.argtypes = [C.c_void_p, C.c_void_p, C.c_void_p, C.c_uint64, C.c_void_p, C.POINTER(C.c_uint64),
                                       C.c_void_p, C.c_size_t]
    L.mhb_mercy_edges.argtypes = [C.c_void_p, C.POINTER(DevReads), C.c_void_p, C.c_uint64, C.c_uint32, C.c_uint32,
                                  C.c_void_p, C.c_uint64, C.c_void_p, C.c_uint64, C.POINTER(C.c_uint64), C.c_void_p,
                                  C.c_size_t]
    L.mhb_mercy_edges_segs.argtypes = [C.c_void_p, C.POINTER(DevReads), C.c_void_p, C.c_uint64, C.c_uint32, C.c_uint32,
                                       C.c_uint32, C.c_void_p, C.c_void_p, C.c_void_p, C.c_void_p, C.c_void_p, C.c_uint64,
                                       C.POINTER(C.c_uint64), C.c_void_p, C.c_size_t]
    L.mhb_mercy_edges_count.argtypes = [C.c_void_p, C.POINTER(DevReads), C.c_void_p, C.c_uint64, C.c_uint32, C.c_uint32,
                                        C.c_uint32, C.c_void_p, C.c_void_p, C.c_void_p, C.c_void_p, C.POINTER(C.c_uint64),
                                        C.c_void_p, C.c_size_t]
    L.mhb_mercy_edges_write.argtypes = [C.c_void_p, C.POINTER(DevReads), C.c_void_p, C.c_uint64, C.c_uint32, C.c_uint32,
                                        C.c_void_p, C.c_uint64, C.c_uint64, C.c_void_p, C.c_size_t]
    L.mhb_mercy_planes_words.restype = C.c_size_t
    L.mhb_mercy_planes_words.argtypes = [C.c_uint64, C.c_uint32]
    L.mhb_mercy_probe_owned.argtypes = [C.c_void_p, C.POINTER(DevReads), C.c_void_p, C.c_uint64, C.c_uint32, C.c_uint32,
                                        C.c_void_p, C.c_uint64, C.c_void_p, C.c_void_p, C.c_uint32, C.c_void_p]
    L.mhb_mercy_count_planes.argtypes = [C.c_void_p, C.POINTER(DevReads), C.c_void_p, C.c_uint64, C.c_uint32, C.c_uint32,
                                         C.c_void_p, C.c_uint32, C.c_uint64, C.POINTER(C.c_uint64), C.c_void_p, C.c_size_t]
    L.mhb_plan_partition.argtypes = [C.c_void_p, C.c_void_p, C.c_uint32, C.c_uint32, C.c_uint32, C.c_void_p, C.c_void_p,
                                     C.c_void_p, C.c_void_p]
    L.mhb_edge_lut_bytes.restype = C.c_size_t
    L.mhb_edge_lut_build.argtypes = [C.c_void_p, C.c_void_p, C.c_uint64, C.c_uint32, C.c_void_p]
    L.mhb_sort_pass_ms.argtypes = [C.c_int, C.c_void_p, C.c_uint32, C.POINTER(C.c_uint32), C.POINTER(C.c_uint64),
                                   C.POINTER(C.c_uint32)]
    L.mhb_set_device.argtypes = [C.c_int]
    L.mhb_partition_scatter.argtypes = [C.c_void_p, C.c_void_p, C.c_uint64, C.c_uint32, C.c_int, C.c_void_p, C.c_void_p,
                                        C.c_void_p, C.c_size_t]
    L.mhb_partition_scatter_hist.argtypes = [C.c_void_p, C.c_void_p, C.c_uint64, C.c_uint32, C.c_int, C.c_void_p, C.c_void_p,
                                             C.c_void_p, C.c_size_t, C.c_int, C.c_void_p, C.POINTER(C.c_int)]
    L.mhb_dev_malloc.argtypes = [C.POINTER(C.c_void_p), C.c_size_t]
    L.mhb_dev_free.argtypes = [C.c_void_p]
    L.mhb_ipc_export.argtypes = [C.c_void_p, C.c_void_p]
    L.mhb_ipc_open.argtypes = [C.c_void_p, C.POINTER(C.c_void_p)]
    L.mhb_ipc_close.argtypes = [C.c_void_p]
    L.mhb_free.argtypes = [C.c_void_p]
    L.mhb_count_run.argtypes = [C.POINTER(CountOpts)]
    L.mhb_seq2sdbg_run.argtypes = [C.POINTER(Seq2SdbgOpts)]
    L.mhb_selftest_count_record.argtypes = [C.c_void_p, C.c_uint32, C.c_uint32, C.c_uint32, C.c_uint32, C.c_void_p,
                                            C.POINTER(C.c_uint32)]
    L.mhb_selftest_count_records_roll.argtypes = [C.c_void_p, C.c_uint32, C.c_uint32, C.c_uint32, C.c_uint32, C.c_void_p,
                                                  C.c_void_p]
    L.mhb_selftest_s2s_record.argtypes = [C.c_void_p, C.c_uint32, C.c_uint32, C.c_uint32, C.c_uint32, C.c_uint32,
                                          C.c_uint32, C.c_void_p]
    L.mhb_s2s_emit_fmt.argtypes = L.mhb_s2s_emit.argtypes + [C.c_int]
    L.mhb_iterate_host.argtypes = [C.POINTER(IterateArgs), C.POINTER(IterateResult)]
    L.mhb_selftest_iterate.argtypes = [C.POINTER(IterateArgs), C.POINTER(IterateResult)]
    L.mhb_iterate_run.argtypes = [C.POINTER(IterateOpts)]
    L.mhb_s2s_extract_edges_pruned.argtypes = [C.c_void_p, C.c_void_p, C.c_void_p, C.c_uint64, C.c_uint64, C.c_uint32,
                                               C.c_void_p, C.c_uint64, C.c_void_p, C.c_void_p, C.c_int]
    L.mhb_read2sdbg_host.argtypes = [C.POINTER(BuildArgs), C.POINTER(BuildResult)]
    L.mhb_read2sdbg_run.argtypes = [C.POINTER(Read2SdbgOpts)]
    L.mhb_selftest_r2s_s1_record.argtypes = [C.c_void_p, C.c_uint32, C.c_uint32, C.c_uint32, C.c_uint32, C.c_uint64, C.c_void_p]
    L.mhb_selftest_r2s_item.argtypes = [C.c_void_p, C.c_uint32, C.c_uint32, C.c_uint32, C.c_uint32, C.c_uint32, C.c_uint32,
                                        C.c_void_p, C.POINTER(C.c_uint32)]
    L.mhb_selftest_kmsort.argtypes = [C.c_void_p, C.c_uint64, C.c_uint32]
    L.mhb_selftest_kmsort_smem.argtypes = [C.c_void_p, C.c_uint64, C.c_uint32, C.c_uint32, C.c_uint32]
    L.mhb_selftest_r2s_s1_group.argtypes = [C.c_void_p, C.c_uint64, C.c_uint32, C.c_int32, C.c_uint32, C.c_uint64, C.c_int,
                                            C.c_void_p, C.c_void_p, C.c_void_p, C.c_void_p, C.c_void_p]
    L.mhb_selftest_r2s_mercy_read.argtypes = [C.c_uint32, C.c_uint64, C.c_uint64, C.c_uint32, C.c_void_p, C.c_void_p, C.c_void_p,
# ... 32 lines not shown
    L.mhb_plan_rounds.argtypes = [C.c_void_p, C.c_uint64, C.c_void_p, C.c_void_p]
    n = L.mhb_plan_rounds(h.ctypes.data, int(max_records), lo, hi)
    if n < 0:
        raise MhbError(L.mhb_last_error().decode())
    return [(int(lo[i]), int(hi[i])) for i in range(n)]


def plan_rounds16(hist256, sub_hist, max_records: int, cap: int = 65536):
    L = load()
    h = np.ascontiguousarray(hist256, dtype=np.uint64)
    sub = None if sub_hist is None else np.ascontiguousarray(sub_hist, dtype=np.uint64).reshape(256, 256)
    lo, hi = (C.c_uint32 * cap)(), (C.c_uint32 * cap)()
    L.mhb_plan_rounds16.argtypes = [C.c_void_p, C.c_void_p, C.c_uint64, C.c_void_p, C.c_void_p, C.c_uint32]
    n = L.mhb_plan_rounds16(h.ctypes.data, sub.ctypes.data if sub is not None else None, int(max_records), lo, hi, cap)
    if n < 0:
        raise MhbError(L.mhb_last_error().decode())
    return [(int(lo[i]), int(hi[i])) for i in range(n)]


def set_round_limit(max_records: int = 0):
    L = load()
    L.mhb_set_round_limit.argtypes = [C.c_uint64]
    _check(L.mhb_set_round_limit(int(max_records)))


def set_s2s_round_limit(max_items: int = 0):
    L = load()
    L.mhb_set_s2s_round_limit.argtypes = [C.c_uint64]
    _check(L.mhb_set_s2s_round_limit(int(max_items)))


def set_r2s_round_limit(s1: int = 0, s2: int = 0):
    L = load()
    L.mhb_set_r2s_round_limit.argtypes = [C.c_uint64, C.c_uint64]
    _check(L.mhb_set_r2s_round_limit(int(s1), int(s2)))


def mercy_host(k: int, edges: np.ndarray, cand_bin: np.ndarray) -> np.ndarray:
    L = load()
    we = words_per_edge(k)
    edges = np.ascontiguousarray(edges, np.uint32).reshape(-1, we)
    cand = np.ascontiguousarray(cand_bin, np.uint32).reshape(-1)
    out, nm, nr = C.POINTER(C.c_uint32)(), C.c_uint64(), C.c_uint64()
    L.mhb_mercy_host.argtypes = [C.c_uint32, C.c_void_p, C.c_uint64, C.c_void_p, C.c_uint64, C.POINTER(C.POINTER(C.c_uint32)),
                                 C.POINTER(C.c_uint64), C.POINTER(C.c_uint64)]
    _check(L.mhb_mercy_host(k, edges.ctypes.data if len(edges) else None, len(edges), cand.ctypes.data if len(cand) else None,
                            len(cand), C.byref(out), C.byref(nm), C.byref(nr)))
    res = np.ctypeslib.as_array(out, (max(nm.value, 1) * we,))[: nm.value * we].reshape(-1, we).copy()
    L.mhb_free(out)
    return res


def sort_pass_ms(back: int = 0):
    buf = (C.c_double * 80)()
    npass, nrec, words = C.c_uint32(), C.c_uint64(), C.c_uint32()
    _check(load().mhb_sort_pass_ms(back, buf, 80, C.byref(npass), C.byref(nrec), C.byref(words)))
    return list(buf[: npass.value]), nrec.value, words.value


def count_record_words(k: int) -> int:
    return load().mhb_count_record_words(C.c_uint32(k))


def words_per_edge(k: int) -> int:
    return load().mhb_words_per_edge(C.c_uint32(k))


def s2s_record_words(k: int) -> int:
    return load().mhb_s2s_record_words(C.c_uint32(k))


def count_sort_bytes(k: int) -> list[int]:
    buf = (C.c_uint8 * 80)()
    n = load().mhb_count_sort_bytes(C.c_uint32(k), buf)
    return list(buf[:n])


def s2s_sort_bytes(k: int) -> list[int]:
    buf = (C.c_uint8 * 80)()
    n = load().mhb_s2s_sort_bytes(C.c_uint32(k), buf)
    return list(buf[:n])


def count_host(bin_words: np.ndarray, n_reads: int, k: int, m: int, want_mercy: bool = True) -> dict:
    L = load()
    bin_words = np.ascontiguousarray(bin_words, dtype=np.uint32).reshape(-1)
    a = CountArgs(k, m, bin_words.ctypes.data if len(bin_words) else None, len(bin_words), n_reads, int(want_mercy))
    r = CountResult()
    _check(L.mhb_count_host(C.byref(a), C.byref(r)))
    wpe = r.words_per_edge
    out = {
        "n_edge_records": r.n_edge_records, "n_solid": r.n_solid, "words_per_edge": wpe,
        "edges": np.ctypeslib.as_array(r.edges, (max(r.n_solid, 1) * wpe,))[: r.n_solid * wpe].reshape(-1, wpe).copy(),
        "cand_ids": (np.ctypeslib.as_array(r.cand_ids, (max(r.n_cand, 1),))[: r.n_cand].copy()
                     if want_mercy else np.zeros(0, np.uint64)),
        "n_has_tips": r.n_has_tips, "counting": np.array(r.counting, dtype=np.int64),
        "ms": {k_: getattr(r, f"t_{k_}_ms") for k_ in ("h2d", "extract", "sort", "count", "mercy", "d2h", "total")},
        "sort_pass_ms": list(r.sort_pass_ms[: r.n_sort_passes]), "n_rounds": int(r.n_rounds),
    }
    L.mhb_free(r.edges)
    if want_mercy:
        L.mhb_free(r.cand_ids)
    return out


def s2s_host(words: np.ndarray, word_off: np.ndarray, length: np.ndarray, mult: np.ndarray, k: int) -> dict:
    L = load()
    words = np.ascontiguousarray(words, np.uint32)
    if len(words) == 0:
        words = np.zeros(1, np.uint32)
    word_off = np.ascontiguousarray(word_off, np.uint64)
    n = len(word_off) - 1
    length = np.ascontiguousarray(length, np.uint32) if n else np.zeros(1, np.uint32)
    mult = np.ascontiguousarray(mult, np.uint16) if n else np.zeros(1, np.uint16)
    a = S2sArgs(k, words.ctypes.data, word_off.ctypes.data, length.ctypes.data, mult.ctypes.data, n)
    r = S2sResult()
    _check(L.mhb_s2s_host(C.byref(a), C.byref(r)))
    table = np.array(r.bucket_table, np.uint64).reshape(NUM_BUCKETS, 4)
    out = {
        "n_records": r.n_records, "n_items": r.n_items, "n_tips": r.n_tips, "n_large_mul": r.n_large_mul,
        "n_bytes": r.n_bytes, "words_per_tip_label": r.words_per_tip_label,
        "bytes": bytes(np.ctypeslib.as_array(r.bytes, (max(r.n_bytes, 1),))[: r.n_bytes]),
        "bucket_table": table, "w_count": np.array(r.w_count, np.uint64), "ones_in_last": r.ones_in_last,
        "ms": {k_: getattr(r, f"t_{k_}_ms") for k_ in ("extract", "sort", "emit", "total")},
    }
    L.mhb_free(r.bytes)
    return out


def build_host(bin_words: np.ndarray, n_reads: int, k: int, m: int, need_mercy: bool = True, want_edges: bool = False,
               sdbg_out: np.ndarray | None = None, copy_bytes: bool = True) -> dict:
    L = load()
    bin_words = np.ascontiguousarray(bin_words, dtype=np.uint32).reshape(-1)
    a = BuildArgs(k, m, bin_words.ctypes.data if len(bin_words) else None, len(bin_words), n_reads, int(need_mercy),
                  int(want_edges), sdbg_out.ctypes.data if sdbg_out is not None else None,
                  sdbg_out.nbytes if sdbg_out is not None else 0)
    r = BuildResult()
    _check(L.mhb_build_host(C.byref(a), C.byref(r)))
    in_place = sdbg_out is not None and C.addressof(r.bytes.contents) == sdbg_out.ctypes.data if r.n_bytes else sdbg_out is not None
    out = {
        "n_edge_records": r.n_edge_records, "n_solid": r.n_solid, "n_cand": r.n_cand, "n_mercy": r.n_mercy,
        "n_sort_items": r.n_sort_items, "n_items": r.n_items, "n_tips": r.n_tips, "n_large_mul": r.n_large_mul,
        "n_bytes": r.n_bytes, "words_per_tip_label": r.words_per_tip_label,
        "bucket_table": np.ctypeslib.as_array(r.bucket_table, (NUM_BUCKETS * 4,)).reshape(NUM_BUCKETS, 4).copy(),
        "w_count": np.array(r.w_count, np.uint64), "ones_in_last": r.ones_in_last,
        "ms": {k_: getattr(r, f"t_{k_}_ms") for k_ in ("total", "h2d", "count", "mercy", "s2s", "d2h")},
    }
    if copy_bytes:
        out["bytes"] = bytes(np.ctypeslib.as_array(r.bytes, (max(r.n_bytes, 1),))[: r.n_bytes])
    if not in_place:
        L.mhb_free(r.bytes)
    L.mhb_free(r.bucket_table)
    if want_edges:
        wpe = r.words_per_edge
        out["edges"] = np.ctypeslib.as_array(r.edges, (max(r.n_solid, 1) * wpe,))[: r.n_solid * wpe].reshape(-1, wpe).copy()
        out["cand_ids"] = np.ctypeslib.as_array(r.cand_ids, (max(r.n_cand, 1),))[: r.n_cand].copy()
        out["counting"] = np.ctypeslib.as_array(r.counting, (65536,)).copy()
        L.mhb_free(r.edges)
        L.mhb_free(r.cand_ids)
        L.mhb_free(r.counting)
    return out


def read2sdbg_host(bin_words: np.ndarray, n_reads: int, k: int, m: int, need_mercy: bool = True) -> dict:
    L = load()
    bin_words = np.ascontiguousarray(bin_words, dtype=np.uint32).reshape(-1)
# ... 188 lines not shown
```

Before: 14.66 billion.

## Add bucketed shared-memory local sort for seq2sdbg records

Adds a dedicated s2s sort that partitions records by the top 16 bits into 65536 buckets and sorts each bucket in shared memory with a packed 64-bit local key. Oversized buckets fall back to a global path. All seq2sdbg callers are routed to it in place of the generic multi-pass LSD radix sort. Event tracing becomes optional in the generic sort. The aim is to avoid many global radix passes, at the cost of extra complexity and fallback paths for skewed buckets.

Result: faster. 16.04 billion (median of 6 runs) (+9.4%).

```diff
diff --git a/include/mhb.h b/include/mhb.h
--- a/include/mhb.h
+++ b/include/mhb.h
@@ -55,6 +55,12 @@
 
 int mhb_sort_records_relaxed(void *stream, uint32_t *a, uint32_t *b, uint64_t n, uint32_t words, const uint8_t *bytes,
                              uint32_t n_bytes, const uint64_t *first_hist, void *ws, size_t ws_bytes, int *result_in_b);
+
+int mhb_s2s_sort(void *stream, uint32_t *a, uint32_t *b, uint64_t n, uint32_t k, const uint64_t *first_hist, void *ws,
+                 size_t ws_bytes, int *result_in_b);
+size_t mhb_s2s_sort_workspace_bytes(uint64_t n, uint32_t k);
+int mhb_s2s_sort_hist_byte(uint64_t n, uint32_t k);
+void mhb_s2s_sort_stats(uint64_t *n_oversized, uint64_t *oversized_items, uint64_t *n_large);
 
 int mhb_partition_scatter(void *stream, const uint32_t *recs, uint64_t n, uint32_t words, int byte,
                           const uint8_t *owner_of_byte_dev, const uint64_t *bin_addr_dev, void *ws, size_t ws_bytes);
@@ -360,6 +366,7 @@
                                     uint64_t *rec4_out, uint32_t *strand4_out);
 int mhb_selftest_s2s_record(const uint32_t *seq_words, uint32_t nwords, uint32_t L, uint32_t k, uint32_t strand,
                             uint32_t offset, uint32_t mult, uint32_t *rec_out);
+int mhb_selftest_s2s_local_key(const uint32_t *recs, uint64_t n, uint32_t k, uint64_t *keys_out);
 
 int mhb_selftest_r2s_s1_record(const uint32_t *pkg_words, uint32_t nwords, uint32_t L, uint32_t k, uint32_t e,
                                uint64_t base_off, uint32_t *rec_out);
diff --git a/megahit_b200/csrc/mhb_hashcount.cu b/megahit_b200/csrc/mhb_hashcount.cu
--- a/megahit_b200/csrc/mhb_hashcount.cu
+++ b/megahit_b200/csrc/mhb_hashcount.cu
@@ -22,18 +22,6 @@
 constexpr u32 kHcPrefetchChunk = 16384;
 
 __device__ __forceinline__ u64 rec_key64(const uint2 r) { return ((u64)r.x << 32) | r.y; }
-
-__global__ void k_bucket_bounds(const uint2 *__restrict__ recs, u64 n, u64 *__restrict__ bounds) {
-  const u32 b = blockIdx.x * blockDim.x + threadIdx.x;
-  if (b > 65536u) return;
-  u64 lo = 0, hi = n;
-  while (lo < hi) {
-    const u64 mid = (lo + hi) >> 1;
-    if ((recs[mid].x >> 16) < b) lo = mid + 1;
-    else hi = mid;
-  }
-  bounds[b] = lo;
-}
 
 __device__ __forceinline__ u64 hc_align(const uint2 *__restrict__ recs, u64 p, u64 lo, u64 hi) {
   if (p <= lo) return lo;
@@ -558,7 +546,7 @@
   u64 *n_slices_dev = (u64 *)(misc + 2);
   CK(cudaMemsetAsync(misc, 0, 256, st));
   CK(cudaMemsetAsync(slice_count, 0, L.max_slices * 4, st));
-  k_bucket_bounds<<<(65537 + 255) / 256, 256, 0, st>>>(recs, n, bounds);
+  k_bucket_bounds<2><<<(65537 + 255) / 256, 256, 0, st>>>(reinterpret_cast<const u32 *>(recs), n, bounds);
   CK_LAUNCH();
   k_slice_counts<<<65536 / 256, 256, 0, st>>>(bounds, HcGeomB::SLICE, bcnt);
   CK_LAUNCH();
diff --git a/megahit_b200/csrc/mhb_host.cu b/megahit_b200/csrc/mhb_host.cu
--- a/megahit_b200/csrc/mhb_host.cu
+++ b/megahit_b200/csrc/mhb_host.cu
@@ -676,7 +676,7 @@
 
 namespace {
 size_t s2s_round_bytes(uint64_t n, uint32_t W, uint32_t k) {
-  return 2 * Arena::pad((size_t)n * W * 4 + 16) + Arena::pad(mhb_sort_workspace_bytes(n, W)) +
+  return 2 * Arena::pad((size_t)n * W * 4 + 16) + Arena::pad(mhb_s2s_sort_workspace_bytes(n, k)) +
          Arena::pad(mhb_s2s_emit_scratch_bytes(n, k)) + Arena::pad((size_t)n * (4ull + 4ull * words_per_tip_label(k)) + 16);
 }
 }
@@ -686,8 +686,6 @@
   const uint32_t k = args->k;
   const uint64_t ns = args->n_seqs;
   const uint32_t W = s2s_record_words(k), WPT = words_per_tip_label(k);
-  uint8_t sort_bytes[72];
-  const uint32_t n_sort = mhb_s2s_sort_bytes(k, sort_bytes);
   const int top_byte = (int)(4 * W - 1);
   cudaStream_t st = 0;
   Timer t_all(st), t(st);
@@ -723,7 +721,7 @@
   uint64_t *d_cursor = g_arena.take<uint64_t>(8);
   uint32_t *d_a = g_arena.take<uint32_t>((size_t)max_items * W + 4);
   uint32_t *d_b = g_arena.take<uint32_t>((size_t)max_items * W + 4);
-  const size_t ws_bytes = mhb_sort_workspace_bytes(max_items, W);
+  const size_t ws_bytes = mhb_s2s_sort_workspace_bytes(max_items, k);
   const size_t scratch_bytes = mhb_s2s_emit_scratch_bytes(max_items, k);
   const uint64_t cap_bytes = max_items * (4ull + 4ull * WPT) + 16;
   char *d_ws = g_arena.take<char>(ws_bytes);
@@ -773,7 +771,7 @@
     t.start();
     CK(cudaMemsetAsync(d_hist0, 0, 256 * 8, st));
     CK(cudaMemsetAsync(d_cursor, 0, 64, st));
-    CKR(mhb_s2s_extract_range(st, &seqs, k, d_a, n_items, r_lo[ri], r_hi[ri], d_cursor, max_items, d_hist0, sort_bytes[0]));
+    CKR(mhb_s2s_extract_range(st, &seqs, k, d_a, n_items, r_lo[ri], r_hi[ri], d_cursor, max_items, d_hist0, mhb_s2s_sort_hist_byte(max_items, k)));
     uint64_t n_round = 0;
     CK(cudaMemcpyAsync(&n_round, d_cursor, 8, cudaMemcpyDeviceToHost, st));
     CK(cudaStreamSynchronize(st));
@@ -782,7 +780,8 @@
     if (n_round == 0) continue;
     t.start();
     int in_b = 0;
-    CKR(mhb_sort_records_impl(st, d_a, d_b, n_round, W, sort_bytes, n_sort, d_hist0, d_ws, ws_bytes, &in_b, nullptr));
+    const bool hist_ok = mhb_s2s_sort_hist_byte(n_round, k) == mhb_s2s_sort_hist_byte(max_items, k);
+    CKR(mhb_s2s_sort(st, d_a, d_b, n_round, k, hist_ok ? d_hist0 : nullptr, d_ws, ws_bytes, &in_b));
     res->t_sort_ms += t.stop();
     t.start();
     CKR(mhb_s2s_emit(st, in_b ? d_b : d_a, n_round, k, d_bytes, cap_bytes, d_table, d_totals, d_scratch, scratch_bytes));
@@ -831,9 +830,7 @@
   Timer t_all(st), t(st);
   t_all.start();
   const uint32_t W = s2s_record_words(k);
-  uint8_t sort_bytes[72];
-  const uint32_t n_sort = mhb_s2s_sort_bytes(k, sort_bytes);
-  const size_t ws_bytes = mhb_sort_workspace_bytes(n_items, W);
+  const size_t ws_bytes = mhb_s2s_sort_workspace_bytes(n_items, k);
   const size_t scratch_bytes = mhb_s2s_emit_scratch_bytes(n_items, k);
   const uint64_t cap_bytes = n_items * (4ull + 4ull * res->words_per_tip_label) + 16;
   size_t need = Arena::pad(n_words * 4 + 64) + Arena::pad((ns + 1) * 8) * 2 + Arena::pad((ns + 1) * 4) +
@@ -885,11 +882,11 @@
   seqs.fixed_stride = 0;
 
   t.start();
-  CKR(mhb_s2s_extract(st, &seqs, k, d_a, n_items, d_hist0, sort_bytes[0]));
+  CKR(mhb_s2s_extract(st, &seqs, k, d_a, n_items, d_hist0, mhb_s2s_sort_hist_byte(n_items, k)));
   res->t_extract_ms = t.stop();
   t.start();
   int in_b = 0;
-  CKR(mhb_sort_records_impl(st, d_a, d_b, n_items, W, sort_bytes, n_sort, d_hist0, d_ws, ws_bytes, &in_b, nullptr));
+  CKR(mhb_s2s_sort(st, d_a, d_b, n_items, k, d_hist0, d_ws, ws_bytes, &in_b));
   res->t_sort_ms = t.stop();
   t.start();
   CKR(mhb_s2s_emit(st, in_b ? d_b : d_a, n_items, k, d_bytes, cap_bytes, d_table, d_totals, d_scratch, scratch_bytes));
@@ -1062,8 +1059,8 @@
   Timer t_all(st), t(st);
   t_all.start();
 
-  uint8_t cbytes[72], sbytes[72];
-  const uint32_t n_csort = mhb_count_sort_bytes(k, cbytes), n_ssort = mhb_s2s_sort_bytes(k, sbytes);
+  uint8_t cbytes[72];
+  const uint32_t n_csort = mhb_count_sort_bytes(k, cbytes);
   const int32_t m = args->m;
   const uint64_t cap_edges = n / (uint64_t)std::max(1, m) + 1;
   const size_t bin_bytes = (args->bin_words * 4 + 15) & ~(size_t)15;
@@ -1235,7 +1232,7 @@
   const uint64_t n_seqs = n_solid + n_mercy;
   const uint64_t n_items = n_seqs * 6;
   res->n_sort_items = n_items;
-  const size_t s_ws = mhb_sort_workspace_bytes(n_items, W2), s_scr = mhb_s2s_emit_scratch_bytes(n_items, k);
+  const size_t s_ws = mhb_s2s_sort_workspace_bytes(n_items, k), s_scr = mhb_s2s_emit_scratch_bytes(n_items, k);
   const uint64_t cap_bytes = n_items * (4ull + 4ull * WPT) + 16;
   const size_t s2s_work = 2 * Arena::pad((size_t)n_items * W2 * 4 + 16) + Arena::pad(s_ws) + Arena::pad(s_scr) + Arena::pad(cap_bytes);
   char *sw = work;
@@ -1266,16 +1263,17 @@
   uint64_t n_sorted = n_items;
   if (!no_prune) {
     CK(cudaMemsetAsync(d_nsolid + 4, 0, 8, st));
-    CKR(mhb_s2s_extract_edges_pruned(st, d_all_edges, d_aux, n_seqs, n_solid, k, s_a, n_items, d_nsolid + 4, d_hist1, sbytes[0]));
+    CKR(mhb_s2s_extract_edges_pruned(st, d_all_edges, d_aux, n_seqs, n_solid, k, s_a, n_items, d_nsolid + 4, d_hist1, mhb_s2s_sort_hist_byte(n_items, k)));
     CK(cudaMemcpyAsync(&n_sorted, d_nsolid + 4, 8, cudaMemcpyDeviceToHost, st));
     CK(cudaStreamSynchronize(st));
     if (n_sorted > n_items) return mhb_set_error(MHB_ERR_CUDA, "internal: pruned item count exceeds 6 per edge");
     res->n_sort_items = n_sorted;
   } else {
-    CKR(mhb_s2s_extract(st, &seqs, k, s_a, n_items, d_hist1, sbytes[0]));
+    CKR(mhb_s2s_extract(st, &seqs, k, s_a, n_items, d_hist1, mhb_s2s_sort_hist_byte(n_items, k)));
   }
   int s_in_b = 0;
-  CKR(mhb_sort_records_impl(st, s_a, s_b, n_sorted, W2, sbytes, n_ssort, d_hist1, s_wsp, s_ws, &s_in_b, nullptr));
+  const bool hist_ok = mhb_s2s_sort_hist_byte(n_sorted, k) == mhb_s2s_sort_hist_byte(n_items, k);
+  CKR(mhb_s2s_sort(st, s_a, s_b, n_sorted, k, hist_ok ? d_hist1 : nullptr, s_wsp, s_ws, &s_in_b));
   CKR(mhb_s2s_emit(st, s_in_b ? s_b : s_a, n_sorted, k, d_bytes, cap_bytes, d_table, d_totals, s_scrp, s_scr));
   uint64_t totals[16];
   CK(cudaMemcpyAsync(totals, d_totals, sizeof(totals), cudaMemcpyDeviceToHost, st));
diff --git a/megahit_b200/csrc/mhb_internal.h b/megahit_b200/csrc/mhb_internal.h
--- a/megahit_b200/csrc/mhb_internal.h
+++ b/megahit_b200/csrc/mhb_internal.h
@@ -9,6 +9,11 @@
 int mhb_sort_records_impl(void *stream, uint32_t *a, uint32_t *b, uint64_t n, uint32_t words, const uint8_t *bytes,
                           uint32_t n_bytes, const uint64_t *first_hist, void *ws, size_t ws_bytes, int *result_in_b,
                           double *pass_ms_host);
+int mhb_sort_records_ex(void *stream, uint32_t *a, uint32_t *b, uint64_t n, uint32_t words, const uint8_t *bytes,
+                        uint32_t n_bytes, const uint64_t *first_hist, void *ws, size_t ws_bytes, int *result_in_b,
+                        double *pass_ms_host, int relaxed);
+int mhb_sort_records_untraced(void *stream, uint32_t *a, uint32_t *b, uint64_t n, uint32_t words, const uint8_t *bytes,
+                              uint32_t n_bytes, const uint64_t *first_hist, void *ws, size_t ws_bytes, int *result_in_b);
 
 size_t mhb_arena_bytes(void);
 
diff --git a/megahit_b200/csrc/mhb_kernels.cuh b/megahit_b200/csrc/mhb_kernels.cuh
--- a/megahit_b200/csrc/mhb_kernels.cuh
+++ b/megahit_b200/csrc/mhb_kernels.cuh
@@ -114,6 +114,16 @@
   rec[W - 1] |= 65535u - counting;
 }
 
+template <int W>
+MHB_HD u64 s2s_local_key(const u32 (&r)[W], u32 k) {
+  u32 w2 = 0;
+  if constexpr (W >= 3) w2 = r[2];
+  const u64 top = ((u64)r[0] << 48) | ((u64)r[1] << 16) | (w2 >> 16);
+  const u32 kb = 2 * k - 16;
+  const u64 flags = (r[W - 1] >> 16) & 15u;
+  return (top & ~(~0ull >> kb)) | (flags << (60 - kb));
+}
+
 #if defined(__CUDACC__)
 template <int WR>
 __device__ __forceinline__ void ld_rec(const u32 *base, u64 idx, u32 (&r)[WR]) {
@@ -161,6 +171,19 @@
 template <int WR>
 __device__ __forceinline__ u32 rec_byte(const u32 (&r)[WR], int b) {
   return (pick<WR>(r, (u32)(WR - 1 - (b >> 2))) >> (8 * (b & 3))) & 255u;
+}
+
+template <int W>
+__global__ void k_bucket_bounds(const u32 *__restrict__ recs, u64 n, u64 *__restrict__ bounds) {
+  const u32 b = blockIdx.x * blockDim.x + threadIdx.x;
+  if (b > 65536u) return;
+  u64 lo = 0, hi = n;
+  while (lo < hi) {
+    const u64 mid = (lo + hi) >> 1;
+    if ((recs[mid * W] >> 16) < b) lo = mid + 1;
+    else hi = mid;
+  }
+  bounds[b] = lo;
 }
 
 __device__ __forceinline__ u32 lane_id() { return threadIdx.x & 31; }
diff --git a/megahit_b200/csrc/mhb_r2s.cu b/megahit_b200/csrc/mhb_r2s.cu
--- a/megahit_b200/csrc/mhb_r2s.cu
+++ b/megahit_b200/csrc/mhb_r2s.cu
@@ -191,7 +191,7 @@
 
 size_t s2_pass_bytes(uint64_t n, uint32_t W, uint32_t k) {
   const uint64_t n_tiles = (n + kDdTile - 1) / kDdTile;
-  return 2 * pad((size_t)n * W * 4 + 16) + pad(mhb_sort_workspace_bytes(n, W)) + pad(n_tiles * 4) + pad(n_tiles * 8) +
+  return 2 * pad((size_t)n * W * 4 + 16) + pad(mhb_s2s_sort_workspace_bytes(n, k)) + pad(n_tiles * 4) + pad(n_tiles * 8) +
          pad((n_tiles / 4096 + 4) * 8) + pad((size_t)n * 8) + pad(mhb_s2s_emit_scratch_bytes(n, k)) +
          pad((size_t)n * (4ull + 4ull * words_per_tip_label(k)) + 16);
 }
@@ -435,11 +435,9 @@
                  unsigned long long *d_counter, PhaseTrace &tr, uint64_t *n_u_out, uint64_t *cap_bytes) {
   const uint32_t W = s2s_record_words(k), WPT = words_per_tip_label(k);
   DevBuf &a = big.a, &b = big.b, &ws = big.ws;
-  const size_t ws_bytes = mhb_sort_workspace_bytes(n, W);
-  uint8_t sbytes[80];
-  const uint32_t n_sb = mhb_s2s_sort_bytes(k, sbytes);
+  const size_t ws_bytes = mhb_s2s_sort_workspace_bytes(n, k);
   int in_b = 0;
-  CKR(mhb_sort_records_relaxed(st, a.as<u32>(), b.as<u32>(), n, W, sbytes, n_sb, nullptr, ws.p, ws_bytes, &in_b));
+  CKR(mhb_s2s_sort(st, a.as<u32>(), b.as<u32>(), n, k, nullptr, ws.p, ws_bytes, &in_b));
   tr.mark("s2.sort");
   const u32 *sorted = in_b ? b.as<u32>() : a.as<u32>();
   u32 *uniq = in_b ? a.as<u32>() : b.as<u32>();
@@ -600,10 +598,10 @@
     const bool rounds = (max_n && ix.n_s1 > max_n) || s1_one > avail;
     if (!rounds) {
       const size_t rec1 = pad((size_t)ix.n_s1 * RW * 4 + 16), ws1 = pad(mhb_sort_workspace_bytes(ix.n_s1, RW));
-      const size_t rec2 = pad((size_t)est_items * W * 4 + 16), ws2 = pad(mhb_sort_workspace_bytes(est_items, W));
+      const size_t rec2 = pad((size_t)est_items * W * 4 + 16), ws2 = pad(mhb_s2s_sort_workspace_bytes(est_items, k));
       const bool share = s1_one - 2 * rec1 - ws1 + 2 * std::max(rec1, rec2) + std::max(ws1, ws2) <= avail;
       CKR(run_stage1(st, pv, ix, k, m, mercy, so, d_hist.as<unsigned long long>(), tr, big,
-                     share ? (size_t)est_items * W * 4 + 16 : 0, share ? mhb_sort_workspace_bytes(est_items, W) : 0));
+                     share ? (size_t)est_items * W * 4 + 16 : 0, share ? mhb_s2s_sort_workspace_bytes(est_items, k) : 0));
       res->n_rounds_s1 = 1;
     } else {
       if (!max_n) {
@@ -664,7 +662,7 @@
   } else if (!s2_rounds) {
     S2Bufs sb;
     DevBuf &a = big.a, &b = big.b, &ws = big.ws;
-    const size_t rec_bytes = (size_t)n_items * W * 4 + 16, ws_bytes = mhb_sort_workspace_bytes(n_items, W);
+    const size_t rec_bytes = (size_t)n_items * W * 4 + 16, ws_bytes = mhb_s2s_sort_workspace_bytes(n_items, k);
     CKR(a.ensure(rec_bytes, "stage-2 items"));
     CKR(b.ensure(rec_bytes, "stage-2 items (sort buffer)"));
     CKR(ws.ensure(ws_bytes, "sort workspace"));
@@ -730,7 +728,7 @@
     CKR(plan_bucket_ranges(h_h16, max_items, &ranges));
     CKR(big.a.ensure((size_t)max_items * W * 4 + 16, "stage-2 items"));
     CKR(big.b.ensure((size_t)max_items * W * 4 + 16, "stage-2 items (sort buffer)"));
-    CKR(big.ws.ensure(mhb_sort_workspace_bytes(max_items, W), "sort workspace"));
+    CKR(big.ws.ensure(mhb_s2s_sort_workspace_bytes(max_items, k), "sort workspace"));
     S2Bufs sb;
     SdbgStitch out;
     uint64_t seen = 0;
diff --git a/megahit_b200/csrc/mhb_s2s_sort.cu b/megahit_b200/csrc/mhb_s2s_sort.cu
--- /dev/null
+++ b/megahit_b200/csrc/mhb_s2s_sort.cu
@@ -0,0 +1,289 @@
+#include <cuda_runtime.h>
+
+#include <algorithm>
+#include <stdio.h>
+#include <stdlib.h>
+#include <string.h>
+
+#include "mhb.h"
+#include "mhb_common.cuh"
+#include "mhb_kernels.cuh"
+
+using namespace mhb;
+
+namespace {
+
+constexpr u32 kLsCapS = 3072, kLsCapL = 8192;
+constexpr int kLsThreadsS = 512, kLsThreadsL = 1024;
+constexpr int kLsDigitBits = 12;
+constexpr u32 kLsDigits = 1u << kLsDigitBits;
+constexpr u32 kLsGroupMax = 256;
+constexpr u32 kLsListCap = 16;
+constexpr uint64_t kLsMaxItems = (uint64_t)MHB_NUM_BUCKETS * kLsCapL * 3 / 4;
+constexpr uint64_t kLsSmallMaxItems = (uint64_t)MHB_NUM_BUCKETS * kLsCapS * 3 / 4;
+
+struct LsCtl {
+  unsigned int ticket, ticket2;
+  unsigned int n_mid;
+  unsigned int n_over;
+  unsigned long long items_over;
+  unsigned long long range[2 * kLsListCap];
+};
+
+template <int W, u32 CAP>
+constexpr size_t ls_smem() {
+  return (size_t)CAP * 8  + ((size_t)CAP * W + 4) * 4  + (kLsDigits + 4) * 4  +
+         (size_t)CAP * 2 * 2 ;
+}
+
+template <int W, u32 CAP, int THREADS>
+__global__ void __launch_bounds__(THREADS, CAP == kLsCapS ? 2 : 1)
+    k_s2s_local_sort(const u32 *__restrict__ in, u32 *__restrict__ out, const u64 *__restrict__ bounds, u32 k, LsCtl *ctl,
+                     unsigned int *ticket, const u32 *__restrict__ ids, u32 n_ids, u32 *mid) {
+  constexpr u32 kLsCap = CAP;
+  constexpr int kLsThreads = THREADS;
+  constexpr int kLsIpt = CAP / THREADS;
+  extern __shared__ __align__(16) unsigned char smem_ls[];
+  u64 *s_key = reinterpret_cast<u64 *>(smem_ls);
+  u32 *s_rec = reinterpret_cast<u32 *>(s_key + kLsCap);
+  u32 *s_grp = s_rec + kLsCap * W + 4;
+  uint16_t *s_src = reinterpret_cast<uint16_t *>(s_grp + kLsDigits + 4);
+  uint16_t *s_perm = s_src + kLsCap;
+  __shared__ u32 s_ticket;
+  __shared__ u32 s_scan[kLsThreads / 32 + 1];
+  const u32 tid = threadIdx.x;
+  const u32 n_units = ids ? n_ids : (u32)MHB_NUM_BUCKETS;
+  if (tid == 0) s_ticket = atomicAdd(ticket, 1u);
+  __syncthreads();
+  u32 t = s_ticket;
+  while (t < n_units) {
+    u32 next = 0;
+    if (tid == 0) next = atomicAdd(ticket, 1u);
+    const u32 b = ids ? ids[t] : t;
+    const u64 lo = bounds[b], hi = bounds[b + 1];
+    bool local = hi - lo <= kLsCap;
+    if (!local && mid && hi - lo <= kLsCapL) {
+      if (tid == 0) mid[atomicAdd(&ctl->n_mid, 1u)] = b;
+      local = true;
+    } else if (local && hi > lo) {
+      const u32 n = (u32)(hi - lo);
+      const u64 w_begin = lo * W, w_end = hi * W, a0 = w_begin & ~3ull;
+      const u32 off = (u32)(w_begin - a0);
+      const u32 nvec = (u32)((w_end - a0) >> 2);
+      const uint4 *src4 = reinterpret_cast<const uint4 *>(in + a0);
+      uint4 *dst4 = reinterpret_cast<uint4 *>(s_rec);
+      for (u32 j0 = 0; j0 < nvec; j0 += 4 * kLsThreads) {
+        uint4 v[4];
+#pragma unroll
+        for (int q = 0; q < 4; ++q) {
+          const u32 j = j0 + q * kLsThreads + tid;
+          if (j < nvec) v[q] = __ldg(src4 + j);
+        }
+#pragma unroll
+        for (int q = 0; q < 4; ++q) {
+          const u32 j = j0 + q * kLsThreads + tid;
+          if (j < nvec) dst4[j] = v[q];
+        }
+      }
+      for (u64 x = a0 + 4ull * nvec + tid; x < w_end; x += kLsThreads) s_rec[x - a0] = __ldg(in + x);
+      for (u32 i = tid; i <= kLsDigits; i += kLsThreads) s_grp[i] = 0;
+      __syncthreads();
+      u64 key[kLsIpt];
+      u32 dr[kLsIpt];
+#pragma unroll
+      for (int q = 0; q < kLsIpt; ++q) {
+        const u32 i = tid + q * kLsThreads;
+        if (i < n) {
+          u32 r[W];
+#pragma unroll
+          for (int j = 0; j < W; ++j) r[j] = s_rec[off + i * W + j];
+          key[q] = s2s_local_key<W>(r, k);
+          const u32 d = (u32)(key[q] >> (64 - kLsDigitBits));
+          dr[q] = (d << 16) | atomicAdd(&s_grp[d], 1u);
+        }
+      }
+      __syncthreads();
+      constexpr int GPT = kLsDigits / kLsThreads;
+      u32 c[GPT], sum = 0, cmax = 0;
+#pragma unroll
+      for (int j = 0; j < GPT; ++j) {
+        c[j] = s_grp[tid * GPT + j];
+        sum += c[j];
+        cmax = max(cmax, c[j]);
+      }
+      u32 total;
+      u32 run = block_excl_scan<kLsThreads>(sum, s_scan, total);
+#pragma unroll
+      for (int j = 0; j < GPT; ++j) {
+        s_grp[tid * GPT + j] = run;
+        run += c[j];
+      }
+      if (tid == 0) s_grp[kLsDigits] = n;
+      local = !__syncthreads_or(cmax > kLsGroupMax);
+      if (local) {
+#pragma unroll
+        for (int q = 0; q < kLsIpt; ++q) {
+          const u32 i = tid + q * kLsThreads;
+          if (i < n) {
+            const u32 p = s_grp[dr[q] >> 16] + (dr[q] & 0xFFFFu);
+            s_key[p] = key[q];
+            s_src[p] = (uint16_t)i;
+          }
+        }
+        __syncthreads();
+        for (u32 p = tid; p < n; p += kLsThreads) {
+          const u64 x = s_key[p];
+          const u32 d = (u32)(x >> (64 - kLsDigitBits));
+          const u32 g0 = s_grp[d], g1 = s_grp[d + 1];
+          u32 rank = g0;
+          for (u32 u = g0; u < g1; ++u) {
+            const u64 y = s_key[u];
+            rank += (y < x || (y == x && u < p)) ? 1u : 0u;
+          }
+          s_perm[rank] = s_src[p];
+        }
+        __syncthreads();
+        for (u32 x = tid; x < n * W; x += kLsThreads) {
+          const u32 i = x / W, j = x - i * W;
+          out[w_begin + x] = s_rec[off + (u32)s_perm[i] * W + j];
+        }
+      }
+    }
+    if (!local && tid == 0) {
+      const u32 slot = atomicAdd(&ctl->n_over, 1u);
+      atomicAdd(&ctl->items_over, (unsigned long long)(hi - lo));
+      if (slot < kLsListCap) {
+        ctl->range[2 * slot] = lo;
+        ctl->range[2 * slot + 1] = hi;
+      }
+    }
+    __syncthreads();
+    if (tid == 0) s_ticket = next;
+    __syncthreads();
+    t = s_ticket;
+  }
+}
+
+bool s2s_local_path(uint32_t k) {
+  const u32 w = s2s_record_words(k);
+  return k >= 9 && (w == 2 || w == 3);
+}
+size_t pad256(size_t x) { return (x + 255) & ~(size_t)255; }
+
+template <int W, u32 CAP, int THREADS>
+int launch_local_sort(cudaStream_t st, const u32 *in, u32 *out, const u64 *bounds, u32 k, LsCtl *ctl, unsigned int *ticket,
+                      const u32 *ids, u32 n_ids, u32 *mid) {
+  constexpr size_t smem = ls_smem<W, CAP>();
+  static int bps = 0;
+  if (!bps) {
+    CK(cudaFuncSetAttribute(k_s2s_local_sort<W, CAP, THREADS>, cudaFuncAttributeMaxDynamicSharedMemorySize, (int)smem));
+    CK(cudaOccupancyMaxActiveBlocksPerMultiprocessor(&bps, k_s2s_local_sort<W, CAP, THREADS>, THREADS, smem));
+    if (bps < 1) return mhb_set_error(MHB_ERR_CUDA, "bucket sort kernel (W=%d, capacity %u) does not fit an SM", W, CAP);
+    if (getenv("MHB_VERBOSE")) fprintf(stderr, "[mhb] s2s bucket sort W=%d: %d threads, capacity %u, %zu B smem, %d CTA/SM\n", W, THREADS, CAP, smem, bps);
+  }
+  const u32 units = ids ? n_ids : (u32)MHB_NUM_BUCKETS;
+  const int grid = (int)std::min<u64>((u64)bps * sm_count(), units);
+  k_s2s_local_sort<W, CAP, THREADS><<<grid, THREADS, smem, st>>>(in, out, bounds, k, ctl, ticket, ids, n_ids, mid);
+  CK_LAUNCH();
+  return MHB_OK;
+}
+
+template <int W>
+int launch_local(cudaStream_t st, bool large, const u32 *in, u32 *out, const u64 *bounds, u32 k, LsCtl *ctl, unsigned int *ticket,
+                 const u32 *ids, u32 n_ids, u32 *mid) {
+  if (large) return launch_local_sort<W, kLsCapL, kLsThreadsL>(st, in, out, bounds, k, ctl, ticket, ids, n_ids, nullptr);
+  return launch_local_sort<W, kLsCapS, kLsThreadsS>(st, in, out, bounds, k, ctl, ticket, ids, n_ids, mid);
+}
+
+bool s2s_bucket_path(uint64_t n, uint32_t k) { return s2s_local_path(k) && n <= kLsMaxItems; }
+
+LsCtl g_last_ctl;
+
+}
+
+extern "C" int mhb_s2s_sort_hist_byte(uint64_t n, uint32_t k) {
+  return s2s_bucket_path(n, k) ? (int)(4 * s2s_record_words(k) - 2) : 2;
+}
+
+extern "C" size_t mhb_s2s_sort_workspace_bytes(uint64_t n, uint32_t k) {
+  const uint32_t W = s2s_record_words(k);
+  const size_t base = pad256(mhb_sort_workspace_bytes(n, W));
+  if (!s2s_local_path(k)) return base;
+  return base + pad256((size_t)(MHB_NUM_BUCKETS + 1) * 8) + pad256(sizeof(LsCtl)) + pad256((size_t)MHB_NUM_BUCKETS * 4);
+}
+
+extern "C" int mhb_s2s_sort(void *stream, uint32_t *a, uint32_t *b, uint64_t n, uint32_t k, const uint64_t *first_hist,
+                            void *ws, size_t ws_bytes, int *result_in_b) {
+  if (k < 1 || k > MHB_MAX_K || !result_in_b) return mhb_set_error(MHB_ERR_ARG, "bad seq2sdbg sort arguments (k=%u)", k);
+  const uint32_t W = s2s_record_words(k);
+  uint8_t bytes[80];
+  const uint32_t nb = mhb_s2s_sort_bytes(k, bytes);
+  const size_t sort_ws = mhb_sort_workspace_bytes(n, W);
+  g_last_ctl = LsCtl{};
+  if (!s2s_bucket_path(n, k)) return mhb_sort_records_relaxed(stream, a, b, n, W, bytes, nb, first_hist, ws, ws_bytes, result_in_b);
+  *result_in_b = 0;
+  if (n == 0) return MHB_OK;
+  if (ws_bytes < mhb_s2s_sort_workspace_bytes(n, k)) return mhb_set_error(MHB_ERR_ARG, "seq2sdbg sort workspace too small");
+  if ((((uintptr_t)a | (uintptr_t)b) & 15) != 0) return mhb_set_error(MHB_ERR_ARG, "seq2sdbg sort buffers must be 16-byte aligned");
+  cudaStream_t st = (cudaStream_t)stream;
+  const uint8_t top[2] = {(uint8_t)(4 * W - 2), (uint8_t)(4 * W - 1)};
+  int in_b = 0;
+  if (int rc = mhb_sort_records_ex(stream, a, b, n, W, top, 2, first_hist, ws, sort_ws, &in_b, nullptr, 1)) return rc;
+  u32 *x = in_b ? b : a, *y = in_b ? a : b;
+  u64 *bounds = reinterpret_cast<u64 *>((char *)ws + pad256(sort_ws));
+  LsCtl *ctl = reinterpret_cast<LsCtl *>((char *)bounds + pad256((size_t)(MHB_NUM_BUCKETS + 1) * 8));
+  u32 *mid = reinterpret_cast<u32 *>((char *)ctl + pad256(sizeof(LsCtl)));
+  CK(cudaMemsetAsync(ctl, 0, sizeof(LsCtl), st));
+  if (W == 2) k_bucket_bounds<2><<<(65537 + 255) / 256, 256, 0, st>>>(x, n, bounds);
+  else k_bucket_bounds<3><<<(65537 + 255) / 256, 256, 0, st>>>(x, n, bounds);
+  CK_LAUNCH();
+  const bool large = n > kLsSmallMaxItems;
+  if (int rc = W == 2 ? launch_local<2>(st, large, x, y, bounds, k, ctl, &ctl->ticket, nullptr, 0, mid)
+                      : launch_local<3>(st, large, x, y, bounds, k, ctl, &ctl->ticket, nullptr, 0, mid)) return rc;
+  LsCtl h;
+  CK(cudaMemcpyAsync(&h, ctl, sizeof(h), cudaMemcpyDeviceToHost, st));
+  CK(cudaStreamSynchronize(st));
+  if (h.n_mid) {
+    if (int rc = W == 2 ? launch_local<2>(st, true, x, y, bounds, k, ctl, &ctl->ticket2, mid, h.n_mid, nullptr)
+                        : launch_local<3>(st, true, x, y, bounds, k, ctl, &ctl->ticket2, mid, h.n_mid, nullptr)) return rc;
+    CK(cudaMemcpyAsync(&h, ctl, sizeof(h), cudaMemcpyDeviceToHost, st));
+    CK(cudaStreamSynchronize(st));
+  }
+  g_last_ctl = h;
+  *result_in_b = y == b ? 1 : 0;
+  if (h.n_over == 0) return MHB_OK;
+  if (h.n_over > kLsListCap) {
+    int r_in_b = 0;
+    if (int rc = mhb_sort_records_untraced(stream, x, y, n, W, bytes, nb, nullptr, ws, sort_ws, &r_in_b)) return rc;
+    *result_in_b = (r_in_b ? y : x) == b ? 1 : 0;
+    return MHB_OK;
+  }
+  for (u32 s = 0; s < h.n_over; ++s) {
+    const u64 lo = h.range[2 * s], hi = h.range[2 * s + 1];
+    int r_in_b = 0;
+    if (int rc = mhb_sort_records_untraced(stream, x + lo * W, y + lo * W, hi - lo, W, bytes, nb - 2, nullptr, ws, sort_ws, &r_in_b)) return rc;
+    if (!r_in_b) CK(cudaMemcpyAsync(y + lo * W, x + lo * W, (hi - lo) * W * 4, cudaMemcpyDeviceToDevice, st));
+  }
+  return MHB_OK;
+}
+
+extern "C" void mhb_s2s_sort_stats(uint64_t *n_oversized, uint64_t *oversized_items, uint64_t *n_large) {
+  if (n_oversized) *n_oversized = g_last_ctl.n_over;
+  if (oversized_items) *oversized_items = g_last_ctl.items_over;
+  if (n_large) *n_large = g_last_ctl.n_mid;
+}
+
+extern "C" int mhb_selftest_s2s_local_key(const uint32_t *recs, uint64_t n, uint32_t k, uint64_t *keys) {
+  if (!s2s_local_path(k) || !recs || !keys) return mhb_set_error(MHB_ERR_ARG, "bad local-key arguments (k=%u)", k);
+  const uint32_t W = s2s_record_words(k);
+  for (uint64_t i = 0; i < n; ++i) {
+    if (W == 2) {
+      const u32 r[2] = {recs[2 * i], recs[2 * i + 1]};
+      keys[i] = s2s_local_key<2>(r, k);
+    } else {
+      const u32 r[3] = {recs[3 * i], recs[3 * i + 1], recs[3 * i + 2]};
+      keys[i] = s2s_local_key<3>(r, k);
+    }
+  }
+  return MHB_OK;
+}
diff --git a/megahit_b200/csrc/mhb_sortdisp.cu b/megahit_b200/csrc/mhb_sortdisp.cu
--- a/megahit_b200/csrc/mhb_sortdisp.cu
+++ b/megahit_b200/csrc/mhb_sortdisp.cu
@@ -209,17 +209,27 @@
 uint64_t g_trace_seq = 0;
 }
 
-int mhb_sort_records_ex(void *stream, uint32_t *a, uint32_t *b, uint64_t n, uint32_t words, const uint8_t *bytes,
-                        uint32_t n_bytes, const uint64_t *first_hist, void *ws, size_t ws_bytes, int *result_in_b,
-                        double *pass_ms_host, int relaxed);
+static int sort_records_core(void *stream, uint32_t *a, uint32_t *b, uint64_t n, uint32_t words, const uint8_t *bytes,
+                             uint32_t n_bytes, const uint64_t *first_hist, void *ws, size_t ws_bytes, int *result_in_b,
+                             double *pass_ms_host, int relaxed, bool trace);
 int mhb_sort_records_impl(void *stream, uint32_t *a, uint32_t *b, uint64_t n, uint32_t words, const uint8_t *bytes,
                           uint32_t n_bytes, const uint64_t *first_hist, void *ws, size_t ws_bytes, int *result_in_b,
                           double *pass_ms_host) {
-  return mhb_sort_records_ex(stream, a, b, n, words, bytes, n_bytes, first_hist, ws, ws_bytes, result_in_b, pass_ms_host, 1);
+  return sort_records_core(stream, a, b, n, words, bytes, n_bytes, first_hist, ws, ws_bytes, result_in_b, pass_ms_host, 1, true);
 }
 int mhb_sort_records_ex(void *stream, uint32_t *a, uint32_t *b, uint64_t n, uint32_t words, const uint8_t *bytes,
-                          uint32_t n_bytes, const uint64_t *first_hist, void *ws, size_t ws_bytes, int *result_in_b,
+                        uint32_t n_bytes, const uint64_t *first_hist, void *ws, size_t ws_bytes, int *result_in_b,
                         double *pass_ms_host, int relaxed) {
+  return sort_records_core(stream, a, b, n, words, bytes, n_bytes, first_hist, ws, ws_bytes, result_in_b, pass_ms_host, relaxed, true);
+}
+int mhb_sort_records_untraced(void *stream, uint32_t *a, uint32_t *b, uint64_t n, uint32_t words, const uint8_t *bytes,
+                              uint32_t n_bytes, const uint64_t *first_hist, void *ws, size_t ws_bytes, int *result_in_b) {
+  return sort_records_core(stream, a, b, n, words, bytes, n_bytes, first_hist, ws, ws_bytes, result_in_b, nullptr, 1, false);
+}
+static int sort_records_core(void *stream, uint32_t *a, uint32_t *b, uint64_t n, uint32_t words, const uint8_t *bytes,
+                             uint32_t n_bytes, const uint64_t *first_hist, void *ws, size_t ws_bytes, int *result_in_b,
+                             double *pass_ms_host, int relaxed, bool trace) {
+  if (pass_ms_host && !trace) return mhb_set_error(MHB_ERR_ARG, "per-pass times need a traced sort");
   static const bool stable_first = getenv("MHB_SORT_STABLE_FIRST") != nullptr;
   if (stable_first) relaxed = 0;
   if (words < 1 || words > 17 || n_bytes > 72 || !result_in_b)
@@ -244,15 +254,18 @@
 #undef M
     CK_LAUNCH();
   }
-  SortTrace &tr = g_trace[g_trace_seq++ & 3];
-  if (!tr.created) {
-    for (int i = 0; i < 74; ++i) CK(cudaEventCreate(&tr.ev[i]));
-    tr.created = true;
-  }
-  tr.n_passes = n_bytes;
-  tr.words = words;
-  tr.n = n;
-  CK(cudaEventRecord(tr.ev[0], st));
+  SortTrace *tr = nullptr;
+  if (trace) {
+    tr = &g_trace[g_trace_seq++ & 3];
+    if (!tr->created) {
+      for (int i = 0; i < 74; ++i) CK(cudaEventCreate(&tr->ev[i]));
+      tr->created = true;
+    }
+    tr->n_passes = n_bytes;
+    tr->words = words;
+    tr->n = n;
+    CK(cudaEventRecord(tr->ev[0], st));
+  }
   u32 *in = a, *out = b;
   for (u32 p = 0; p < n_bytes; ++p) {
     k_hist_scan256<<<1, 256, 0, st>>>(hist + (u64)p * 256, bin_base, (u64)(uintptr_t)out, words * 4);
@@ -269,17 +282,17 @@
 #undef M
     }
     if (rc) return rc;
-    CK(cudaEventRecord(tr.ev[p + 1], st));
+    if (tr) CK(cudaEventRecord(tr->ev[p + 1], st));
     u32 *t = in;
     in = out;
     out = t;
   }
   *result_in_b = (in == b) ? 1 : 0;
   if (pass_ms_host) {
-    CK(cudaEventSynchronize(tr.ev[n_bytes]));
+    CK(cudaEventSynchronize(tr->ev[n_bytes]));
     for (u32 p = 0; p < n_bytes; ++p) {
       float ms = 0;
-      CK(cudaEventElapsedTime(&ms, tr.ev[p], tr.ev[p + 1]));
+      CK(cudaEventElapsedTime(&ms, tr->ev[p], tr->ev[p + 1]));
       pass_ms_host[p] = ms;
     }
   }
diff --git a/megahit_b200/dev.py b/megahit_b200/dev.py
--- a/megahit_b200/dev.py
+++ b/megahit_b200/dev.py
@@ -27,6 +27,16 @@
     fn = L.mhb_sort_records_relaxed if relaxed else L.mhb_sort_records
     lib._check(fn(_stream(), _ptr(a), _ptr(b), n, words, bytes_arr, len(sort_bytes), _ptr(first_hist), _ptr(ws), ws.numel(),
                   C.byref(in_b)))
+    return b if in_b.value else a
+
+
+def s2s_sort(a: torch.Tensor, b: torch.Tensor, n: int, k: int, first_hist=None, ws=None):
+    L = lib.load()
+    need = L.mhb_s2s_sort_workspace_bytes(n, k)
+    if ws is None or ws.numel() < need:
+        ws = torch.empty(need, dtype=torch.uint8, device=a.device)
+    in_b = C.c_int(0)
+    lib._check(L.mhb_s2s_sort(_stream(), _ptr(a), _ptr(b), n, k, _ptr(first_hist), _ptr(ws), ws.numel(), C.byref(in_b)))
     return b if in_b.value else a
 
 
@@ -167,7 +177,7 @@
         i32 = dict(dtype=torch.int32, device=device)
         self.a = torch.empty(n * self.W + 4, **i32)
         self.b = torch.empty(n * self.W + 4, **i32)
-        self.ws = torch.empty(L.mhb_sort_workspace_bytes(n, self.W), dtype=torch.uint8, device=device)
+        self.ws = torch.empty(L.mhb_s2s_sort_workspace_bytes(n, k), dtype=torch.uint8, device=device)
         self.scratch = torch.empty(L.mhb_s2s_emit_scratch_bytes(n, k), dtype=torch.uint8, device=device)
         wpt = (k + 15) // 16
         self.cap_bytes = n * (4 + 4 * wpt) + 16
@@ -192,10 +202,10 @@
         if timed:
             ev[0].record()
         lib._check(self.L.mhb_s2s_extract(_stream(), C.byref(seqs), self.k, _ptr(self.a), self.n_items, _ptr(self.hist0),
-                                          self.sort_bytes[0]))
+                                          lib.s2s_sort_hist_byte(self.n_items, self.k)))
         if timed:
             ev[1].record()
-        srt = sort_records(self.a, self.b, self.n_items, self.W, self.sort_bytes, self.hist0, self.ws, relaxed=True)
+        srt = s2s_sort(self.a, self.b, self.n_items, self.k, self.hist0, self.ws)
         if timed:
             ev[2].record()
         lib._check(self.L.mhb_s2s_emit(_stream(), _ptr(srt), self.n_items, self.k, _ptr(self.bytes), self.cap_bytes,
@@ -213,12 +223,14 @@
         if timed:
             ev[0].record()
         lib._check(self.L.mhb_s2s_extract_edges_pruned(_stream(), _ptr(edges), _ptr(aux), n_edges, n_aux, self.k, _ptr(self.a),
-                                                       cap, _ptr(self.cursor), _ptr(self.hist0), self.sort_bytes[0]))
+                                                       cap, _ptr(self.cursor), _ptr(self.hist0),
+                                                       lib.s2s_sort_hist_byte(cap, self.k)))
         self.n_items = int(self.cursor.item())
         assert self.n_items <= cap
         if timed:
             ev[1].record()
-        srt = sort_records(self.a, self.b, self.n_items, self.W, self.sort_bytes, self.hist0, self.ws, relaxed=True)
+        same = lib.s2s_sort_hist_byte(self.n_items, self.k) == lib.s2s_sort_hist_byte(cap, self.k)
+        srt = s2s_sort(self.a, self.b, self.n_items, self.k, self.hist0 if same else None, self.ws)
         if timed:
             ev[2].record()
         lib._check(self.L.mhb_s2s_emit(_stream(), _ptr(srt), self.n_items, self.k, _ptr(self.bytes), self.cap_bytes,
diff --git a/megahit_b200/lib.py b/megahit_b200/lib.py
--- a/megahit_b200/lib.py
+++ b/megahit_b200/lib.py
@@ -135,6 +135,8 @@
     "mhb_iterate_host", "mhb_iterate_run", "mhb_selftest_iterate", "mhb_s2s_extract_edges_pruned", "mhb_s2s_emit_fmt", "mhb_read2sdbg_host", "mhb_read2sdbg_run", "mhb_selftest_r2s_s1_record", "mhb_selftest_r2s_item",
     "mhb_selftest_kmsort", "mhb_selftest_kmsort_smem", "mhb_selftest_r2s_s1_group", "mhb_selftest_r2s_mercy_read",
     "mhb_buildlib_host", "mhb_buildlib_free", "mhb_set_buildlib_chunk", "mhb_buildlib_run", "mhb_selftest_fastx",
+    "mhb_s2s_sort", "mhb_s2s_sort_workspace_bytes", "mhb_s2s_sort_hist_byte", "mhb_s2s_sort_stats",
+    "mhb_selftest_s2s_local_key",
 ]
 
 
@@ -163,6 +165,14 @@
     L.mhb_sort_records.argtypes = [C.c_void_p, C.c_void_p, C.c_void_p, C.c_uint64, C.c_uint32, C.c_void_p, C.c_uint32,
                                    C.c_void_p, C.c_void_p, C.c_size_t, C.POINTER(C.c_int)]
     L.mhb_sort_records_relaxed.argtypes = L.mhb_sort_records.argtypes
+    L.mhb_s2s_sort.argtypes = [C.c_void_p, C.c_void_p, C.c_void_p, C.c_uint64, C.c_uint32, C.c_void_p, C.c_void_p, C.c_size_t,
+                               C.POINTER(C.c_int)]
+    L.mhb_s2s_sort_workspace_bytes.argtypes = [C.c_uint64, C.c_uint32]
+    L.mhb_s2s_sort_workspace_bytes.restype = C.c_size_t
+    L.mhb_s2s_sort_hist_byte.argtypes = [C.c_uint64, C.c_uint32]
+    L.mhb_s2s_sort_stats.argtypes = [C.POINTER(C.c_uint64), C.POINTER(C.c_uint64), C.POINTER(C.c_uint64)]
+    L.mhb_s2s_sort_stats.restype = None
+    L.mhb_selftest_s2s_local_key.argtypes = [C.c_void_p, C.c_uint64, C.c_uint32, C.c_void_p]
     L.mhb_count_solid.argtypes = [C.c_void_p, C.c_void_p, C.c_uint64, C.c_uint32, C.c_int32, C.c_void_p, C.c_void_p,
                                   C.c_uint64, C.c_void_p, C.c_void_p, C.c_void_p, C.c_size_t]
     L.mhb_count_hashed_workspace_bytes.restype = C.c_size_t
@@ -361,6 +371,23 @@
     return list(buf[:n])
 
 
+def s2s_sort_hist_byte(n: int, k: int) -> int:
+    return load().mhb_s2s_sort_hist_byte(C.c_uint64(n), C.c_uint32(k))
+
+
+def s2s_sort_stats() -> tuple[int, int, int]:
+    a, b, c = C.c_uint64(), C.c_uint64(), C.c_uint64()
+    load().mhb_s2s_sort_stats(C.byref(a), C.byref(b), C.byref(c))
+    return a.value, b.value, c.value
+
+
+def selftest_s2s_local_key(recs: np.ndarray, k: int) -> np.ndarray:
+    recs = np.ascontiguousarray(recs, dtype=np.uint32)
+    keys = np.zeros(len(recs), dtype=np.uint64)
+    _check(load().mhb_selftest_s2s_local_key(recs.ctypes.data, len(recs), k, keys.ctypes.data))
+    return keys
+
+
 def count_host(bin_words: np.ndarray, n_reads: int, k: int, m: int, want_mercy: bool = True) -> dict:
     L = load()
     bin_words = np.ascontiguousarray(bin_words, dtype=np.uint32).reshape(-1)
```
